# chemprop/chemprop

Measured on AMD Instinct MI355X. Metric: million directed-edge-updates/sec (depth=3, hidden=300), higher is better.
Workload: dtype f32 (exact 3-term f16 split of fp32 operands, fp32 accumulate); 1 GPU; qm9-shaped synthetic molecules, 512 mols/GPU/step, BondMessagePassing depth=3 hidden=300, forward (plan K0 + K1..K5); mols_per_gpu=512, directed_edges_per_gpu=9120, parallelism=dp1 (molecule shards, no data-path collective), launch=eager

## Files before the change

### chemprop_amd/_lib.py

```python
from __future__ import annotations

import ctypes as C
import os
import shutil
import subprocess
from typing import Optional

_HERE = os.path.dirname(os.path.abspath(__file__))
_ROOT = os.path.dirname(_HERE)
CSRC = os.path.join(_HERE, "csrc")
INCLUDE = os.path.join(_ROOT, "include")
LIB_PATH = os.environ.get("DMPNN_LIB") or os.path.join(_HERE, "libdmpnn_gfx950.so")
SOURCES = ["dmpnn_abi.hip", "dmpnn_prepare.hip", "dmpnn_segment.hip", "dmpnn_gemm.hip", "dmpnn_gemm_p1.hip",
           "dmpnn_gemm_p2.hip", "dmpnn_gemm_p3.hip", "dmpnn_gemm_p4.hip", "dmpnn_gemm_s1.hip", "dmpnn_mega.hip", "dmpnn_mega16.hip", "dmpnn_mega16_lp.hip", "dmpnn_mega16_bwd.hip", "dmpnn_rows16.hip", "dmpnn_step16.hip", "dmpnn_bstep16.hip", "dmpnn_backward.hip", "dmpnn_molagg.hip", "dmpnn_collate.hip", "dmpnn_tiles_large.hip", "dmpnn_optim.hip", "dmpnn_wgrad16.hip", "dmpnn_head.hip", "dmpnn_vd.hip"]
HEADERS = ["dmpnn_common.hpp", "dmpnn_spill_impl.hpp", "dmpnn_gemm_impl.hpp", "dmpnn_mega_impl.hpp", "dmpnn_mega16_impl.hpp", "dmpnn_mega16_bwd_impl.hpp", "dmpnn_rows16_impl.hpp", "dmpnn_seg16.hpp", "dmpnn_step16_impl.hpp"]
ABI_VERSION = 15
PLAN_NOFFSETS = 15

EXPORTS = [
    "dmpnn_version", "dmpnn_debug_timestamps", "dmpnn_last_error_string", "dmpnn_last_launch_count", "dmpnn_plan_bytes",
    "dmpnn_plan_layout", "dmpnn_prepare", "dmpnn_prepare_light", "dmpnn_prepare_tiles", "dmpnn_message_fwd", "dmpnn_aggregate_fwd",
    "dmpnn_linear_fwd", "dmpnn_linear16_wsplit_bytes", "dmpnn_linear16_ok", "dmpnn_linear16_fwd", "dmpnn_update_fwd", "dmpnn_forward", "dmpnn_forward_can_fuse", "dmpnn_forward_wsplit_bytes", "dmpnn_forward_keep_bits_bytes", "dmpnn_forward_spill_bytes", "dmpnn_backward_ws_bytes", "dmpnn_backward", "dmpnn_message_bwd",
    "dmpnn_aggregate_bwd", "dmpnn_linear_wgrad_ws_bytes", "dmpnn_linear_wgrad",
    "dmpnn_molagg_ws_bytes", "dmpnn_molagg_bounds", "dmpnn_molagg_fwd", "dmpnn_molagg_bwd", "dmpnn_gather_rows", "dmpnn_collate", "dmpnn_pack_tiles", "dmpnn_max_tiles",
    "dmpnn_prepare_tiles_from_table", "dmpnn_prepare_with_batch", "dmpnn_tile_plan_any_size", "dmpnn_split_row_floats", "dmpnn_forward_can_fuse16", "dmpnn_adam_step",
    "dmpnn_full_plan_keeps_tiles", "dmpnn_head_ws_bytes", "dmpnn_head", "dmpnn_train_step", "dmpnn_forward_tiles", "dmpnn_forward_route", "dmpnn_dropout_keep",
    "dmpnn_clip_grad", "dmpnn_clip_grad_ws_bytes", "dmpnn_train_route", "dmpnn_forward_h0_bytes", "dmpnn_tile_waves", "dmpnn_debug_lds_poison",
    "dmpnn_vd_ws_bytes", "dmpnn_vd_forward", "dmpnn_vd_backward",
]

ACT = {"none": 0, "relu": 1, "leakyrelu": 2, "prelu": 3, "tanh": 4, "elu": 5}
F_UNDIRECTED = 1
F_FUSED = 2
F_MEGA = 4
F_KEEP = 8
F_SPLIT16 = 16
F_WSPLIT_READY = 32
F_LOADER_TILES = 64
F_STORE16 = 128
F_ATOM = 1024
F_TILE_PLAN = 2048
F_H0_RESIDUAL = 256
F_ROW_FINALIZE = 512
ROUTES = ("general", "general16", "fused", "fused16", "mega", "mega16")
PLAN_NOMEGA_MASK = 15
PLAN_NOFUSE_MASK = 7


class GemmArgs(C.Structure):
    _fields_ = [
        ("M", C.c_int64), ("N", C.c_int64), ("K1", C.c_int64), ("K2", C.c_int64),
        ("A1", C.c_void_p), ("lda1", C.c_int64), ("gather1", C.c_void_p), ("gather1_rows", C.c_int64),
        ("A2", C.c_void_p), ("lda2", C.c_int64),
        ("W", C.c_void_p), ("ldw", C.c_int64),
        ("bias", C.c_void_p),
        ("Cadd", C.c_void_p), ("ldcadd", C.c_int64),
        ("C", C.c_void_p), ("ldc", C.c_int64),
        ("Zpre", C.c_void_p), ("ldz", C.c_int64),
        ("act", C.c_int), ("act_slope", C.c_float), ("act_slope_ptr", C.c_void_p),
    ]


class FwdArgs(C.Structure):
    _fields_ = [
        ("plan", C.c_void_p), ("n_atoms", C.c_int64), ("n_edges", C.c_int64),
        ("d_v", C.c_int64), ("d_e", C.c_int64), ("d_h", C.c_int64), ("d_vd", C.c_int64),
        ("depth", C.c_int32), ("flags", C.c_uint32),
        ("act", C.c_int32), ("act_slope", C.c_float), ("act_slope_ptr", C.c_void_p),
        ("V", C.c_void_p), ("ldv", C.c_int64),
        ("E", C.c_void_p), ("lde", C.c_int64),
        ("V_d", C.c_void_p), ("ldvd", C.c_int64),
        ("W_i", C.c_void_p), ("b_i", C.c_void_p),
        ("W_h", C.c_void_p), ("b_h", C.c_void_p),
        ("W_o", C.c_void_p), ("b_o", C.c_void_p),
        ("W_d", C.c_void_p), ("b_d", C.c_void_p),
        ("ldh", C.c_int64), ("H0", C.c_void_p), ("Hs", C.c_void_p), ("n_hslots", C.c_int32),
        ("Ms", C.c_void_p), ("n_mslots", C.c_int32),
        ("Mv", C.c_void_p), ("Hv", C.c_void_p),
        ("out", C.c_void_p), ("ldout", C.c_int64),
        ("wsplit", C.c_void_p), ("wsplit_bytes", C.c_size_t),
        ("edge_index", C.c_void_p), ("rev_edge_index", C.c_void_p),
        ("n_tiles_launch", C.c_int64),
        ("spill_ws", C.c_void_p), ("spill_bytes", C.c_size_t),
        ("msplit", C.c_void_p), ("msplit_bytes", C.c_size_t),
        ("dropout_p", C.c_float), ("dropout_seed", C.c_uint64),
        ("keep_bits", C.c_void_p), ("keep_bits_bytes", C.c_size_t),
        ("h0_bytes", C.c_size_t),
    ]


class BwdArgs(C.Structure):
    _fields_ = [
        ("f", FwdArgs), ("gout", C.c_void_p), ("ldgout", C.c_int64),
        ("gW_i", C.c_void_p), ("gb_i", C.c_void_p), ("gW_h", C.c_void_p), ("gb_h", C.c_void_p),
        ("gW_o", C.c_void_p), ("gb_o", C.c_void_p), ("gW_d", C.c_void_p), ("gb_d", C.c_void_p),
        ("ws", C.c_void_p), ("ws_bytes", C.c_size_t),
        ("g_edge", C.c_void_p), ("ld_gedge", C.c_int64),
    ]


MAX_FFN_LAYERS = 8
MAX_COMPONENTS = 8
DROP_SITE_FFN = 0x10000
LOSS = {"mse": 0, "mae": 1, "bce": 2, "ce": 3, "mve": 4, "evidential": 5, "quantile": 6}
STEP_FORWARD, STEP_BACKWARD, STEP_UPDATE = 1, 2, 4


class HeadArgs(C.Structure):
    _fields_ = [
        ("n_atoms", C.c_int64), ("n_mols", C.c_int64), ("d_h", C.c_int64),
        ("batch", C.c_void_p),
        ("agg_mode", C.c_int32), ("agg_norm", C.c_float),
        ("bn_weight", C.c_void_p), ("bn_bias", C.c_void_p), ("bn_running_mean", C.c_void_p), ("bn_running_var", C.c_void_p),
        ("bn_eps", C.c_float), ("bn_momentum", C.c_float), ("bn_training", C.c_int32),
        ("n_layers", C.c_int32), ("act", C.c_int32), ("act_slope", C.c_float),
        ("W", C.c_void_p * MAX_FFN_LAYERS), ("b", C.c_void_p * MAX_FFN_LAYERS), ("dims", C.c_int64 * (MAX_FFN_LAYERS + 1)),
        ("loss", C.c_int32),
        ("targets", C.c_void_p), ("weights", C.c_void_p), ("task_weights", C.c_void_p), ("lt_mask", C.c_void_p), ("gt_mask", C.c_void_p),
        ("preds", C.c_void_p), ("loss_out", C.c_void_p),
        ("gW", C.c_void_p * MAX_FFN_LAYERS), ("gb", C.c_void_p * MAX_FFN_LAYERS), ("g_bn_weight", C.c_void_p), ("g_bn_bias", C.c_void_p),
        ("gHv", C.c_void_p), ("ldg", C.c_int64),
        ("ws", C.c_void_p), ("ws_bytes", C.c_size_t),
        ("bn_num_batches_tracked", C.c_void_p),
        ("n_classes", C.c_int32),
        ("evid_v_kl", C.c_float), ("evid_eps", C.c_float), ("quantile_alpha", C.c_float),
        ("X_d", C.c_void_p), ("ld_xd", C.c_int64),
        ("n_components", C.c_int32),
        ("ffn_dropout_p", C.c_float), ("ffn_dropout_seed", C.c_uint64),
    ]


class TrainRouteInfo(C.Structure):
    _fields_ = [("plan_kind", C.c_int32), ("route", C.c_int32), ("keep_rows", C.c_int32), ("keep_bits", C.c_int32), ("lean", C.c_int32)]


class StepComponent(C.Structure):
    _fields_ = [
        ("edge_index", C.c_void_p), ("rev_edge_index", C.c_void_p), ("batch", C.c_void_p), ("plan_bytes", C.c_size_t), ("plan_ready", C.c_int32),
        ("bwd", BwdArgs),
    ]


class VdArgs(C.Structure):
    _fields_ = [
        ("n_atoms", C.c_int64), ("d_h", C.c_int64), ("d_vd", C.c_int64),
        ("Hv", C.c_void_p), ("ldhv", C.c_int64),
        ("V_d", C.c_void_p), ("ldvd", C.c_int64),
        ("W_d", C.c_void_p), ("b_d", C.c_void_p),
        ("out", C.c_void_p), ("ldout", C.c_int64),
        ("gout", C.c_void_p), ("ldgout", C.c_int64),
        ("gHv", C.c_void_p), ("ldghv", C.c_int64),
        ("gW_d", C.c_void_p), ("gb_d", C.c_void_p),
        ("ws", C.c_void_p), ("ws_bytes", C.c_size_t),
    ]


VD_MAX_WIDTH = 544


class StepArgs(C.Structure):
    _fields_ = [
        ("edge_index", C.c_void_p), ("rev_edge_index", C.c_void_p), ("batch", C.c_void_p), ("plan_bytes", C.c_size_t), ("plan_ready", C.c_int32),
        ("stages", C.c_int32),
        ("bwd", BwdArgs), ("head", HeadArgs),
        ("p", C.c_void_p), ("g", C.c_void_p), ("m", C.c_void_p), ("v", C.c_void_p), ("n_params", C.c_int64),
        ("lr", C.c_float), ("beta1", C.c_float), ("beta2", C.c_float), ("eps", C.c_float), ("weight_decay", C.c_float),
        ("bias_corr1", C.c_float), ("sqrt_bias_corr2", C.c_float), ("grad_scale", C.c_float), ("dev_scalars", C.c_void_p),
        ("clip_val", C.c_float), ("clip_mode", C.c_int32), ("clip_ws", C.c_void_p),
        ("n_extra", C.c_int32), ("extra", C.POINTER(StepComponent)),
        ("vd", C.POINTER(VdArgs)),
    ]


def sources() -> list[str]:
    return [os.path.join(CSRC, s) for s in SOURCES if os.path.isfile(os.path.join(CSRC, s))]


def _stale() -> bool:
    if os.environ.get("DMPNN_LIB"):
        return False
    if not os.path.isfile(LIB_PATH):
        return True
    t = os.path.getmtime(LIB_PATH)
    deps = sources() + [os.path.join(CSRC, h) for h in HEADERS] + [os.path.join(INCLUDE, "dmpnn.h")]
    return any(os.path.getmtime(d) > t for d in deps if os.path.isfile(d))


def build(force: bool = False, verbose: bool = False, defines=(), out: Optional[str] = None) -> str:
    lib_path = out or LIB_PATH
    if not force and not _stale() and out is None:
        return LIB_PATH
    hipcc = shutil.which("hipcc") or "/opt/rocm/bin/hipcc"
    if not os.path.isfile(hipcc):
        raise RuntimeError("hipcc not found: cannot build libdmpnn_gfx950.so")
    import concurrent.futures as cf
    import tempfile

    flags = ["--offload-arch=gfx950", "-O3", "-std=c++17", "-fPIC", f"-I{INCLUDE}", f"-I{CSRC}", *[f"-D{d}" for d in defines]]
    with tempfile.TemporaryDirectory(prefix="dmpnn_build_") as tmp:
        def cc(src):
            obj = os.path.join(tmp, os.path.basename(src) + ".o")
            cmd = [hipcc, *flags, "-c", src, "-o", obj]
            if verbose:
                print(" ".join(cmd))
            r = subprocess.run(cmd, capture_output=True, text=True)
            if r.returncode != 0:
                raise RuntimeError(f"hipcc failed on {src} ({r.returncode}):\n{r.stdout}\n{r.stderr}")
            return obj

        with cf.ThreadPoolExecutor(max_workers=8) as ex:
            objs = list(ex.map(cc, sources()))
        linked = os.path.join(os.path.dirname(objs[0]), "libdmpnn.so")
        cmd = [hipcc, "--offload-arch=gfx950", "-shared", "-fPIC", *objs, "-o", linked]
        if verbose:
            print(" ".join(cmd))
        r = subprocess.run(cmd, capture_output=True, text=True)
        if r.returncode != 0:
            raise RuntimeError(f"hipcc link failed ({r.returncode}):\n{r.stdout}\n{r.stderr}")
        shutil.copyfile(linked, lib_path + ".tmp")
        os.chmod(lib_path + ".tmp", 0o755)
    os.replace(lib_path + ".tmp", lib_path)
    _clean_unbundle_temporaries(lib_path)
    return lib_path


def _clean_unbundle_temporaries(lib_path: str) -> int:
    import glob

    n = 0
    for f in glob.glob(glob.escape(lib_path) + ".*"):
        tail = f[len(lib_path) + 1:]
        if tail.split(".", 1)[0].isdigit() and ("hipv4-" in tail or "host-" in tail):
            try:
                os.remove(f)
                n += 1
            except OSError:
                pass
    return n


_lib: Optional[C.CDLL] = None


def load() -> C.CDLL:
    global _lib
    if _lib is not None:
        return _lib
    import torch

    if _stale() and (shutil.which("hipcc") or os.path.isfile("/opt/rocm/bin/hipcc")):
        build()
    if not os.path.isfile(LIB_PATH):
        raise RuntimeError(
            f"{LIB_PATH} is missing: run `python -c 'import __graft_entry__ as g; g.build()'` "
            "(the MI355X engine has no CPU / eager fallback)")
    lib = C.CDLL(LIB_PATH)
    lib.dmpnn_version.restype = C.c_int
    lib.dmpnn_last_error_string.restype = C.c_char_p
    lib.dmpnn_last_launch_count.restype = C.c_int
    lib.dmpnn_plan_bytes.restype = C.c_size_t
    lib.dmpnn_plan_bytes.argtypes = [C.c_int64, C.c_int64]
    lib.dmpnn_plan_layout.argtypes = [C.c_int64, C.c_int64, C.POINTER(C.c_int64)]
    lib.dmpnn_forward_can_fuse.argtypes = [C.POINTER(FwdArgs)]
    lib.dmpnn_prepare.argtypes = [C.c_void_p, C.c_void_p, C.c_int64, C.c_int64, C.c_void_p, C.c_size_t, C.c_void_p]
    lib.dmpnn_prepare_light.argtypes = lib.dmpnn_prepare.argtypes
    lib.dmpnn_prepare_tiles.argtypes = [C.c_void_p, C.c_void_p, C.c_void_p, C.c_int64, C.c_int64, C.c_void_p, C.c_size_t, C.c_void_p]
    lib.dmpnn_message_fwd.argtypes = [C.c_void_p, C.c_int64, C.c_int64, C.c_int64, C.c_void_p, C.c_int64,
                                      C.c_void_p, C.c_int64, C.c_int, C.c_float, C.c_void_p, C.c_uint, C.c_void_p]
    lib.dmpnn_aggregate_fwd.argtypes = [C.c_void_p, C.c_int64, C.c_int64, C.c_int64, C.c_void_p, C.c_int64,
                                        C.c_void_p, C.c_int64, C.c_int, C.c_float, C.c_void_p, C.c_void_p]
    lib.dmpnn_linear_fwd.argtypes = [C.POINTER(GemmArgs), C.c_void_p]
    lib.dmpnn_update_fwd.argtypes = [C.c_void_p, C.c_int64, C.c_int64, C.c_int64, C.c_void_p, C.c_int64, C.c_void_p, C.c_int64,
                                     C.c_void_p, C.c_void_p, C.c_void_p, C.c_int64, C.c_void_p, C.c_int64, C.c_void_p,
                                     C.c_int64, C.c_int, C.c_float, C.c_void_p, C.c_void_p]
    lib.dmpnn_forward.argtypes = [C.POINTER(FwdArgs), C.c_void_p]
    lib.dmpnn_backward_ws_bytes.argtypes = [C.POINTER(FwdArgs)]
    lib.dmpnn_backward.argtypes = [C.POINTER(BwdArgs), C.c_void_p]
    lib.dmpnn_message_bwd.argtypes = [C.c_void_p, C.c_int64, C.c_int64, C.c_int64, C.c_void_p, C.c_int64,
                                      C.c_void_p, C.c_int64, C.c_void_p]
    lib.dmpnn_aggregate_bwd.argtypes = lib.dmpnn_message_bwd.argtypes
    lib.dmpnn_linear_wgrad_ws_bytes.argtypes = [C.c_int64, C.c_int64, C.c_int64, C.c_int]
    lib.dmpnn_linear_wgrad.argtypes = [C.POINTER(GemmArgs), C.c_void_p, C.c_int64, C.c_void_p, C.c_int64,
                                       C.c_void_p, C.c_void_p, C.c_size_t, C.c_void_p]
    size_t_fns = ("dmpnn_plan_bytes", "dmpnn_backward_ws_bytes", "dmpnn_linear_wgrad_ws_bytes", "dmpnn_forward_wsplit_bytes", "dmpnn_forward_spill_bytes",
                  "dmpnn_forward_keep_bits_bytes",
                  "dmpnn_molagg_ws_bytes", "dmpnn_linear16_wsplit_bytes", "dmpnn_head_ws_bytes", "dmpnn_clip_grad_ws_bytes", "dmpnn_forward_h0_bytes", "dmpnn_vd_ws_bytes")
    lib.dmpnn_linear16_wsplit_bytes.argtypes = [C.c_int64, C.c_int64]
    lib.dmpnn_linear16_ok.argtypes = [C.POINTER(GemmArgs)]
    lib.dmpnn_linear16_fwd.argtypes = [C.POINTER(GemmArgs), C.c_void_p, C.c_size_t, C.c_int, C.c_void_p]
    lib.dmpnn_gather_rows.argtypes = [C.c_void_p, C.c_int64, C.c_int64, C.c_void_p, C.c_int64, C.c_int64, C.c_void_p, C.c_int64,
                                      C.c_void_p]
    lib.dmpnn_pack_tiles.argtypes = [C.c_void_p, C.c_void_p, C.c_int64, C.c_void_p, C.c_void_p, C.c_int64]
    lib.dmpnn_pack_tiles.restype = C.c_int64
    lib.dmpnn_max_tiles.argtypes = [C.c_int64, C.c_int64]
    lib.dmpnn_prepare_with_batch.argtypes = [C.c_void_p, C.c_void_p, C.c_void_p, C.c_int64, C.c_int64, C.c_void_p, C.c_size_t, C.c_void_p]
    lib.dmpnn_prepare_with_batch.restype = C.c_int
    lib.dmpnn_tile_plan_any_size.argtypes = [C.c_int64, C.c_int64]
    lib.dmpnn_max_tiles.restype = C.c_int64
    lib.dmpnn_prepare_tiles_from_table.argtypes = [C.c_void_p, C.c_void_p, C.c_int64, C.c_int64, C.c_int64, C.c_void_p, C.c_size_t,
                                                   C.c_void_p]
    lib.dmpnn_collate.argtypes = [C.c_void_p, C.c_void_p, C.c_int64, C.c_void_p, C.c_void_p, C.c_void_p, C.c_int64, C.c_int64,
                                  C.c_void_p, C.c_void_p, C.c_void_p, C.c_void_p]
    lib.dmpnn_molagg_ws_bytes.argtypes = [C.c_int64]
    lib.dmpnn_molagg_bounds.argtypes = [C.c_void_p, C.c_int64, C.c_int64, C.c_void_p, C.c_size_t, C.c_void_p]
    lib.dmpnn_molagg_fwd.argtypes = [C.c_void_p, C.c_int64, C.c_int64, C.c_int64, C.c_int64, C.c_void_p, C.c_int, C.c_float,
                                     C.c_void_p, C.c_int64, C.c_void_p]
    lib.dmpnn_molagg_bwd.argtypes = [C.c_void_p, C.c_int64, C.c_void_p, C.c_int64, C.c_int64, C.c_int64, C.c_void_p, C.c_int,
                                     C.c_float, C.c_void_p, C.c_int64, C.c_void_p]
    lib.dmpnn_forward_wsplit_bytes.argtypes = [C.POINTER(FwdArgs)]
    lib.dmpnn_forward_keep_bits_bytes.argtypes = [C.POINTER(FwdArgs)]
    lib.dmpnn_forward_spill_bytes.argtypes = [C.POINTER(FwdArgs)]
    lib.dmpnn_forward_h0_bytes.argtypes = [C.POINTER(FwdArgs)]
    lib.dmpnn_forward_can_fuse16.argtypes = [C.POINTER(FwdArgs)]
    lib.dmpnn_adam_step.argtypes = [C.c_void_p, C.c_void_p, C.c_void_p, C.c_void_p, C.c_int64, C.c_float, C.c_float, C.c_float, C.c_float,
                                    C.c_float, C.c_float, C.c_float, C.c_float, C.c_void_p, C.c_void_p]
    lib.dmpnn_train_route.argtypes = [C.POINTER(FwdArgs), C.c_int64, C.c_int32, C.c_int32, C.c_int32, C.c_int32, C.c_int32, C.POINTER(TrainRouteInfo)]
    lib.dmpnn_clip_grad.argtypes = [C.c_void_p, C.c_int64, C.c_float, C.c_int32, C.c_float, C.c_void_p, C.c_void_p]
    lib.dmpnn_dropout_keep.argtypes = [C.c_uint64, C.c_int32, C.c_int64, C.c_int64, C.c_float]
    lib.dmpnn_forward_route.argtypes = [C.POINTER(FwdArgs), C.c_int, C.c_int, C.c_int, C.c_int]
    lib.dmpnn_tile_waves.restype = C.c_int
    lib.dmpnn_tile_waves.argtypes = [C.c_int64, C.c_int64, C.c_int64, C.c_int64]
    lib.dmpnn_forward_tiles.argtypes = [C.POINTER(FwdArgs), C.c_void_p, C.c_void_p, C.c_void_p, C.c_int64, C.c_size_t, C.c_void_p]
    lib.dmpnn_full_plan_keeps_tiles.argtypes = [C.c_int64, C.c_int64]
    lib.dmpnn_head_ws_bytes.argtypes = [C.POINTER(HeadArgs)]
    lib.dmpnn_head.argtypes = [C.POINTER(HeadArgs), C.c_void_p, C.c_int64, C.c_void_p]
    lib.dmpnn_train_step.argtypes = [C.POINTER(StepArgs), C.c_void_p]
    lib.dmpnn_vd_ws_bytes.argtypes = [C.POINTER(VdArgs)]
    lib.dmpnn_vd_forward.argtypes = [C.POINTER(VdArgs), C.c_void_p]
    lib.dmpnn_vd_backward.argtypes = [C.POINTER(VdArgs), C.c_void_p]
    lib.dmpnn_split_row_floats.argtypes = [C.c_int64]
    lib.dmpnn_split_row_floats.restype = C.c_int64
    lib.dmpnn_debug_timestamps.argtypes = [C.c_void_p]
    for name in size_t_fns:
        getattr(lib, name).restype = C.c_size_t
    for name in EXPORTS:
        if name != "dmpnn_last_error_string" and name not in size_t_fns and name not in ("dmpnn_pack_tiles", "dmpnn_max_tiles", "dmpnn_split_row_floats"):
            getattr(lib, name).restype = C.c_int
    if lib.dmpnn_version() != ABI_VERSION:
        raise RuntimeError(f"libdmpnn ABI version {lib.dmpnn_version()} != {ABI_VERSION} (stale build?)")
    _lib = lib
    return lib


_ENV_DATA = getattr(os.environ, "_data", None)
_ENV_KEYS: dict = {}


def opt(name: str, default: str) -> str:
    if _ENV_DATA is None or os.name != "posix":
        return os.environ.get(name, default)
    k = _ENV_KEYS.get(name)
    if k is None:
        k = _ENV_KEYS[name] = name.encode()
    v = _ENV_DATA.get(k)
    return default if v is None else v.decode()


class DmpnnError(RuntimeError):
    pass


def check(rc: int, what: str) -> None:
    if rc != 0:
        msg = load().dmpnn_last_error_string().decode(errors="replace")
        raise DmpnnError(f"{what} failed (code {rc}): {msg}")
```

### chemprop_amd/csrc/dmpnn_abi.hip

```cpp
#include <stdarg.h>
#include <stdlib.h>
#include <string.h>

#include "dmpnn_common.hpp"
#include "dmpnn_mega16_impl.hpp"

namespace dmpnn {

static thread_local char g_err[512] = "";
static thread_local int g_launches = 0;

void set_error(const char* fmt, ...) {
    va_list ap;
    va_start(ap, fmt);
    vsnprintf(g_err, sizeof(g_err), fmt, ap);
    va_end(ap);
}
static __global__ __launch_bounds__(1024) void k_debug_lds_poison(unsigned pat, unsigned* sink) {
    extern __shared__ unsigned lds_words[];
    constexpr int n = (160 * 1024 - 64) / 4;
    for (int i = threadIdx.x; i < n; i += 1024) lds_words[i] = pat;
    __syncthreads();
    if (sink && lds_words[(threadIdx.x * 7) % n] == 0x12345u) sink[0] = 1;
}
// ... 209 lines not shown
    if (n_edges == 0) {
        if (Mv && n_atoms > 0) {
            for (int64_t v = 0; v < n_atoms; ++v)
                if (hipMemsetAsync(Mv + v * ld_mv, 0, (size_t)d_h * sizeof(float), static_cast<hipStream_t>(stream)) != hipSuccess) {
                    set_error("update_fwd: memset failed");
                    return DMPNN_EHIP;
                }
        }
        return DMPNN_OK;
    }
    const int* plan_i = static_cast<const int*>(plan);
    const PlanLayout L = plan_layout(n_atoms, n_edges);
    dmpnn_gemm_args g;
    memset(&g, 0, sizeof(g));
    g.M = n_edges; g.N = d_h; g.K1 = d_h;
    g.A1 = M; g.lda1 = ld_m;
    g.W = W_h; g.ldw = d_h; g.bias = b_h;
    g.Cadd = H0; g.ldcadd = ld_h0;
    g.C = H_out; g.ldc = ld_hout;
    g.act = act; g.act_slope = act_slope; g.act_slope_ptr = act_slope_ptr;
    GemmExtra x;
    memset(&x, 0, sizeof(x));
    x.seg = true;
    x.tile_row = plan_i + L.tile_row; x.tile_atom = plan_i + L.tile_atom; x.n_tiles = (int)L.max_tiles;
    x.row_ptr = plan_i + L.row_ptr; x.revp = plan_i + L.revp;
    x.Mout = M_next; x.ldm = ld_mnext; x.Sout = Mv; x.lds = ld_mv;
    return launch_linear_ex(g, x, static_cast<hipStream_t>(stream));
}

static size_t steps16_wsplit_bytes(const dmpnn_fwd_args& a) {
    const int64_t h = a.d_h;
    size_t n = linear16_wsplit_bytes(h, a.d_v + a.d_e) + linear16_wsplit_bytes(h, h) + linear16_wsplit_bytes(h, a.d_v + h);
    n += linear16_wsplit_bytes(h + a.d_vd, h + a.d_vd) * ((a.W_d && a.d_vd > 0) ? 1 : 0);
    n += linear16_wsplit_bytes(h, h) + linear16_wsplit_bytes(h, a.d_v);
    return n;
}

size_t dmpnn_forward_wsplit_bytes(const dmpnn_fwd_args* a) {
    if (!a || a->d_h <= 0 || a->d_v <= 0 || a->d_e < 0) return 0;
    return (a->flags & DMPNN_F_MEGA) ? mega16_wsplit_bytes(*a) : steps16_wsplit_bytes(*a);
}

static bool keep_bits_apply(const dmpnn_fwd_args& a) {
    const unsigned need = DMPNN_F_TILE_PLAN | DMPNN_F_KEEP | DMPNN_F_MEGA | DMPNN_F_SPLIT16 | DMPNN_F_FUSED;
    return (a.flags & need) == need && (a.act == DMPNN_ACT_NONE || a.act == DMPNN_ACT_RELU || a.act == DMPNN_ACT_LEAKYRELU) &&
           !(a.dropout_p > 0.f) && !a.W_d && a.n_atoms > 0 && a.n_edges > 0;
}
size_t dmpnn_forward_keep_bits_bytes(const dmpnn_fwd_args* a) {
    if (!a) return 0;
    if ((a->flags & (DMPNN_F_FUSED | DMPNN_F_SPLIT16)) == (DMPNN_F_FUSED | DMPNN_F_SPLIT16) && !(a->flags & DMPNN_F_MEGA)) return fused16_lean_bits_bytes(*a);
    if (!keep_bits_apply(*a)) return 0;
    return (size_t)a->depth * (size_t)plan_layout(a->n_atoms, a->n_edges).max_mtiles * 256u * 8u;
}

size_t dmpnn_forward_h0_bytes(const dmpnn_fwd_args* a) { return a ? fused16_h0q_bytes(*a) : 0; }

size_t dmpnn_forward_spill_bytes(const dmpnn_fwd_args* a) {
    if (!a || a->n_atoms < 0 || a->n_edges < 0 || a->ldh <= 0) return 0;
    return (size_t)(3 * a->n_edges + a->n_atoms) * (size_t)a->ldh * sizeof(float);
}

static bool al_ptr(const void* p, int bytes) { return (reinterpret_cast<uintptr_t>(p) & (uintptr_t)(bytes - 1)) == 0; }

int dmpnn_forward_can_fuse(const dmpnn_fwd_args* a) {
    if (!a) return 0;
    const int64_t h = a->d_h, dv = a->d_v, de = a->d_e;
    if (a->flags & DMPNN_F_UNDIRECTED) return 0;
    if (h <= 0 || h % 4 != 0 || h > 320 || a->ldh % 4 != 0) return 0;
    if (dv % 2 != 0 || de % 2 != 0 || a->ldv % 2 != 0 || a->lde % 2 != 0) return 0;
    if (!al_ptr(a->V, 8) || !al_ptr(a->E, 8) || !al_ptr(a->W_i, 8) || !al_ptr(a->W_h, 16)) return 0;
    if (!al_ptr(a->H0, 16) || !al_ptr(a->Ms, 16) || !al_ptr(a->Mv, 16) || (a->Hs && !al_ptr(a->Hs, 16))) return 0;
    if (a->n_atoms * a->ldv * 4 > 0x7FFFFFFF || a->n_edges * a->lde * 4 > 0x7FFFFFFF) return 0;
    return mega_shapes_ok(*a) ? 2 : 1;
}

static const int64_t kSteps16MinEdges = 20000, kFused16MinEdges = 2048;

int dmpnn_tile_waves(int64_t n_atoms, int64_t n_edges, int64_t d_h, int64_t n_tiles) {
    dmpnn_fwd_args t;
    memset(&t, 0, sizeof(t));
    t.n_atoms = n_atoms; t.n_edges = n_edges; t.d_h = d_h;
    return tile_waves(t, n_tiles > 0 ? (int)n_tiles : (int)plan_layout(n_atoms, n_edges).max_mtiles);
}

int dmpnn_forward_route(const dmpnn_fwd_args* a, int keep, int max_level, int plan_kind, int arith) {
    if (!a || max_level < 0 || plan_kind < 0 || plan_kind > 2 || arith < 0 || arith > 1) return -1;
    const bool undirected = (a->flags & DMPNN_F_UNDIRECTED) != 0;
    int level = undirected ? 0 : dmpnn_forward_can_fuse(a);
    if (level > max_level) level = max_level;
    if (plan_kind == 2) return (level == 2 && arith == 0 && !(keep && a->W_d)) ? DMPNN_ROUTE_MEGA16 : -1;
    if (plan_kind == 1 && keep) return -1;
    const int64_t nE = a->n_edges, h = a->d_h;
    if (!keep && !undirected && arith == 0 && nE >= kFused16MinEdges && (level == 1 || (level == 0 && h > 320 && max_level >= 1))) {
        dmpnn_fwd_args t = *a;
        t.flags &= ~(unsigned)(DMPNN_F_KEEP | DMPNN_F_STORE16);
        if (fused16_shapes_ok(t)) return DMPNN_ROUTE_FUSED16;
    }
    if (keep && level == 1 && arith == 0 && nE >= kSteps16MinEdges && plan_kind == 0) {
        dmpnn_fwd_args t = *a;
        t.flags = (t.flags | DMPNN_F_FUSED | DMPNN_F_SPLIT16) & ~(unsigned)(DMPNN_F_MEGA | DMPNN_F_STORE16);
        if (fused16_lean_shapes(t)) return DMPNN_ROUTE_FUSED16;
    }
    if (level == 1 && arith == 0 && nE >= kSteps16MinEdges && plan_kind != 1) level = 0;
    if (level == 2) return arith == 0 ? DMPNN_ROUTE_MEGA16 : DMPNN_ROUTE_MEGA;
    if (level == 1) return DMPNN_ROUTE_FUSED;
    if (plan_kind == 1) return -1;
    return (arith == 0 && (h > 320 || nE >= kSteps16MinEdges)) ? DMPNN_ROUTE_GENERAL16 : DMPNN_ROUTE_GENERAL;
}

int dmpnn_train_route(const dmpnn_fwd_args* a, int64_t n_mols, int32_t have, int32_t oversize, int32_t max_level, int32_t arith,
                      int32_t keep_rows, dmpnn_train_route_info* out) {
    DMPNN_CHECK_ARG(a && out && max_level >= 0 && (arith == 0 || arith == 1) && keep_rows >= -1 && keep_rows <= 1, "train_route: bad arguments");
    memset(out, 0, sizeof(*out));
    const int64_t nV = a->n_atoms, nE = a->n_edges, h = a->d_h;
    const bool undirected = (a->flags & DMPNN_F_UNDIRECTED) != 0, atom = (a->flags & DMPNN_F_ATOM) != 0;
    const bool relu_class = a->act == DMPNN_ACT_RELU || a->act == DMPNN_ACT_LEAKYRELU;
    const bool builtin = a->act == DMPNN_ACT_NONE || relu_class || a->act == DMPNN_ACT_TANH || a->act == DMPNN_ACT_ELU;
    bool tiles = !undirected && !a->W_d && builtin && max_level >= 2 && arith == 0 && nE > 0 && nV > 0 && oversize != 1;
    if (a->dropout_p > 0.f && !relu_class) tiles = false;
    if (!(h > 0 && h % 4 == 0 && h <= 320 && a->d_v % 2 == 0 && a->d_e % 2 == 0)) tiles = false;
    if (atom && !(a->d_e >= 2 && a->d_e <= 16) ) tiles = false;
    const bool small = small_plan_fits(nV, nE), table = (have & 2) != 0, large = (have & 1) != 0 && tiles_large_fits(nV, nE);
    if (!(small || table || large)) tiles = false;
    if (!(n_mols > 0 && nE <= 30 * n_mols && (table || large || small))) tiles = false;
    out->plan_kind = tiles ? 2 : 0;
    int cap = max_level;
    if (oversize == 1 && cap > 1) cap = 1;
    dmpnn_fwd_args t = *a;
    if (table || large) t.flags |= DMPNN_F_LOADER_TILES;
    out->route = dmpnn_forward_route(&t, 1, cap, out->plan_kind, arith);
    if (out->route < 0 && out->plan_kind == 2) {
        out->plan_kind = 0;
        out->route = dmpnn_forward_route(&t, 1, cap, 0, arith);
    }
    const int64_t n_steps = a->depth > 1 ? a->depth - 1 : 0;
    const bool rows = keep_rows == 1 || (keep_rows < 0 && nE * n_steps >= DMPNN_KEEP_ROWS_MIN);
    out->keep_rows = (!atom && n_steps > 0 && h > 0 && h <= 320 && rows) ? 1 : 0;
    if (out->route == DMPNN_ROUTE_MEGA16) {
        out->keep_bits = (out->plan_kind == 2 && (relu_class || a->act == DMPNN_ACT_NONE) && !(a->dropout_p > 0.f)) ? 1 : 0;
    } else if (out->route == DMPNN_ROUTE_FUSED16) {
        dmpnn_fwd_args l = *a;
        l.flags = (l.flags | DMPNN_F_FUSED | DMPNN_F_SPLIT16) & ~(unsigned)(DMPNN_F_MEGA | DMPNN_F_STORE16);
        out->lean = fused16_lean_shapes(l) ? 1 : 0;
        out->keep_bits = out->lean;
    }
    return DMPNN_OK;
}

int dmpnn_forward_tiles(const dmpnn_fwd_args* a, const int64_t* batch, const int* tile_row, const int* tile_atom, int64_t n_tiles,
                        size_t plan_bytes, void* stream) {
    DMPNN_CHECK_ARG(a != nullptr && a->plan != nullptr, "forward_tiles: null args / plan");
    void* plan = const_cast<void*>(a->plan);
    bool did_split = false;
    if (tile_row && tile_atom && n_tiles > 0) {
        const dmpnn::PlanLayout L = dmpnn::plan_layout(a->n_atoms, a->n_edges);
        const bool ok = a->n_atoms >= 0 && a->n_edges >= 0 && a->n_atoms < (1ll << 31) && a->n_edges < (1ll << 31) &&
                        plan_bytes >= (size_t)L.words * sizeof(int) && n_tiles <= L.max_mtiles;
        if (ok) DMPNN_TRY(launch_tiles_from_table_split(tile_row, tile_atom, n_tiles, a->n_atoms, a->n_edges, static_cast<int*>(plan),
                                                        static_cast<hipStream_t>(stream), a, &did_split));
        if (!did_split)
            DMPNN_TRY(dmpnn_prepare_tiles_from_table(tile_row, tile_atom, n_tiles, a->n_atoms, a->n_edges, plan, plan_bytes, stream));
    } else
        DMPNN_TRY(prepare_tiles_and_bounds(a->edge_index, a->rev_edge_index, batch, a->n_atoms, a->n_edges, plan, plan_bytes, nullptr, 0, stream, nullptr, a, &did_split));
    if (!did_split) return dmpnn_forward(a, stream);
    dmpnn_fwd_args f = *a;
    f.flags |= DMPNN_F_WSPLIT_READY;
    return dmpnn_forward(&f, stream);
}

int dmpnn_forward(const dmpnn_fwd_args* a, void* stream) {
    g_launches = 0;
    DMPNN_CHECK_ARG(a != nullptr, "forward: null args");
    DMPNN_TRY(check_graph_sizes(a->n_atoms, a->n_edges));
    const int64_t nV = a->n_atoms, nE = a->n_edges, h = a->d_h, dv = a->d_v, de = a->d_e;
    DMPNN_CHECK_ARG(a->plan, "forward: null plan");
    DMPNN_CHECK_ARG(h > 0 && dv > 0 && de >= 0 && a->d_vd >= 0 && a->depth >= 1, "forward: bad dimensions");
    DMPNN_CHECK_ARG(a->act >= DMPNN_ACT_RELU && a->act <= DMPNN_ACT_ELU,
                    "forward: activation %d is not built in (chain the row kernels instead)", a->act);
    DMPNN_CHECK_ARG(a->act != DMPNN_ACT_PRELU || a->act_slope_ptr, "forward: PReLU needs act_slope_ptr");
    DMPNN_CHECK_ARG(a->W_i && a->W_h && a->W_o && a->b_o, "forward: null weight");
    DMPNN_CHECK_ARG(a->ldh >= h && a->ldv >= dv && a->lde >= de, "forward: leading dimension too small");
    DMPNN_CHECK_ARG(nV == 0 || (a->V && a->Mv && a->out), "forward: null V / Mv / out");
    DMPNN_CHECK_ARG(nE == 0 || (a->E && (a->H0 || (a->flags & DMPNN_F_MEGA))), "forward: null E / H0");
    const bool has_vd = a->W_d != nullptr;
    DMPNN_CHECK_ARG(!has_vd || (a->d_vd > 0 && a->V_d && a->b_d && a->Hv && a->ldvd >= a->d_vd),
                    "forward: W_d given but V_d / b_d / Hv / d_vd missing");
    DMPNN_CHECK_ARG(a->ldout >= h + (has_vd ? a->d_vd : 0), "forward: ldout too small");
    const bool fused = a->flags & DMPNN_F_FUSED;
    DMPNN_CHECK_ARG(!(a->flags & DMPNN_F_STORE16) || (fused && (a->flags & DMPNN_F_SPLIT16) && !(a->flags & (DMPNN_F_KEEP | DMPNN_F_ATOM))),
                    "forward: DMPNN_F_STORE16 only goes with the fused routes on the f16 pipe (DMPNN_F_FUSED | DMPNN_F_SPLIT16 [| DMPNN_F_MEGA]), inference, bond messages");
    const bool lean16 = fused && (a->flags & DMPNN_F_SPLIT16) && (a->flags & DMPNN_F_KEEP) && !(a->flags & DMPNN_F_MEGA) && a->keep_bits;
    if (a->depth > 1 && nE > 0 && !(a->flags & DMPNN_F_MEGA) && !lean16) {
        DMPNN_CHECK_ARG(a->Ms && a->n_mslots >= 1, "forward: missing Ms workspace");
        DMPNN_CHECK_ARG(fused || (a->Hs && a->n_hslots >= 1), "forward: missing Hs workspace");
    }

    if (a->flags & DMPNN_F_ATOM) {
        DMPNN_CHECK_ARG((a->flags & DMPNN_F_FUSED) && (a->flags & DMPNN_F_MEGA) && (a->flags & DMPNN_F_SPLIT16) &&
                        !has_vd && de >= 1 && de <= 16 && a->dropout_p == 0.f,
                        "forward: DMPNN_F_ATOM (atom messages) runs on the whole-forward tile kernel only (DMPNN_F_FUSED | DMPNN_F_MEGA | "
                        "DMPNN_F_SPLIT16, 1 <= d_e <= 16, no W_d, no dropout inside the kernels) — chain the row kernels otherwise");
        DMPNN_CHECK_ARG(!(a->flags & DMPNN_F_KEEP) || (de % 2 == 0 && dv % 2 == 0 && h % 2 == 0 &&
                        (a->depth < 2 || nE == 0 || (a->msplit && aligned16(a->msplit) && a->msplit_bytes >= (size_t)(a->depth - 1) * (size_t)nE * 16 * sizeof(float)))),
                        "forward: DMPNN_F_ATOM | DMPNN_F_KEEP needs even d_v / d_e / d_h and `msplit` >= (depth - 1) * n_edges * 64 bytes, 16-byte aligned");
    }
    if (a->dropout_p != 0.f) {
        DMPNN_CHECK_ARG(a->dropout_p > 0.f && a->dropout_p < 1.f, "forward: dropout_p must lie in [0, 1)");
        const bool tile_train = (a->flags & DMPNN_F_MEGA) && (a->flags & DMPNN_F_SPLIT16) && (a->flags & DMPNN_F_KEEP);
        const bool lean_train = lean16 && fused16_lean_shapes(*a, true);
        DMPNN_CHECK_ARG(lean_train || (tile_train && !has_vd && (a->act == DMPNN_ACT_RELU || a->act == DMPNN_ACT_LEAKYRELU)),
                        "forward: dropout inside the kernels needs the training forward of the tile kernel (DMPNN_F_MEGA | DMPNN_F_SPLIT16 | "
                        "DMPNN_F_KEEP) or the lean training forward of the per-step fused route (DMPNN_F_FUSED | DMPNN_F_SPLIT16 | DMPNN_F_KEEP "
                        "with keep_bits; d_h <= 320, d_h %% 4 == 0, even d_v / d_e, depth 2 .. %d, a full plan), a ReLU-class activation and "
                        "no W_d — run dropout between the row kernels otherwise", kWProdMaxJobs);
    }
    hipStream_t s = static_cast<hipStream_t>(stream);
    const PlanView pv = plan_view(a->plan, nV, nE);
    const int64_t slot = nE * a->ldh;
    const int* plan_i = static_cast<const int*>(a->plan);

    if (fused && (a->flags & DMPNN_F_SPLIT16) && !(a->flags & DMPNN_F_MEGA)) {
        DMPNN_CHECK_ARG(fused16_shapes_ok(*a), "forward: DMPNN_F_FUSED | DMPNN_F_SPLIT16 given but the shapes do not allow it "
                        "(directed, d_h %% 4 == 0, d_h <= 640, even d_v / d_e; with DMPNN_F_KEEP: depth - 1 kept H / M slots and `msplit`)");
        DMPNN_CHECK_ARG(nE == 0 || (a->H0 && ((a->flags & DMPNN_F_KEEP) ? (a->Ms || a->depth == 1 || lean16) : (a->Ms && a->n_mslots >= 2))),
                        "forward(fused16): H0 and two split message slots (training: `msplit` + the kept fp32 slots) are required");
        DMPNN_CHECK_ARG(a->wsplit && a->wsplit_bytes >= steps16_wsplit_bytes(*a), "forward(fused16): wsplit workspace missing or too small");
        SplitWView w[6];
        unsigned char* wp = static_cast<unsigned char*>(a->wsplit);
        const bool ready = (a->flags & DMPNN_F_WSPLIT_READY) != 0;
        const float* Ws[6] = {a->W_i, a->W_h, a->W_o, has_vd ? a->W_d : nullptr, a->W_o + dv, a->W_o};
        const int64_t Ns[6] = {h, h, h, h + a->d_vd, h, h}, Ks[6] = {dv + de, h, dv + h, h + a->d_vd, h, dv};
        const int64_t Ls[6] = {dv + de, h, dv + h, h + a->d_vd, dv + h, dv + h};
        SplitWJob jobs[6];
        SplitWView views[6];
        int idx[6], nj = 0;
        for (int i = 0; i < 6; ++i) {
            if (!Ws[i]) continue;
            if (ready) w[i] = split_weights_view_of(wp, Ns[i], Ks[i]);
            else { jobs[nj] = SplitWJob{Ws[i], Ls[i], Ns[i], Ks[i], 0, wp}; idx[nj++] = i; }
            wp += linear16_wsplit_bytes(Ns[i], Ks[i]);
        }
        mega16::SplitArgs sp;
        const bool pend = nj > 0 && split_weights_args(jobs, nj, views, &sp);
        for (int k = 0; k < nj; ++k) w[idx[k]] = views[k];
        DMPNN_TRY(launch_fused16_forward(*a, w, has_vd ? a->Hv : a->out, has_vd ? a->ldh : a->ldout, s, pend ? &sp : nullptr));
        if (has_vd) {
            dmpnn_gemm_args g;
            memset(&g, 0, sizeof(g));
            g.M = nV; g.N = h + a->d_vd; g.K1 = h; g.K2 = a->d_vd;
            g.A1 = a->Hv; g.lda1 = a->ldh;
            g.A2 = a->V_d; g.lda2 = a->ldvd;
            g.W = a->W_d; g.ldw = h + a->d_vd; g.bias = a->b_d;
            g.C = a->out; g.ldc = a->ldout; g.act = DMPNN_ACT_NONE;
            if (linear16_ok(g)) DMPNN_TRY(launch_linear16_view(g, w[3], nullptr, 0, s));
            else DMPNN_TRY(launch_linear(g, s));
        }
        return DMPNN_OK;
    }
    if (fused) {
        DMPNN_CHECK_ARG(dmpnn_forward_can_fuse(a), "forward: DMPNN_F_FUSED given but the shapes / alignment do not allow it "
                        "(d_h %% 4, d_h <= 320, even d_v / d_e, directed); call dmpnn_forward_can_fuse first");
        const PlanLayout L = plan_layout(nV, nE);
        DMPNN_CHECK_ARG((a->flags & DMPNN_F_MEGA) || a->depth <= 2 || a->n_mslots >= 2,
                        "forward(fused): depth > 2 needs at least two message slots");
        if (a->flags & DMPNN_F_MEGA) {
            DMPNN_CHECK_ARG(mega_shapes_ok(*a), "forward: DMPNN_F_MEGA given but the shapes do not allow it");
            DMPNN_CHECK_ARG(!a->keep_bits || (keep_bits_apply(*a) && aligned16(a->keep_bits) && a->keep_bits_bytes >= dmpnn_forward_keep_bits_bytes(a)),
                            "forward: keep_bits needs DMPNN_F_TILE_PLAN | DMPNN_F_KEEP on the tile kernel (f16 pipe), a ReLU-class activation, no "
                            "dropout, no W_d, and dmpnn_forward_keep_bits_bytes() bytes");
            DMPNN_CHECK_ARG(!(a->flags & DMPNN_F_KEEP) || a->depth == 1 || nE == 0 ||
                            (a->Hs && a->n_hslots >= a->depth - 1 && a->n_mslots >= a->depth - 1),
                            "forward(mega, keep): needs depth-1 H and M slots");
            if (nV > 0) {
                if (a->flags & DMPNN_F_SPLIT16) DMPNN_TRY(launch_mega16_forward(*a, has_vd ? a->Hv : a->out, has_vd ? a->ldh : a->ldout, s));
                else DMPNN_TRY(launch_mega_forward(*a, has_vd ? a->Hv : a->out, has_vd ? a->ldh : a->ldout, s));
            }
            if (has_vd) {
                dmpnn_gemm_args g;
                memset(&g, 0, sizeof(g));
                g.M = nV; g.N = h + a->d_vd; g.K1 = h; g.K2 = a->d_vd;
                g.A1 = a->Hv; g.lda1 = a->ldh;
                g.A2 = a->V_d; g.lda2 = a->ldvd;
                g.W = a->W_d; g.ldw = h + a->d_vd; g.bias = a->b_d;
                g.C = a->out; g.ldc = a->ldout; g.act = DMPNN_ACT_NONE;
                DMPNN_TRY(launch_linear(g, s));
            }
            return DMPNN_OK;
        }
        GemmExtra x;
        memset(&x, 0, sizeof(x));
        x.seg = true;
        x.tile_row = plan_i + L.tile_row; x.tile_atom = plan_i + L.tile_atom; x.n_tiles = nE > 0 ? (int)L.max_tiles : 0;
        x.row_ptr = plan_i + L.row_ptr; x.revp = plan_i + L.revp;
        const int T = a->depth;
        if (nE == 0 && nV > 0) {
            hipError_t e = hipMemsetAsync(a->Mv, 0, (size_t)nV * a->ldh * sizeof(float), s);
            if (e != hipSuccess) { set_error("forward: memset failed: %s", hipGetErrorString(e)); return DMPNN_EHIP; }
        }
        if (nE > 0) {
            dmpnn_gemm_args g;
            memset(&g, 0, sizeof(g));
            g.M = nE; g.N = h; g.K1 = dv; g.K2 = de;
            g.A1 = a->V; g.lda1 = a->ldv; g.gather1 = plan_i + L.srcp; g.gather1_rows = nV;
            g.A2 = a->E; g.lda2 = a->lde;
            g.W = a->W_i; g.ldw = dv + de; g.bias = a->b_i;
            g.Zpre = a->H0; g.ldz = a->ldh;
            g.act = a->act; g.act_slope = a->act_slope; g.act_slope_ptr = a->act_slope_ptr;
// ... 127 lines not shown
```

### chemprop_amd/csrc/dmpnn_collate.hip

```cpp
#include "dmpnn_common.hpp"

namespace dmpnn {
namespace {

__device__ __forceinline__ int owner(const int* __restrict__ off, int n_mols, int i) {
    int lo = 0, hi = n_mols;
    while (hi - lo > 1) {
        const int mid = (lo + hi) >> 1;
        if (off[mid] <= i) lo = mid; else hi = mid;
    }
    return lo;
}

__global__ __launch_bounds__(256) void k_collate(const int* __restrict__ atom_off, const int* __restrict__ edge_off, int n_mols,
                                                 const int* __restrict__ src, const int* __restrict__ dst,
                                                 const int* __restrict__ rev, int nV, int nE, long long* __restrict__ edge_index,
                                                 long long* __restrict__ rev_edge_index, long long* __restrict__ batch) {
    const int n = nE > nV ? nE : nV;
    for (int i = blockIdx.x * blockDim.x + threadIdx.x; i < n; i += gridDim.x * blockDim.x) {
        if (i < nE) {
            const int s = src[i], d = dst[i], r = rev[i];
            const int m = owner(edge_off, n_mols, i);
            const long long a0 = atom_off[m], e0 = edge_off[m];
            edge_index[i] = s + a0;
            edge_index[(long long)nE + i] = d + a0;
            rev_edge_index[i] = r + e0;
        }
        if (i < nV) batch[i] = owner(atom_off, n_mols, i);
    }
}

__global__ __launch_bounds__(256) void k_tiles_from_table(const int* __restrict__ tile_row, const int* __restrict__ tile_atom,
                                                          int n_tiles, int nV, int nE, int* __restrict__ plan, PlanLayout L) {
    tiles_from_table_body(tile_row, tile_atom, n_tiles, nV, nE, plan, L);
}

}
}

extern "C" int64_t dmpnn_pack_tiles(const int* atom_off, const int* edge_off, int64_t n_mols, int* tile_row, int* tile_atom,
                                    int64_t cap) {
    if (n_mols < 0 || cap < 1 || !tile_row || !tile_atom || (n_mols > 0 && (!atom_off || !edge_off))) return -2;
    int64_t n = 0, m = 0;
    while (m < n_mols) {
        const int a0 = atom_off[m], e0 = edge_off[m];
        int64_t q = m;
        while (q < n_mols && atom_off[q + 1] - a0 <= dmpnn::kMegaBA && edge_off[q + 1] - e0 <= dmpnn::kMegaBM) ++q;
        if (q == m) q = m + 1;
        if (atom_off[q] == a0 && edge_off[q] == e0) { m = q; continue; }
        if (n + 1 >= cap) return -2;
        tile_row[n] = e0; tile_atom[n] = a0;
        ++n;
        m = q;
    }
    tile_row[n] = n_mols ? edge_off[n_mols] : 0;
    tile_atom[n] = n_mols ? atom_off[n_mols] : 0;
    return n;
}

extern "C" int64_t dmpnn_max_tiles(int64_t n_atoms, int64_t n_edges) { return dmpnn::mega_max_tiles(n_atoms, n_edges); }

extern "C" int dmpnn_prepare_tiles_from_table(const int* tile_row, const int* tile_atom, int64_t n_tiles, int64_t n_atoms,
                                              int64_t n_edges, void* plan, size_t plan_bytes, void* stream) {
    DMPNN_CHECK_ARG(n_atoms >= 0 && n_edges >= 0 && n_tiles >= 0 && n_atoms < (1ll << 31) && n_edges < (1ll << 31), "tiles_from_table: bad sizes");
    DMPNN_CHECK_ARG(plan && (n_tiles == 0 || (tile_row && tile_atom)), "tiles_from_table: NULL pointer");
    const dmpnn::PlanLayout L = dmpnn::plan_layout(n_atoms, n_edges);
    if (plan_bytes < (size_t)L.words * sizeof(int)) {
        dmpnn::set_error("tiles_from_table: plan buffer too small (%zu < %zu bytes)", plan_bytes, (size_t)L.words * sizeof(int));
        return DMPNN_ENOSPC;
    }
    DMPNN_CHECK_ARG(n_tiles <= L.max_mtiles, "tiles_from_table: %lld tiles exceed the launch bound %lld of this batch size",
                    (long long)n_tiles, (long long)L.max_mtiles);
    hipLaunchKernelGGL(dmpnn::k_tiles_from_table, dim3(1), dim3(256), 0, static_cast<hipStream_t>(stream), tile_row, tile_atom,
                       (int)n_tiles, (int)n_atoms, (int)n_edges, static_cast<int*>(plan), L);
    DMPNN_CHECK_LAUNCH("k_tiles_from_table");
    return DMPNN_OK;
}

extern "C" int dmpnn_collate(const int* atom_off, const int* edge_off, int64_t n_mols, const int* src, const int* dst,
                             const int* rev, int64_t n_atoms, int64_t n_edges, int64_t* edge_index, int64_t* rev_edge_index,
                             int64_t* batch, void* stream) {
    DMPNN_CHECK_ARG(n_mols >= 0 && n_atoms >= 0 && n_edges >= 0 && n_atoms < (1ll << 31) && n_edges < (1ll << 31) && n_mols < (1ll << 31),
                    "collate: bad sizes");
    if (n_atoms == 0 && n_edges == 0) return DMPNN_OK;
    DMPNN_CHECK_ARG(n_mols > 0 && atom_off && edge_off, "collate: atoms / edges without molecules");
    DMPNN_CHECK_ARG(n_edges == 0 || (src && dst && rev && edge_index && rev_edge_index), "collate: NULL edge arrays");
    DMPNN_CHECK_ARG(n_atoms == 0 || batch, "collate: NULL batch");
    const int64_t n = n_edges > n_atoms ? n_edges : n_atoms;
    int64_t blocks = (n + 255) / 256;
    if (blocks > 4096) blocks = 4096;
    hipLaunchKernelGGL(dmpnn::k_collate, dim3((unsigned)blocks), dim3(256), 0, static_cast<hipStream_t>(stream), atom_off, edge_off,
                       (int)n_mols, src, dst, rev, (int)n_atoms, (int)n_edges, reinterpret_cast<long long*>(edge_index),
                       reinterpret_cast<long long*>(rev_edge_index), reinterpret_cast<long long*>(batch));
    DMPNN_CHECK_LAUNCH("k_collate");
    return DMPNN_OK;
}
```

### chemprop_amd/csrc/dmpnn_common.hpp

```cpp
#pragma once

#include <hip/hip_runtime.h>
#include <stdint.h>
#include <stdio.h>
#include <string.h>

#include "dmpnn.h"

namespace dmpnn {

namespace mega16 { struct SplitArgs; }

void set_error(const char* fmt, ...);
void count_launch(const char* name);

#define DMPNN_CHECK_ARG(cond, ...)                 \
    do {                                           \
        if (!(cond)) {                             \
            ::dmpnn::set_error(__VA_ARGS__);       \
            return DMPNN_EINVAL;                   \
        }                                          \
    } while (0)

#define DMPNN_CHECK_LAUNCH(name)                                                         \
    do {                                                                                 \
        hipError_t e__ = hipGetLastError();                                              \
        if (e__ != hipSuccess) {                                                         \
            ::dmpnn::set_error("launch of %s failed: %s", name, hipGetErrorString(e__)); \
            return DMPNN_EHIP;                                                           \
        }                                                                                \
        ::dmpnn::count_launch(name);                                                     \
    } while (0)

#define DMPNN_TRY(expr)               \
    do {                              \
        int rc__ = (expr);            \
        if (rc__ != DMPNN_OK) return rc__; \
    } while (0)

constexpr int kFusedBM = 48;
constexpr int kFusedMaxDeg = 24;
constexpr int kFusedMinB0 = kFusedBM - kFusedMaxDeg + 1;
constexpr int kMegaBM = 48;
constexpr int kMegaBA = 32;
struct PlanLayout {
    int64_t src, dst, rev, row_ptr, perm, cursor, inv, srcp, dstp, revp, ident, tile_row, tile_atom, mtile_row, mtile_atom, words;
    int64_t max_tiles, max_mtiles;
};
inline int64_t align4(int64_t x) { return (x + 3) & ~int64_t(3); }
inline int64_t fused_max_tiles(int64_t nE) { return (nE + kFusedMinB0 - 1) / kFusedMinB0 + 1; }
inline int64_t mega_max_tiles(int64_t nV, int64_t nE) { return 2 * (nE / kMegaBM + nV / kMegaBA) + 4 + nV / 64 + 1; }
inline PlanLayout plan_layout(int64_t nV, int64_t nE) {
    PlanLayout L;
    int64_t o = DMPNN_HDR_WORDS;
    L.src = o; o += align4(nE);
    L.dst = o; o += align4(nE);
    L.rev = o; o += align4(nE);
    L.row_ptr = o; o += align4(nV + 1);
    L.perm = o; o += align4(nE);
    L.cursor = o; o += align4(nV);
    L.inv = o; o += align4(nE);
    L.srcp = o; o += align4(nE);
    L.dstp = o; o += align4(nE);
    L.revp = o; o += align4(nE);
    L.ident = o; o += align4(nE);
    L.max_tiles = fused_max_tiles(nE);
    L.tile_row = o; o += align4(L.max_tiles + 2);
    L.tile_atom = o; o += align4(L.max_tiles + 2);
    L.max_mtiles = mega_max_tiles(nV, nE);
    L.mtile_row = o; o += align4(L.max_mtiles + 2);
    L.mtile_atom = o; o += align4(L.max_mtiles + 2);
    L.words = o;
    return L;
}

enum : int { PLAN_ASYMMETRIC = 1, PLAN_RANGE_ERROR = 2, PLAN_HUGE_DEGREE = 4, PLAN_NO_PIECE_TILES = 8,
             PLAN_TILES_ONLY = 16 };
constexpr int kPlanNoFuse = PLAN_ASYMMETRIC | PLAN_RANGE_ERROR | PLAN_HUGE_DEGREE | PLAN_TILES_ONLY;
constexpr int kPlanNoMegaLean = PLAN_RANGE_ERROR | PLAN_NO_PIECE_TILES;
constexpr int kPlanNoMega = kPlanNoFuse | PLAN_NO_PIECE_TILES;

struct PlanView {
    const int* hdr;
    const int* src;
    const int* dst;
    const int* rev;
    const int* row_ptr;
    const int* perm;
};
inline PlanView plan_view(const void* plan, int64_t nV, int64_t nE) {
    const int* p = static_cast<const int*>(plan);
    PlanLayout L = plan_layout(nV, nE);
    return PlanView{p, p + L.src, p + L.dst, p + L.rev, p + L.row_ptr, p + L.perm};
}
inline PlanView plan_view_rows(const void* plan, int64_t nV, int64_t nE) {
    const int* p = static_cast<const int*>(plan);
    PlanLayout L = plan_layout(nV, nE);
    return PlanView{p, p + L.srcp, p + L.dstp, p + L.revp, p + L.row_ptr, p + L.ident};
}

__host__ __device__ __forceinline__ unsigned drop_hash(unsigned seed_lo, unsigned seed_hi, unsigned site, unsigned row, unsigned col) {
    unsigned h = (row * 1024u + col) ^ seed_lo ^ (site * 0x9E3779B9u);
    h ^= h >> 16; h *= 0x7FEB352Du; h ^= h >> 15; h += seed_hi; h *= 0x846CA68Bu; h ^= h >> 16;
    h *= 0x9E3779B1u; h ^= h >> 15;
    return h;
}
inline unsigned drop_threshold(float p) {
    const double t = (double)p * 4294967296.0;
    return t >= 4294967295.0 ? 4294967295u : (unsigned)t;
}

template <int BYTES>
__device__ __forceinline__ void warm_kernargs() {
    const unsigned long long kp = (unsigned long long)__builtin_amdgcn_kernarg_segment_ptr();
    constexpr int L = (BYTES + 63) / 64;
    static_assert(L <= 12, "argument block larger than the warm-up covers");
    int d[12];
#define DMPNN_WARM(i) if constexpr (L > i) asm volatile("s_load_dword %0, %1, %2" : "=s"(d[i]) : "s"(kp), "n"(i * 64));
    DMPNN_WARM(0) DMPNN_WARM(1) DMPNN_WARM(2) DMPNN_WARM(3) DMPNN_WARM(4) DMPNN_WARM(5)
    DMPNN_WARM(6) DMPNN_WARM(7) DMPNN_WARM(8) DMPNN_WARM(9) DMPNN_WARM(10) DMPNN_WARM(11)
#undef DMPNN_WARM
    asm volatile("s_waitcnt lgkmcnt(0)" ::: "memory");
}

__device__ __forceinline__ float apply_act(float z, int act, float slope) {
    switch (act) {
        case DMPNN_ACT_RELU: return z < 0.f ? 0.f : z;
        case DMPNN_ACT_LEAKYRELU:
        case DMPNN_ACT_PRELU: return z > 0.f ? z : slope * z;
        case DMPNN_ACT_TANH: return tanhf(z);
        case DMPNN_ACT_ELU: return z > 0.f ? z : expm1f(z);
        default: return z;
    }
}
__device__ __noinline__ float apply_act_slow(float z, int act) {
    return act == DMPNN_ACT_TANH ? tanhf(z) : (z > 0.f ? z : expm1f(z));
}
__device__ __forceinline__ float apply_act_small(float z, int act, float slope) {
    if (act == DMPNN_ACT_TANH || act == DMPNN_ACT_ELU) return apply_act_slow(z, act);
    const float neg = act == DMPNN_ACT_NONE ? 1.f : (act == DMPNN_ACT_RELU ? 0.f : slope);
    return (z > 0.f ? z : neg * z) + 0.f;
}
__device__ __forceinline__ float4 apply_act4(float4 z, int act, float slope) {
    if (act == DMPNN_ACT_NONE) return z;
    return make_float4(apply_act(z.x, act, slope), apply_act(z.y, act, slope),
                       apply_act(z.z, act, slope), apply_act(z.w, act, slope));
}
__device__ __forceinline__ float act_grad_from_out(float y, int act, float slope) {
    switch (act) {
        case DMPNN_ACT_RELU: return y > 0.f ? 1.f : 0.f;
        case DMPNN_ACT_LEAKYRELU: return y > 0.f ? 1.f : slope;
        case DMPNN_ACT_TANH: return 1.f - y * y;
        case DMPNN_ACT_ELU: return y > 0.f ? 1.f : y + 1.f;
        default: return 1.f;
    }
}

int launch_prepare(const int64_t* edge_index, const int64_t* rev, int64_t nV, int64_t nE, int* plan,
                   int light, hipStream_t s, bool keep_mtiles = false);
bool prepare_can_keep_mtiles(int64_t nV, int64_t nE);
__device__ __forceinline__ void tiles_from_table_body(const int* __restrict__ tile_row, const int* __restrict__ tile_atom,
                                                          int n_tiles, int nV, int nE, int* __restrict__ plan, PlanLayout L) {
    __shared__ int bad_s, spill_s;
    if (threadIdx.x == 0) { bad_s = 0; spill_s = 0; }
    __syncthreads();
    int* mrow = plan + L.mtile_row;
    int* matom = plan + L.mtile_atom;
    const int slots = (int)L.max_mtiles + 2;
    int bad = 0;
    for (int t = threadIdx.x; t < slots; t += blockDim.x) {
        int r = nE, a = nV;
        if (t < n_tiles) {
            r = tile_row[t]; a = tile_atom[t];
            const int r1 = t + 1 < n_tiles ? tile_row[t + 1] : nE, a1 = t + 1 < n_tiles ? tile_atom[t + 1] : nV;
            if (r < 0 || a < 0 || r1 < r || a1 < a || r1 > nE || a1 > nV) bad = 1;
            else if (a1 == a && r1 != r) bad = 1;
            else if (r1 - r > kMegaBM || a1 - a > kMegaBA) atomicAdd(&spill_s, 1);
            if (t == 0 && (r != 0 || a != 0)) bad = 1;
        }
        mrow[t] = r;
        matom[t] = a;
    }
    if (n_tiles == 0 && (nE > 0 || nV > 0)) bad = 1;
    if (bad) atomicOr(&bad_s, 1);
    __syncthreads();
    if (threadIdx.x < DMPNN_HDR_WORDS) {
        int v = 0;
        const int h = threadIdx.x;
        if (h == DMPNN_HDR_FLAGS) v = (bad_s ? PLAN_NO_PIECE_TILES : 0) | PLAN_TILES_ONLY;
        if (h == DMPNN_HDR_NMTILES) v = bad_s ? 0 : n_tiles;
        if (h == DMPNN_HDR_NSPILL) v = bad_s ? 0 : spill_s;
        if (h == DMPNN_HDR_LIGHT) v = 2;
        if (h == DMPNN_HDR_NATOMS) v = nV;
        if (h == DMPNN_HDR_NEDGES) v = nE;
        if (h == DMPNN_HDR_TILE_STRIDE) v = kFusedBM;
        plan[h] = v;
    }
}

int launch_tiles_from_table_split(const int* tile_row, const int* tile_atom, int64_t n_tiles, int64_t nV, int64_t nE, int* plan, hipStream_t s,
                                  const dmpnn_fwd_args* split_for, bool* did_split);
int launch_prepare_tiles_batch(const int64_t* edge_index, const int64_t* batch, int64_t nV, int64_t nE, int* plan, hipStream_t s,
                               int* mol_bounds = nullptr, int64_t n_mols = 0, const dmpnn_fwd_args* split_for = nullptr, bool* did_split = nullptr);
bool mega16_split_args(const dmpnn_fwd_args& a, mega16::SplitArgs* sp);
size_t fused16_h0q_bytes(const dmpnn_fwd_args& a);
bool mega16_keeps_rows(const dmpnn_fwd_args& a);
int prepare_tiles_and_bounds(const int64_t* edge_index, const int64_t* rev, const int64_t* batch, int64_t nV, int64_t nE, void* plan,
                             size_t plan_bytes, int* mol_bounds, int64_t n_mols, void* stream, bool* wrote_bounds,
                             const dmpnn_fwd_args* split_for = nullptr, bool* did_split = nullptr);
int molagg_fwd_rows(const float* H, int64_t ldh, int64_t n_atoms, int64_t d_h, int64_t n_mols, const void* ws, int mode,
                    float norm, float* out, int64_t ldo, int64_t rows, void* stream);
int molagg_bwd_rows(const float* gout, int64_t ldg, const int64_t* batch, int64_t n_atoms, int64_t d_h, int64_t n_mols,
                    const void* ws, int mode, float norm, float* gH, int64_t ldgh, int64_t rows, void* stream);
bool tiles_large_fits(int64_t nV, int64_t nE);
int launch_prepare_tiles_large(const int64_t* edge_index, const int64_t* batch, int64_t nV, int64_t nE, int* plan, hipStream_t s);
constexpr int kSmallPlanMaxAtoms = 6144, kSmallPlanMaxEdges = 10240;
inline size_t small_plan_lds_bytes(int64_t nV, int64_t nE) {
    return ((size_t)(3 * (nV + 2)) * 4 + (size_t)(5 * nE + 2) * 2 + 31) & ~size_t(15);
}
inline bool small_plan_fits(int64_t nV, int64_t nE) {
    return nV <= kSmallPlanMaxAtoms && nE <= kSmallPlanMaxEdges && small_plan_lds_bytes(nV, nE) <= 160 * 1024 - 2048;
}
int launch_message(const PlanView& pv, int64_t nV, int64_t nE, int64_t h, const float* Hin,
                   int64_t ld_in, float* M, int64_t ld_m, int act, float slope,
                   const float* slope_ptr, unsigned flags, hipStream_t s);
int launch_aggregate(const PlanView& pv, int64_t nV, int64_t nE, int64_t h, const float* Hin,
                     int64_t ld_in, float* Mv, int64_t ld_mv, int act, float slope,
                     const float* slope_ptr, hipStream_t s);
int launch_linear(const dmpnn_gemm_args& a, hipStream_t s);

struct GemmExtra {
    const int* gather2; int64_t gather2_rows;
    const int* tile_row; int n_tiles;
    bool seg;
    const int* tile_atom; const int* row_ptr; const int* revp;
    float* Mout; int64_t ldm;
    float* Sout; int64_t lds;
    const int* poison_flags; int poison_mask;
};
int launch_linear_ex(const dmpnn_gemm_args& a, const GemmExtra& x, hipStream_t s);
bool mega_shapes_ok(const dmpnn_fwd_args& a);
int launch_mega_forward(const dmpnn_fwd_args& a, float* out, int64_t ldout, hipStream_t s);
size_t mega16_wsplit_bytes(const dmpnn_fwd_args& a);
size_t mega16_fwd_wsplit_bytes(const dmpnn_fwd_args& a);
struct SplitWView { const unsigned char* p; const float* inv_scale; int nc; };
size_t linear16_wsplit_bytes(int64_t N, int64_t K);
int split_weights_view(const float* W, int64_t ldw, int64_t N, int64_t K, int tr, void* ws, SplitWView* out, hipStream_t s);
SplitWView split_weights_view_of(void* ws, int64_t N, int64_t K);
struct SplitWJob { const float* W; int64_t ldw, N, K; int tr; void* ws; };
int split_weights_views(const SplitWJob* jobs, int n, SplitWView* out, hipStream_t s);
bool split_weights_args(const SplitWJob* jobs, int n, SplitWView* out, mega16::SplitArgs* sp);
int launch_split_args(const mega16::SplitArgs& sp, hipStream_t s);
bool linear16_ok(const dmpnn_gemm_args& a);
int launch_linear16_view(const dmpnn_gemm_args& a, const SplitWView& W, const int* poison_flags, int poison_mask, hipStream_t s);
int launch_mega16_forward(const dmpnn_fwd_args& a, float* out, int64_t ldout, hipStream_t s);
int tile_waves(const dmpnn_fwd_args& a, int n_tiles);
bool fused16_shapes_ok(const dmpnn_fwd_args& a);
bool fused16_lean_shapes(const dmpnn_fwd_args& a, bool on_demand = false);
size_t fused16_lean_bits_bytes(const dmpnn_fwd_args& a);
bool fused16_lean(const dmpnn_fwd_args& a);
int64_t split_row_floats(int64_t d_h);

struct WSplitJob {
    int64_t M; int C;
    const float* A1; int64_t lda1; const int* g1; int K1;
    const float* A2; int64_t lda2; const int* g2; int K2;
    int ones;
    unsigned char* out; float* scales;
    int n_ct, n_chunks, wg0;
    const long long* g1_64; int64_t g1_rows;
};
struct WSplitArgs { WSplitJob job[8]; int n_jobs; };
struct WProdArgs {
    const unsigned char* Z; const float* sZ; const unsigned char* A; const float* sA;
    int n_nt, n_kt, n_chunks, chunks_per_split, splits;
    int N, Kt; float* slab; int ldk; int64_t slab_stride;
};
struct WProdPlan { int n_nt, n_kt, n_chunks, chunks_per_split, splits, ldk; int64_t slab_stride; };
constexpr int kWProdMaxJobs = 8;
struct WProdJobs { WProdArgs job[4]; int wg0[5]; int n_jobs; };
struct WProdRPlan { int n_kg, splits, rows_per_split, ldk; int64_t slab_stride; };
WProdRPlan plan_wgrad16r(int64_t M, int N, int K, int rows_per_split = 0);
void wgrad16r_plan_launch(const int64_t* M, const int* K, int n, int reserve, int* rows_out);
constexpr int kWProdRMaxJobs = 16;
struct WProdRJob { const unsigned char* Z; int tsz; const unsigned char* A; int tsa; int64_t M; int N, K; float* slab; WProdRPlan plan; float* slab_b; };
int launch_wgrad16r(const WProdRJob* jobs, int n, hipStream_t s);
struct SRJob { const float* A1; int64_t lda1; int K1; const int* g1; const long long* g1_64; int64_t g1_rows;
               const float* A2; int64_t lda2; int K2; const int* g2; int64_t M; unsigned char* out; int ts; };
int launch_rows2sr(const SRJob* jobs, int n, hipStream_t s);
size_t wsplit16_bytes(int64_t M, int64_t C);
struct AggRide {
    float* Hm; int ld; const int64_t* batch; int* table; int n_mols; int mode; float norm;
    bool taken;
};
extern thread_local AggRide g_agg_ride;
struct ExtraWgrad {
    const float* Z; int64_t ldz; const float* A; int64_t lda; int64_t M; int N, K, ones;
    float* gW; int64_t ldgw; float* gb; float* ws;
};
size_t extra_wgrad_ws_floats(int64_t M, int N, int Kt);
int backward_impl(const dmpnn_bwd_args* b, void* stream, const ExtraWgrad* extra, bool* extra_done);
void wsplit16_job(WSplitJob* j, int64_t M, int C, const float* A1, int64_t lda1, const int* g1, int K1, const float* A2, int64_t lda2,
                  const int* g2, int K2, int ones, void* ws);
int launch_wsplit16(WSplitArgs& a, hipStream_t s);
bool wgrad16_operand_ok(const float* A1, int64_t lda1, int K1, const float* A2, int64_t lda2, int K2);
WProdPlan plan_wgrad16(int64_t M, int N, int Kt);
void wgrad16_add(WProdJobs* jobs, const WSplitJob& Z, const WSplitJob& A, const WProdPlan& p, int N, int Kt, float* slab);
int launch_wgrad16(const WProdJobs& jobs, hipStream_t s);
int launch_fused16_forward(const dmpnn_fwd_args& a, const SplitWView* w16, float* out, int64_t ldout, hipStream_t s,
                           const mega16::SplitArgs* pending = nullptr);
int launch_bstep16(const dmpnn_fwd_args& f, int site, const float* Tin, const float* gMv, const SplitWView* W, float* Tout,
                   unsigned char* Zrows, hipStream_t s);
size_t mega16_bwd_wsplit_bytes(int64_t h);
struct Mega16BwdRows { unsigned char* gZ; unsigned char* gH0; unsigned char* gZO; int tsr; };
int launch_mega16_backward(const dmpnn_fwd_args& f, const float* gHO, int64_t ldg, const float* HO, int64_t ldho, float* gZO,
                           float* gZs, float* gH0, void* wsplit, float* sp_gM, float* sp_Ta, hipStream_t s, const float* g_edge = nullptr, int64_t ld_gedge = 0,
                           const Mega16BwdRows* rows = nullptr);

int vd_check_args(const dmpnn_vd_args* a, bool bwd);
int vd_forward_impl(const dmpnn_vd_args* a, void* stream);
int vd_backward_impl(const dmpnn_vd_args* a, void* stream, bool split_ready);

inline bool aligned16(const void* p) { return (reinterpret_cast<uintptr_t>(p) & 15u) == 0; }

inline int check_linear_lds(const dmpnn_gemm_args& a, const char* who) {
    const struct { bool live; int64_t ld, width; const char* name; } t[] = {
        {a.K1 > 0, a.lda1, a.K1, "lda1 < K1"},       {a.K2 > 0, a.lda2, a.K2, "lda2 < K2"},   {true, a.ldw, a.K1 + a.K2, "ldw < K1 + K2"},
        {a.Cadd != nullptr, a.ldcadd, a.N, "ldcadd < N"}, {a.C != nullptr, a.ldc, a.N, "ldc < N"}, {a.Zpre != nullptr, a.ldz, a.N, "ldz < N"}};
    for (const auto& x : t)
        DMPNN_CHECK_ARG(!x.live || x.ld >= x.width, "%s: leading dimension below its width (%s: %lld < %lld)", who, x.name, (long long)x.ld,
                        (long long)x.width);
    return DMPNN_OK;
}

}
```

### chemprop_amd/csrc/dmpnn_mega16_impl.hpp

```cpp
#pragma once

#include <type_traits>

#include "dmpnn_mega_impl.hpp"

namespace dmpnn {
namespace mega16 {

using gemm::BK;
using gemm::f32x4;
using gemm::kOOB;
using gemm::kThreads;
using gemm::rsrc_t;
using gemm::u32x4;
using gemm::u32x2;
using mega::RT_A;
using mega::RT_E;

typedef _Float16 h8 __attribute__((ext_vector_type(8)));
typedef _Float16 h4 __attribute__((ext_vector_type(4)));
typedef _Float16 h2 __attribute__((ext_vector_type(2)));


struct SplitW {
    const unsigned char* p;
    const float* inv_scale;
    int nc;
};

struct Mega16K {
    mega::MegaK m;
    SplitW Wi, Wh, WoM, WoV;
    SplitW WhE; int atom_de;
    float* atom_me; long long me_slot;
    unsigned char* Mrows; int tsr; long long mrow_slot;
    unsigned long long* keep_bits; long long bits_slot;
    float* agg_Hm; int agg_ld; const long long* agg_batch; const int* agg_bounds; int* agg_done; int agg_n_mols; int agg_mode; float agg_norm;
};

template <int I, int N, class F>
__device__ __forceinline__ void static_for(F&& f) {
    if constexpr (I < N) {
        f(std::integral_constant<int, I>{});
        static_for<I + 1, N>(f);
    }
}

__device__ __forceinline__ float scale_for(float maxabs) {
    if (!(maxabs > 0.f) || !(maxabs < 3.0e38f)) return 1.f;
    int e;
    frexpf(maxabs, &e);
    const int k = 14 - e;
    return ldexpf(1.f, k > 126 ? 126 : (k < -126 ? -126 : k));
}
__device__ __forceinline__ void store_keep4(float* p, float4 v) {
#if defined(DMPNN_NT_KEEP)
    __builtin_nontemporal_store(f32x4{v.x, v.y, v.z, v.w}, reinterpret_cast<f32x4*>(p));
#else
    *reinterpret_cast<float4*>(p) = v;
#endif
}
__device__ __forceinline__ void split2(float x0, float x1, float s, unsigned& hi, unsigned& lo) {
    const float a = x0 * s, b = x1 * s;
    const h2 h = h2{(_Float16)a, (_Float16)b};
    const h2 l = h2{(_Float16)(a - (float)h[0]), (_Float16)(b - (float)h[1])};
    hi = __builtin_bit_cast(unsigned, h); lo = __builtin_bit_cast(unsigned, l);
}
__device__ __forceinline__ void split4(float4 x, float s, h4& hi, h4& lo) {
    unsigned h0, l0, h1, l1;
    split2(x.x, x.y, s, h0, l0);
    split2(x.z, x.w, s, h1, l1);
    hi = __builtin_bit_cast(h4, u32x2{h0, h1});
    lo = __builtin_bit_cast(h4, u32x2{l0, l1});
}
__device__ __forceinline__ float rcp_pow2_exact(float s) { return __uint_as_float(0x7F000000u - __float_as_uint(s)); }

struct SplitJob {
    const float* W; int ldw; int col0; int K;
    int scale_col0, scale_K;
    unsigned char* out; int nc; float* inv_scale;
    int tr;
    int N;
};
struct SplitArgs {
    SplitJob job[8];
    int n_jobs, N;
};
__device__ __forceinline__ void split_weights_wave(const SplitArgs& a, int wave, int lane) {
    const int Np = (a.N + 15) & ~15;
    const int j = wave / Np, n = wave - j * Np;
    if (j >= a.n_jobs) return;
    const SplitJob& J = a.job[j];
    const int NJ = J.N > 0 ? J.N : a.N;
    if (n >= ((NJ + 15) & ~15)) return;
    const bool live = n < NJ;
    const long long rs = J.tr ? 1 : J.ldw, ks = J.tr ? J.ldw : 1;
    const float* row = J.W + (long long)(live ? n : 0) * rs;
    float mx = 0.f;
    for (int k = lane; k < J.scale_K; k += 64) mx = fmaxf(mx, fabsf(row[(J.scale_col0 + k) * ks]));
    for (int off = 32; off > 0; off >>= 1) mx = fmaxf(mx, __shfl_xor(mx, off));
    const float s = live ? scale_for(mx) : 0.f;
    if (lane == 0 && J.inv_scale && live) J.inv_scale[n] = 1.f / s;
    _Float16* out = reinterpret_cast<_Float16*>(J.out);
    const int T = n >> 4, li = n & 15;
    for (int k = lane; k < J.nc * 32; k += 64) {
        const float x = (k < J.K && live) ? row[(J.col0 + k) * ks] * s : 0.f;
        const _Float16 hi = (_Float16)x;
        const _Float16 lo = (_Float16)(x - (float)hi);
        const int c = k >> 5, kk = k & 31, lg = kk >> 3, j = kk & 7;
        const long long base = (((long long)T * J.nc + c) * 2) * 512 + (lg * 16 + li) * 8 + j;
        out[base] = hi;
        out[base + 512] = lo;
    }
}
static __global__ __launch_bounds__(256) void k_split_weights(SplitArgs a) {
    split_weights_wave(a, blockIdx.x * 4 + (threadIdx.x >> 6), threadIdx.x & 63);
}

__device__ __forceinline__ void rows_to_sr(const float* src, long long ld, long long row0, int nrows, int N, unsigned char* dst, int ts,
                                           int wave, int lane, int n_waves) {
    for (int r = wave; r < nrows; r += n_waves) {
        const float* x = src + (row0 + r) * ld;
        float v[8];
        float mx = 0.f;
#pragma unroll
        for (int j = 0; j < 8; ++j) {
            const int c = lane + 64 * j;
            v[j] = c < N ? x[c] : 0.f;
            mx = fmaxf(mx, fabsf(v[j]));
        }
        for (int off = 32; off > 0; off >>= 1) mx = fmaxf(mx, __shfl_xor(mx, off));
        const float sc = scale_for(mx);
        unsigned char* o = dst + (row0 + r) * ts;
#pragma unroll
        for (int j = 0; j < 8; ++j) {
            const int c = lane + 64 * j;
            if (c < N) {
                const float y = v[j] * sc;
                const _Float16 hi = (_Float16)y;
                *reinterpret_cast<_Float16*>(o + (c >> 5) * 128 + (c & 31) * 2) = hi;
                *reinterpret_cast<_Float16*>(o + (c >> 5) * 128 + 64 + (c & 31) * 2) = (_Float16)(y - (float)hi);
            }
        }
        if (lane == 0) *reinterpret_cast<float4*>(o + (ts - 16)) = make_float4(sc, mx > 0.f ? 0.f : 1.f, 0.f, 0.f);
    }
}

#if !defined(DMPNN_TILE8_BRING)
#define DMPNN_TILE8_BRING 1
#endif
template <int WN>
constexpr size_t tile_region_bytes() {
    constexpr size_t ts = 64 * WN * 4 + 16, tsg = 4 * 128 + 16;
    return (size_t)kMegaBM * (ts > tsg ? ts : tsg);
}
constexpr int kAtomK = 16;
constexpr size_t kAtomLds = (size_t)(kMegaBM + kMegaBA) * kAtomK * sizeof(float);
template <int WN>
constexpr size_t lds_bytes() {
    return tile_region_bytes<WN>() + (size_t)(3 * kMegaBM + kMegaBA + 24) * sizeof(int) + 10 * 64 * 16;
}
template <int WN>
constexpr size_t lds_bytes_atom() { return lds_bytes<WN>() + kAtomLds; }

template <int WN, bool SA, bool KEEP, int NW = 4, bool LP = false>
__global__ __launch_bounds__(64 * NW, 2) void k_mpnn_tile16(Mega16K G) {
    static_assert(!(LP && KEEP), "the hi-halves-alone form is inference only");
    static_assert(NW == 4 || (NW == 8 && WN == 5), "the 8-wave form splits 20 column tiles 3+3+3+3+2+2+2+2");
    const mega::MegaK& g = G.m;
    constexpr int KT = 64 * NW;
    constexpr int JR = 16 / NW;
    constexpr int BM = kMegaBM, BA = kMegaBA, BN = 64 * WN, LDC = BN + 4, QN = BN / 4;
    constexpr int TS = BN * 4 + 16;
    constexpr int ITEMS = (BM * QN + KT - 1) / KT;
    extern __shared__ __attribute__((aligned(16))) unsigned char lds[];
    unsigned char* T16 = lds;
    static_assert(LDC * 4 == TS, "the fp32 tile and the split A tile have the same footprint");
    constexpr int META_OFF = (int)tile_region_bytes<WN>();
    float* T = reinterpret_cast<float*>(lds);
    int* revl = reinterpret_cast<int*>(lds + META_OFF);
    int* aor = revl + BM;
    int* asrc = aor + BM;
    int* rp = asrc + BM;
    unsigned* maxbits = reinterpret_cast<unsigned*>(rp + BA + 1);
    h8* cfrag = reinterpret_cast<h8*>(lds + META_OFF + (((3 * BM + BA + 1 + 8) * 4 + 15) / 16) * 16);

    using T_ = std::true_type;
    using F_ = std::false_type;
    int tid = threadIdx.x, lane = tid & 63, wave = tid >> 6;
    int li = lane & 15, lg = lane >> 4;
    int kq = tid & 7;
    auto launder = [&]() {
        asm volatile("" : "+v"(tid));
        lane = tid & 63; wave = tid >> 6; li = lane & 15; lg = lane >> 4; kq = tid & 7;
    };
#if !defined(DMPNN_NO_KERNARG_WARM)
    warm_kernargs<(int)sizeof(Mega16K)>();
#endif
    int n_stamp = 0;
    auto stamp = [&]() {
        if (g.dbg && blockIdx.x == 0 && threadIdx.x == 0 && n_stamp < 32) g.dbg[n_stamp] = (long long)__builtin_readcyclecounter();
        ++n_stamp;
    };
    stamp();
    const int t = blockIdx.x;
    int rs = g.mtile_row[t], re = g.mtile_row[t + 1];
    int va = g.mtile_atom[t], vb = g.mtile_atom[t + 1];
    int hdr_light = g.flags[DMPNN_HDR_LIGHT], hdr_flags = g.flags[0], hdr_tiles = g.flags[DMPNN_HDR_NMTILES];
    asm volatile("" : "+v"(rs), "+v"(re), "+v"(va), "+v"(vb), "+v"(hdr_light), "+v"(hdr_flags), "+v"(hdr_tiles));
    rs = __builtin_amdgcn_readfirstlane(rs); re = __builtin_amdgcn_readfirstlane(re);
    va = __builtin_amdgcn_readfirstlane(va); vb = __builtin_amdgcn_readfirstlane(vb);
    hdr_light = __builtin_amdgcn_readfirstlane(hdr_light); hdr_flags = __builtin_amdgcn_readfirstlane(hdr_flags);
    hdr_tiles = __builtin_amdgcn_readfirstlane(hdr_tiles);
    const int nrows = re - rs, na = vb - va;
    const int N = g.h, qn = N >> 2;
    const bool lean = hdr_light == 2;
    const bool poison = (hdr_flags & (lean ? kPlanNoMegaLean : g.poison_mask)) != 0 || (lean && g.nE > 0 && (!g.edge_index || !g.rev64)) ||
                        hdr_tiles > (int)gridDim.x;
    if (poison) {
        const float nanv = __int_as_float(0x7fc00000);
        const long long total = (long long)g.nV * N;
        for (long long i = (long long)blockIdx.x * KT + tid; i < total; i += (long long)gridDim.x * KT)
            g.out[(i / N) * g.ldout + (i % N)] = nanv;
        return;
    }
    if (na <= 0 || nrows < 0 || va < 0 || vb > g.nV || rs < 0 || re > g.nE) return;
    if (nrows > BM || na > BA) {
        if (NW > 4 && threadIdx.x >= kThreads) return;
        const mega::MegaK& gs = spill::fresh_kernargs<Mega16K>()->m;
        if ((KEEP && gs.drop_thr) || G.atom_de) {
            const float nanv = __int_as_float(0x7fc00000);
            for (int i = tid; i < na * N; i += kThreads) gs.out[(long long)(va + i / N) * gs.ldout + (i % N)] = nanv;
            if constexpr (KEEP) {
                if (gs.Hs)
                    for (int i = tid; i < nrows * N; i += kThreads)
                        for (int sl = 0; sl < gs.depth - 1; ++sl) gs.Hs[(long long)sl * gs.slot + (long long)(rs + i / N) * gs.ldh + (i % N)] = nanv;
            }
            return;
        }
        spill::forward(mega::spill_view(gs, gs.flags[DMPNN_HDR_LIGHT] == 2, rs, nrows, va, na, gs.slope_ptr ? *gs.slope_ptr : gs.slope),
                       reinterpret_cast<float*>(lds));
        if constexpr (KEEP) {
            const Mega16K& Gs = *spill::fresh_kernargs<Mega16K>();
            if (Gs.Mrows && gs.Ms) {
                __threadfence_block();
                __syncthreads();
                for (int sl = 0; sl < gs.depth - 1; ++sl)
                    rows_to_sr(gs.Ms + (long long)sl * gs.slot, gs.ldh, rs, nrows, gs.h, Gs.Mrows + (long long)sl * Gs.mrow_slot, Gs.tsr,
                               (int)(threadIdx.x >> 6), (int)(threadIdx.x & 63), kThreads / 64);
            }
        }
        return;
    }
    const float slope = g.slope_ptr ? *g.slope_ptr : g.slope;
    const float neg_slope = g.act == DMPNN_ACT_NONE ? 1.f : (g.act == DMPNN_ACT_RELU ? 0.f : slope);
    constexpr bool simple_act = SA;

    int revl_v = 0, rp_v = 0, aor_v = 0, asrc_v = 0;
    bool row_bad = false;
    unsigned ro1[JR * RT_E], ro2[JR * RT_E];
    {
        int i1[JR * RT_E], i2[JR * RT_E];
        if (lean && nrows > 0) {
            const int e = rs + (tid < nrows ? tid : 0);
            const long long es = g.edge_index[e], ed = g.edge_index[(long long)g.nE + e], er = g.rev64[e];
            const long long r_l = er - rs, d_l = ed - va, s_l = es - va;
            row_bad = tid < nrows && (r_l < 0 || r_l >= nrows || d_l < 0 || d_l >= na || s_l < 0 || s_l >= na);
            revl_v = (tid < nrows && !row_bad) ? (int)r_l : 0;
            aor_v = (tid < nrows && !row_bad) ? (int)d_l : 0;
            asrc_v = (tid < nrows && !row_bad) ? (int)s_l : 0;
#pragma unroll
            for (int j = 0; j < JR * RT_E; ++j) {
                const int r = wave + NW * j;
                const long long sj = g.edge_index[r < nrows ? rs + r : rs];
                i1[j] = (sj >= 0 && sj < g.nV) ? (int)sj : 0;
                i2[j] = rs + r;
            }
        } else if (lean) {
#pragma unroll
            for (int j = 0; j < JR * RT_E; ++j) { i1[j] = 0; i2[j] = 0; }
        } else {
            revl_v = tid < nrows ? g.revp[rs + tid] - rs : 0;
            rp_v = g.row_ptr[va + (tid <= na ? tid : na)] - rs;
#pragma unroll
            for (int j = 0; j < JR * RT_E; ++j) {
                const int r = wave + NW * j;
                i1[j] = g.srcp[r < nrows ? rs + r : 0];
                i2[j] = g.perm[r < nrows ? rs + r : 0];
            }
        }
#pragma unroll
        for (int j = 0; j < JR * RT_E; ++j) {
            const bool ok = wave + NW * j < nrows;
            ro1[j] = ok ? (unsigned)i1[j] * (unsigned)g.ldv * 4u : kOOB;
            ro2[j] = ok ? (unsigned)i2[j] * (unsigned)g.lde * 4u : kOOB;
        }
    }
    const rsrc_t rVg = gemm::make_rsrc(g.V, g.v_bytes), rEg = gemm::make_rsrc(g.E, g.e_bytes);
    u32x2 a_grp[JR * RT_E];
    {
        const int k = lane * 2;
        const unsigned k1o = k < g.d_v ? (unsigned)k * 4u : kOOB;
        const unsigned k2o = (k >= g.d_v && k < g.d_v + g.d_e) ? (unsigned)(k - g.d_v) * 4u : kOOB;
#pragma unroll
        for (int j = 0; j < JR * RT_E; ++j)
            a_grp[j] = __builtin_amdgcn_raw_buffer_load_b64(rVg, gemm::join_off(ro1[j], k1o), 0, 0) |
                       __builtin_amdgcn_raw_buffer_load_b64(rEg, gemm::join_off(ro2[j], k2o), 0, 0);
    }
    unsigned pf_word[4] = {0u, 0u, 0u, 0u};
#if defined(DMPNN_META_STAMPS)
    stamp();
#endif
    if (tid < BM) { revl[tid] = revl_v; asrc[tid] = asrc_v; if (lean) aor[tid] = aor_v; }
    if (tid <= BA) rp[tid] = rp_v;
    if (tid < 8) maxbits[tid] = 0u;
    __syncthreads();
#if defined(DMPNN_META_STAMPS)
    stamp();
#endif
    if (row_bad) atomicOr(&maxbits[5], 1u);
    if (!lean && tid < na)
        for (int r = rp[tid]; r < rp[tid + 1]; ++r) aor[r] = tid;
    __syncthreads();
#if defined(DMPNN_META_STAMPS)
    stamp();
#endif
    int ar[12];
    {
        const int4 q0 = *reinterpret_cast<const int4*>(aor + lg * 4), q1 = *reinterpret_cast<const int4*>(aor + 16 + lg * 4),
                   q2 = *reinterpret_cast<const int4*>(aor + 32 + lg * 4);
        const int qa[12] = {q0.x, q0.y, q0.z, q0.w, q1.x, q1.y, q1.z, q1.w, q2.x, q2.y, q2.z, q2.w};
#pragma unroll
        for (int i = 0; i < 12; ++i) ar[i] = ((i >> 2) * 16 + lg * 4 + (i & 3)) < nrows ? qa[i] : -2;
    }
    for (int f = wave; f < 10; f += NW) {
        const bool agg = f >= 6;
        const int ff = agg ? f - 6 : f, jt = ff >> 1, ks = ff & 1;
        const int j = jt * 16 + li;
        int a_t = -1, rv = -1;
        if (agg) {
            a_t = j < na ? j : -1;
        } else if (j < nrows) {
            rv = revl[j];
            a_t = lean ? asrc[j] : aor[rv];
        }
        if (G.atom_de) rv = -1;
        unsigned hb[8];
#pragma unroll
        for (int sl = 0; sl < 8; ++sl) {
            const int row = ks == 0 ? (sl < 4 ? lg * 4 + sl : 16 + lg * 4 + (sl - 4)) : (sl < 4 ? 32 + lg * 4 + sl : -2);
            const int av = ks == 0 ? ar[sl] : (sl < 4 ? ar[8 + sl] : -2);
            const bool in = av == a_t, isrev = row == rv;
            hb[sl] = in ? (isrev ? 0u : 0x3C00u) : (isrev ? 0xBC00u : 0u);
        }
        const u32x4 pk = {hb[0] | (hb[1] << 16), hb[2] | (hb[3] << 16), hb[4] | (hb[5] << 16), hb[6] | (hb[7] << 16)};
        cfrag[f * 64 + lane] = __builtin_bit_cast(h8, pk);
    }
    __syncthreads();

    auto wave_max = [&](float v) -> float {
        int u = (int)__float_as_uint(v);
        u = max(u, __builtin_amdgcn_update_dpp(0, u, 0xB1, 0xf, 0xf, true));
        u = max(u, __builtin_amdgcn_update_dpp(0, u, 0x4E, 0xf, 0xf, true));
        u = max(u, __builtin_amdgcn_update_dpp(0, u, 0x141, 0xf, 0xf, true));
        u = max(u, __builtin_amdgcn_update_dpp(0, u, 0x140, 0xf, 0xf, true));
        const int m = max(max(__builtin_amdgcn_readlane(u, 0), __builtin_amdgcn_readlane(u, 16)),
                          max(__builtin_amdgcn_readlane(u, 32), __builtin_amdgcn_readlane(u, 48)));
        return __uint_as_float((unsigned)m);
    };
    int scale_phase = 0;
    float tile_mx = 0.f;
// ... 676 lines not shown
```

### chemprop_amd/csrc/dmpnn_prepare.hip

```cpp
#include <atomic>
#include <limits.h>

#include "dmpnn_common.hpp"
#include "dmpnn_mega16_impl.hpp"

namespace dmpnn {

extern thread_local long long* g_debug_stamps;

namespace {

constexpr int kBlock = 256;

__global__ void k_plan_init(int* __restrict__ plan, int64_t cursor_off, int nV, int nE, int keep_mtiles) {
    const int64_t tid = blockIdx.x * (int64_t)blockDim.x + threadIdx.x;
    if (tid < DMPNN_HDR_WORDS) {
        int v = 0;
        if (tid == DMPNN_HDR_NATOMS) v = nV;
        if (tid == DMPNN_HDR_NEDGES) v = nE;
        if (keep_mtiles) {
            if (tid == DMPNN_HDR_FLAGS) v = plan[tid] & PLAN_NO_PIECE_TILES;
            if (tid == DMPNN_HDR_NMTILES || tid == DMPNN_HDR_NSPILL) v = plan[tid];
        }
        plan[tid] = v;
// ... 773 lines not shown
    S.tag = 0u;
    int64_t o = (L.src + 1) & ~int64_t(1);
    S.aoff = o; o += align4(2 * (nV + 2));
    S.eoff = o; o += align4(2 * (nV + 2));
    S.done = o; o += align4(2 * (int64_t)S.n_bounds);
    S.end = o;
    return S;
}
__device__ __forceinline__ void st_agent(int* p, int v) { __hip_atomic_store(p, v, __ATOMIC_RELAXED, __HIP_MEMORY_SCOPE_AGENT); }
__device__ __forceinline__ int ld_agent(const int* p) { return __hip_atomic_load(p, __ATOMIC_RELAXED, __HIP_MEMORY_SCOPE_AGENT); }
__device__ __forceinline__ void st_tagged(int* base, int m, unsigned tag, int v) {
    __hip_atomic_store(reinterpret_cast<unsigned long long*>(base) + m, ((unsigned long long)tag << 32) | (unsigned)v, __ATOMIC_RELAXED, __HIP_MEMORY_SCOPE_AGENT);
}

__device__ __forceinline__ void tiles_bounds_block(const int64_t* __restrict__ edge_index, const int64_t* __restrict__ batch, int* __restrict__ plan,
                                                   const MultiScratch& S, int nV, int nE, int b) {
    __shared__ int bad_blk;
    if (threadIdx.x == 0) bad_blk = 0;
    __syncthreads();
    const int i = b * kSmallThreads + (int)threadIdx.x;
    const int64_t last = batch[nV - 1];
    const int n_mols = last < 0 ? 0 : (last >= nV ? nV : (int)last + 1);
    int* aoff = plan + S.aoff;
    int* eoff = plan + S.eoff;
    const int64_t* dst = edge_index + nE;
    int bad = 0;
    auto clampm = [&](int64_t m) -> int { return m < 0 ? 0 : (m >= n_mols ? (n_mols > 0 ? n_mols - 1 : 0) : (int)m); };
    const int64_t bm = i < nV ? batch[i] : 0, bp = (i > 0 && i < nV) ? batch[i - 1] : -1;
    int64_t d = (i < nE) ? dst[i] : 0, dp = (i > 0 && i <= nE && nE > 0) ? dst[i - 1] : 0;
    if (i < nE && (d < 0 || d >= nV)) { bad |= PLAN_RANGE_ERROR; d = 0; }
    if (dp < 0 || dp >= nV) dp = 0;
    const int64_t em64 = i < nE ? batch[d] : 0, ep64 = (i > 0 && i <= nE && nE > 0) ? batch[dp] : -1;
    if (i < nV) {
        if (bm < 0 || bm >= nV) bad |= PLAN_RANGE_ERROR;
        if (bm < bp || bm > last) bad |= PLAN_NO_PIECE_TILES;
        const int m = clampm(bm), pm = i > 0 ? clampm(bp) : -1;
        for (int mm = pm + 1; mm <= m; ++mm) st_tagged(aoff, mm, S.tag, i);
    } else if (i == nV) {
        st_tagged(aoff, n_mols, S.tag, nV);
    }
    if (i < nE) {
        if (em64 < ep64) bad |= PLAN_NO_PIECE_TILES;
        const int m = clampm(em64), pm = i > 0 ? clampm(ep64) : -1;
        for (int mm = pm + 1; mm <= m; ++mm) st_tagged(eoff, mm, S.tag, i);
    } else if (i == nE) {
        const int pm = nE > 0 ? clampm(ep64) : -1;
        for (int mm = pm + 1; mm <= n_mols; ++mm) st_tagged(eoff, mm, S.tag, nE);
    }
    if (bad) atomicOr(&bad_blk, bad);
    asm volatile("s_waitcnt vmcnt(0)" ::: "memory");
    __syncthreads();
    if (threadIdx.x == 0)
        __hip_atomic_store(reinterpret_cast<unsigned long long*>(plan + S.done) + b, ((unsigned long long)S.tag << 32) | (unsigned)bad_blk,
                           __ATOMIC_RELAXED, __HIP_MEMORY_SCOPE_AGENT);
}

__device__ __forceinline__ void tiles_pack_block(int* lds_i, const int64_t* __restrict__ batch, int* __restrict__ plan, const PlanLayout& L,
                                                 const MultiScratch& S, int nV, int nE, long long* dbg, int* __restrict__ mol_bounds, int n_mols_out) {
    int n_stamp = 0;
    auto stamp = [&]() {
        if (dbg && threadIdx.x == 0 && n_stamp < 16) dbg[n_stamp] = (long long)__builtin_readcyclecounter();
        ++n_stamp;
    };
    stamp();
    int* fa = lds_i;
    int* fe = fa + nV + 2;
    int* Y = fe + nV + 2;
    __shared__ int bad_s, flags_s, spill_s;
    const int tid = threadIdx.x;
    if (tid == 0) { bad_s = 0; flags_s = 0; spill_s = 0; }
    const int64_t last = batch[nV - 1];
    const int nm = last < 0 ? 0 : (last >= nV ? nV : (int)last + 1);
    __syncthreads();
    unsigned long long* done = reinterpret_cast<unsigned long long*>(plan + S.done);
    {
        unsigned long long* a64 = reinterpret_cast<unsigned long long*>(plan + S.aoff);
        unsigned long long* e64 = reinterpret_cast<unsigned long long*>(plan + S.eoff);
        for (int m = tid; m <= nm; m += kSmallThreads) {
            unsigned long long wa = 0ull, we = 0ull;
            int spins = 0;
            for (;;) {
                wa = __hip_atomic_load(a64 + m, __ATOMIC_RELAXED, __HIP_MEMORY_SCOPE_AGENT);
                we = __hip_atomic_load(e64 + m, __ATOMIC_RELAXED, __HIP_MEMORY_SCOPE_AGENT);
                if (((unsigned)(wa >> 32) == S.tag && (unsigned)(we >> 32) == S.tag) || ++spins >= kBoundsMaxSpins) break;
                __builtin_amdgcn_s_sleep(2);
            }
            const bool ok = (unsigned)(wa >> 32) == S.tag && (unsigned)(we >> 32) == S.tag;
            if (!ok) atomicOr(&flags_s, PLAN_NO_PIECE_TILES);
            fa[m] = ok ? (int)(unsigned)wa : 0;
            fe[m] = ok ? (int)(unsigned)we : 0;
            __hip_atomic_store(a64 + m, 0ull, __ATOMIC_RELAXED, __HIP_MEMORY_SCOPE_AGENT);
            __hip_atomic_store(e64 + m, 0ull, __ATOMIC_RELAXED, __HIP_MEMORY_SCOPE_AGENT);
        }
    }
    __syncthreads();
    stamp();
    __syncthreads();
    stamp();
    {
        int bad = 0;
        for (int m = tid; m <= nm; m += kSmallThreads) {
            const int a = fa[m], e = fe[m];
            if (a < 0 || a > nV || e < 0 || e > nE) bad = 1;
            if (m > 0 && (fa[m - 1] > a || fe[m - 1] > e)) bad = 1;
        }
        if (bad) atomicOr(&flags_s, PLAN_NO_PIECE_TILES);
    }
    __syncthreads();
    if ((flags_s & (PLAN_NO_PIECE_TILES | PLAN_RANGE_ERROR)) && tid == 0) bad_s = 1;
    __syncthreads();
    stamp();
    unsigned long long w_early = 0ull;
    if (tid < S.n_bounds) w_early = __hip_atomic_load(done + tid, __ATOMIC_RELAXED, __HIP_MEMORY_SCOPE_AGENT);
    tiles_batch_finish(fa, fe, Y, nm, &bad_s, &flags_s, &spill_s, plan, L, nV, nE, dbg, n_stamp, mol_bounds, n_mols_out);
    __shared__ int late_s;
    if (tid == 0) late_s = 0;
    __syncthreads();
    if (tid < S.n_bounds) {
        unsigned long long w = w_early;
        int spins = 0;
        while ((unsigned)(w >> 32) != S.tag && ++spins < kBoundsMaxSpins) {
            __builtin_amdgcn_s_sleep(8);
            w = __hip_atomic_load(done + tid, __ATOMIC_RELAXED, __HIP_MEMORY_SCOPE_AGENT);
        }
        if ((unsigned)(w >> 32) != S.tag) atomicOr(&late_s, PLAN_NO_PIECE_TILES);
        else if ((unsigned)w) atomicOr(&late_s, (int)((unsigned)w & (PLAN_NO_PIECE_TILES | PLAN_RANGE_ERROR)));
        __hip_atomic_store(done + tid, 0ull, __ATOMIC_RELAXED, __HIP_MEMORY_SCOPE_AGENT);
    }
    __syncthreads();
    if (tid == 0 && (late_s & ~flags_s)) {
        plan[DMPNN_HDR_FLAGS] |= late_s & (PLAN_NO_PIECE_TILES | PLAN_RANGE_ERROR);
        if (late_s & PLAN_NO_PIECE_TILES) { plan[DMPNN_HDR_NMTILES] = 0; plan[DMPNN_HDR_NSPILL] = 0; }
        if (mol_bounds) mol_bounds[2 * n_mols_out] |= ((late_s & PLAN_RANGE_ERROR) ? 1 : 0) | ((late_s & PLAN_NO_PIECE_TILES) ? 2 : 0);
    }
}

__global__ __launch_bounds__(kSmallThreads) void k_prepare_tiles_batch_multi(const int64_t* __restrict__ edge_index, const int64_t* __restrict__ batch,
                                                                            int* __restrict__ plan, PlanLayout L, MultiScratch S, int nV, int nE,
                                                                            long long* dbg, int* __restrict__ mol_bounds, int n_mols_out,
                                                                            mega16::SplitArgs sp) {
    extern __shared__ __attribute__((aligned(16))) int lds_i[];
    const int b = (int)blockIdx.x;
    if (b < S.n_bounds) tiles_bounds_block(edge_index, batch, plan, S, nV, nE, b);
    else if (b + 1 < (int)gridDim.x) mega16::split_weights_wave(sp, (b - S.n_bounds) * (kSmallThreads / 64) + (int)(threadIdx.x >> 6), (int)(threadIdx.x & 63));
    else tiles_pack_block(lds_i, batch, plan, L, S, nV, nE, dbg, mol_bounds, n_mols_out);
}

__global__ __launch_bounds__(256) void k_tiles_from_table_split(const int* __restrict__ tile_row, const int* __restrict__ tile_atom, int n_tiles,
                                                                int nV, int nE, int* __restrict__ plan, PlanLayout L, mega16::SplitArgs sp) {
    if (blockIdx.x == 0) tiles_from_table_body(tile_row, tile_atom, n_tiles, nV, nE, plan, L);
    else mega16::split_weights_wave(sp, ((int)blockIdx.x - 1) * 4 + (int)(threadIdx.x >> 6), (int)(threadIdx.x & 63));
}

}

int launch_tiles_from_table_split(const int* tile_row, const int* tile_atom, int64_t n_tiles, int64_t nV, int64_t nE, int* plan, hipStream_t s,
                                  const dmpnn_fwd_args* split_for, bool* did_split) {
    *did_split = false;
    mega16::SplitArgs sp;
    if (!split_for || !(split_for->flags & DMPNN_F_MEGA) || !(split_for->flags & DMPNN_F_SPLIT16) || (split_for->flags & DMPNN_F_WSPLIT_READY) ||
        !mega16_split_args(*split_for, &sp))
        return DMPNN_OK;
    const PlanLayout L = plan_layout(nV, nE);
    const int waves = ((sp.N + 15) & ~15) * sp.n_jobs;
    hipLaunchKernelGGL(k_tiles_from_table_split, dim3((unsigned)(1 + (waves + 3) / 4)), dim3(256), 0, s, tile_row, tile_atom, (int)n_tiles, (int)nV,
                       (int)nE, plan, L, sp);
    DMPNN_CHECK_LAUNCH("k_tiles_from_table_split");
    *did_split = true;
    return DMPNN_OK;
}

static size_t tiles_batch_lds_bytes(int64_t nV, int64_t nE) {
    return ((size_t)(3 * (nV + 2)) * 4 + (size_t)(nV + 1 + nE + 2) * 2 + 31) & ~size_t(15);
}

int launch_prepare_tiles_batch(const int64_t* edge_index, const int64_t* batch, int64_t nV64, int64_t nE64, int* plan, hipStream_t s,
                               int* mol_bounds, int64_t n_mols, const dmpnn_fwd_args* split_for, bool* did_split) {
    const int nV = (int)nV64, nE = (int)nE64;
    const PlanLayout L = plan_layout(nV, nE);
    if (did_split) *did_split = false;
    mega16::SplitArgs sp;
    {
        const char* k0e = getenv("DMPNN_K0_SINGLE");
        const bool multi_off = k0e && atoi(k0e) != 0;
        MultiScratch S = multi_scratch(L, nV, nE);
        static std::atomic<unsigned> launch_no{0u};
        S.tag = kBoundsTag ^ (launch_no.fetch_add(1u, std::memory_order_relaxed) * 0x9E3779B1u);
        if (S.tag == 0u) S.tag = kBoundsTag;
        if (!multi_off && nV > 0 && S.end <= L.tile_row) {
            const bool split = split_for && did_split && (split_for->flags & DMPNN_F_MEGA) && (split_for->flags & DMPNN_F_SPLIT16) &&
                               !(split_for->flags & DMPNN_F_WSPLIT_READY) && mega16_split_args(*split_for, &sp);
            if (!split) memset(&sp, 0, sizeof(sp));
            static bool attr3_set = false;
            if (!attr3_set) {
                hipError_t e = hipFuncSetAttribute(reinterpret_cast<const void*>(&k_prepare_tiles_batch_multi),
                                                   hipFuncAttributeMaxDynamicSharedMemorySize, 160 * 1024 - 2048);
                if (e != hipSuccess) {
                    set_error("hipFuncSetAttribute(k_prepare_tiles_batch_multi): %s", hipGetErrorString(e));
                    return DMPNN_EHIP;
                }
                attr3_set = true;
            }
            const int waves = split ? ((sp.N + 15) & ~15) * sp.n_jobs : 0, wpb = kSmallThreads / 64;
            const size_t lds = ((size_t)(3 * (nV + 2)) * 4 + 31) & ~size_t(15);
            hipLaunchKernelGGL(k_prepare_tiles_batch_multi, dim3((unsigned)(S.n_bounds + (waves + wpb - 1) / wpb + 1)), dim3(kSmallThreads), lds, s,
                               edge_index, batch, plan, L, S, nV, nE, g_debug_stamps ? g_debug_stamps + 32 : nullptr, mol_bounds, (int)n_mols, sp);
            DMPNN_CHECK_LAUNCH("k_prepare_tiles_batch_multi");
            if (split) *did_split = true;
            return DMPNN_OK;
        }
    }
    if (split_for && did_split && (split_for->flags & DMPNN_F_MEGA) && (split_for->flags & DMPNN_F_SPLIT16) && !(split_for->flags & DMPNN_F_WSPLIT_READY) &&
        mega16_split_args(*split_for, &sp)) {
        static bool attr2_set = false;
        if (!attr2_set) {
            hipError_t e = hipFuncSetAttribute(reinterpret_cast<const void*>(&k_prepare_tiles_batch_split),
                                               hipFuncAttributeMaxDynamicSharedMemorySize, 160 * 1024 - 2048);
            if (e != hipSuccess) {
                set_error("hipFuncSetAttribute(k_prepare_tiles_batch_split): %s", hipGetErrorString(e));
                return DMPNN_EHIP;
            }
            attr2_set = true;
        }
        const int waves = ((sp.N + 15) & ~15) * sp.n_jobs, wpb = kSmallThreads / 64;
        hipLaunchKernelGGL(k_prepare_tiles_batch_split, dim3((unsigned)(1 + (waves + wpb - 1) / wpb)), dim3(kSmallThreads), tiles_batch_lds_bytes(nV, nE), s,
                           edge_index, batch, plan, L, nV, nE, g_debug_stamps ? g_debug_stamps + 32 : nullptr, mol_bounds, (int)n_mols, sp);
        DMPNN_CHECK_LAUNCH("k_prepare_tiles_batch_split");
        *did_split = true;
        return DMPNN_OK;
    }
    static bool attr_set = false;
    if (!attr_set) {
        hipError_t e = hipFuncSetAttribute(reinterpret_cast<const void*>(&k_prepare_tiles_batch),
                                           hipFuncAttributeMaxDynamicSharedMemorySize, 160 * 1024 - 2048);
        if (e != hipSuccess) {
            set_error("hipFuncSetAttribute(k_prepare_tiles_batch): %s", hipGetErrorString(e));
            return DMPNN_EHIP;
        }
        attr_set = true;
    }
    hipLaunchKernelGGL(k_prepare_tiles_batch, dim3(1), dim3(kSmallThreads), tiles_batch_lds_bytes(nV, nE), s, edge_index, batch, plan,
                       L, nV, nE, g_debug_stamps ? g_debug_stamps + 32 : nullptr, mol_bounds, (int)n_mols);
    DMPNN_CHECK_LAUNCH("k_prepare_tiles_batch");
    return DMPNN_OK;
}

bool prepare_can_keep_mtiles(int64_t nV, int64_t nE) {
    const PlanLayout L = plan_layout(nV, nE);
    return (nV + kScanThreads * kScanItems - 1) / (kScanThreads * kScanItems) <= L.max_tiles + 2;
}

int launch_prepare(const int64_t* edge_index, const int64_t* rev, int64_t nV64, int64_t nE64,
                   int* plan, int light, hipStream_t s, bool keep_mtiles) {
    const int nV = (int)nV64, nE = (int)nE64;
    const PlanLayout L = plan_layout(nV, nE);
    if (small_plan_fits(nV, nE)) {
        const size_t lds = small_plan_lds_bytes(nV, nE);
        static bool attr_set = false;
        if (!attr_set) {
            hipError_t e = hipFuncSetAttribute(reinterpret_cast<const void*>(&k_prepare_small),
                                               hipFuncAttributeMaxDynamicSharedMemorySize, 160 * 1024 - 2048);
            if (e != hipSuccess) {
                set_error("hipFuncSetAttribute(k_prepare_small): %s", hipGetErrorString(e));
                return DMPNN_EHIP;
            }
            attr_set = true;
        }
        hipLaunchKernelGGL(k_prepare_small, dim3(1), dim3(kSmallThreads), lds, s, edge_index, rev, plan, L, nV, nE, light,
                           g_debug_stamps ? g_debug_stamps + 32 : nullptr);
        DMPNN_CHECK_LAUNCH("k_prepare_small");
        return DMPNN_OK;
    }
    {
        const int64_t n = nV > DMPNN_HDR_WORDS ? nV : DMPNN_HDR_WORDS;
        int grid = (int)((n + kBlock - 1) / kBlock);
        if (grid > 2048) grid = 2048;
        hipLaunchKernelGGL(k_plan_init, dim3(grid), dim3(kBlock), 0, s, plan, L.cursor, nV, nE, keep_mtiles ? 1 : 0);
        DMPNN_CHECK_LAUNCH("k_plan_init");
    }
    if (nE > 0) {
        const int grid = (nE + kBlock - 1) / kBlock;
        hipLaunchKernelGGL(k_convert_count, dim3(grid), dim3(kBlock), 0, s, edge_index, rev, plan, L, nV, nE);
        DMPNN_CHECK_LAUNCH("k_convert_count");
    }
    {
        const int nblk = nV > 0 ? (nV + kScanThreads * kScanItems - 1) / (kScanThreads * kScanItems) : 1;
        int* part = plan + (keep_mtiles ? L.tile_row : L.mtile_row);
        if (nblk > 1) {
            hipLaunchKernelGGL(k_scan_totals, dim3(nblk), dim3(kScanThreads), 0, s, plan, L, nV, part);
            DMPNN_CHECK_LAUNCH("k_scan_totals");
        }
        hipLaunchKernelGGL(k_scan, dim3(nblk), dim3(kScanThreads), 0, s, plan, L, nV, part);
        DMPNN_CHECK_LAUNCH("k_scan");
    }
    if (nE > 0) {
        const int grid = (nE + kBlock - 1) / kBlock;
        hipLaunchKernelGGL(k_fill, dim3(grid), dim3(kBlock), 0, s, plan, L, nE);
        DMPNN_CHECK_LAUNCH("k_fill");
        const int gridv = (nV + kBlock - 1) / kBlock;
        hipLaunchKernelGGL(k_sort_rows, dim3(gridv), dim3(kBlock), 0, s, plan, L, nV);
        DMPNN_CHECK_LAUNCH("k_sort_rows");
        hipLaunchKernelGGL(k_inverse, dim3(grid), dim3(kBlock), 0, s, plan, L, nE);
        DMPNN_CHECK_LAUNCH("k_inverse");
    }
    {
        const int64_t n = nV > nE ? nV : nE;
// ... 11 lines not shown
```

### chemprop_amd/data.py

```python
from __future__ import annotations

from typing import NamedTuple, Sequence

import numpy as np
import torch
from torch import Tensor


class MolGraph(NamedTuple):

    V: np.ndarray
    E: np.ndarray
    edge_index: np.ndarray
    rev_edge_index: np.ndarray


TILE_MAX_ATOMS, TILE_MAX_EDGES = 32, 48


def molecules_oversize(n_atoms, n_edges) -> bool:
    n_atoms, n_edges = np.asarray(n_atoms), np.asarray(n_edges)
    return bool(n_atoms.size and (int(n_atoms.max()) > TILE_MAX_ATOMS or int(n_edges.max()) > TILE_MAX_EDGES))


class BatchMolGraph:

    __slots__ = ("V", "E", "edge_index", "rev_edge_index", "batch", "_size", "tiles", "oversize")

    def __init__(self, mgs: Sequence[MolGraph]):
        self._size = len(mgs)
        self.tiles = None
        n_atoms = np.fromiter((len(mg.V) for mg in mgs), dtype=np.int64, count=len(mgs))
        n_edges = np.fromiter((mg.edge_index.shape[1] for mg in mgs), dtype=np.int64, count=len(mgs))
        self.oversize = molecules_oversize(n_atoms, n_edges)
        atom_off = np.concatenate([[0], np.cumsum(n_atoms)[:-1]]) if len(mgs) else np.zeros(0, np.int64)
        edge_off = np.concatenate([[0], np.cumsum(n_edges)[:-1]]) if len(mgs) else np.zeros(0, np.int64)

        self.V = torch.from_numpy(np.concatenate([mg.V for mg in mgs])).float()
        self.E = torch.from_numpy(np.concatenate([mg.E for mg in mgs])).float()
        ei = np.hstack([mg.edge_index + o for mg, o in zip(mgs, atom_off)])
        self.edge_index = torch.from_numpy(ei).long()
        rev = np.concatenate([mg.rev_edge_index + o for mg, o in zip(mgs, edge_off)])
        self.rev_edge_index = torch.from_numpy(rev).long()
        self.batch = torch.from_numpy(np.repeat(np.arange(len(mgs), dtype=np.int64), n_atoms))

    def __len__(self) -> int:
        return self._size

    def to(self, device) -> None:
        self.V = self.V.to(device)
        self.E = self.E.to(device)
        self.edge_index = self.edge_index.to(device)
        self.rev_edge_index = self.rev_edge_index.to(device)
        self.batch = self.batch.to(device)
        self.tiles = None

    @classmethod
    def from_tensors(cls, V: Tensor, E: Tensor, edge_index: Tensor, rev_edge_index: Tensor,
                     batch: Tensor, size: int | None = None) -> "BatchMolGraph":
        self = object.__new__(cls)
        self.V, self.E = V, E
        self.edge_index, self.rev_edge_index, self.batch = edge_index, rev_edge_index, batch
        self._size = int(size) if size is not None else (int(batch[-1]) + 1 if batch.numel() else 0)
        self.tiles = None
        self.oversize = None
        return self

    def __copy__(self):
        b = BatchMolGraph.from_tensors(self.V, self.E, self.edge_index, self.rev_edge_index, self.batch, self._size)
        b.tiles = self.tiles
        b.oversize = self.oversize
        return b


_WIRE_MAGIC = 0x31424D44
_WIRE_HEADER = 8


def _align16(n: int) -> int:
    return (n + 15) // 16 * 16


class PackedBatch:

    __slots__ = ("buf", "n_mols", "n_atoms", "n_edges", "n_erows", "d_v", "d_e", "sections", "n_tiles", "oversize")

    def __init__(self, mgs: Sequence[MolGraph], pin: bool = False, tiles: bool = True):
        n_mols = len(mgs)
        n_at = np.fromiter((len(mg.V) for mg in mgs), dtype=np.int64, count=n_mols)
        n_ed = np.fromiter((mg.edge_index.shape[1] for mg in mgs), dtype=np.int64, count=n_mols)
        nV, nE = int(n_at.sum()), int(n_ed.sum())
        nEr = int(sum(len(mg.E) for mg in mgs))
        if nV >= 2 ** 31 or nE >= 2 ** 31:
            raise ValueError("PackedBatch: more than 2^31 atoms or edges in one batch")
        d_v = int(mgs[0].V.shape[1]) if n_mols else 0
        d_e = int(mgs[0].E.shape[1]) if n_mols else 0
        atom_off = np.zeros(n_mols + 1, dtype=np.int32)
        edge_off = np.zeros(n_mols + 1, dtype=np.int32)
        atom_off[1:] = np.cumsum(n_at)
        edge_off[1:] = np.cumsum(n_ed)
        n_tiles, trow, tatom = -1, None, None
        self.oversize = molecules_oversize(n_at, n_ed)
        if tiles and n_mols and nV and not self.oversize:
            from . import _lib

            lib = _lib.load()
            cap = int(lib.dmpnn_max_tiles(nV, nE)) + 1
            trow, tatom = np.empty(cap, dtype=np.int32), np.empty(cap, dtype=np.int32)
            n_tiles = int(lib.dmpnn_pack_tiles(atom_off.ctypes.data, edge_off.ctypes.data, n_mols, trow.ctypes.data,
                                               tatom.ctypes.data, cap))
            if n_tiles < 0:
                n_tiles = -1
        nt = n_tiles + 1 if n_tiles >= 0 else 0
        sec, o = {}, _WIRE_HEADER * 8
        for name, nbytes in (("atom_off", 4 * (n_mols + 1)), ("edge_off", 4 * (n_mols + 1)), ("src", 4 * nE), ("dst", 4 * nE),
                             ("rev", 4 * nE), ("V", 4 * nV * d_v), ("E", 4 * nEr * d_e), ("tile_row", 4 * nt), ("tile_atom", 4 * nt)):
            sec[name] = (o, nbytes)
            o = _align16(o + nbytes)
        if pin:
            buf = torch.empty(o, dtype=torch.uint8).pin_memory()
            raw = buf.numpy()
            raw[:] = 0
        else:
            raw = np.zeros(o, dtype=np.uint8)
            buf = torch.from_numpy(raw)
        view = lambda name, dt: raw[sec[name][0]:sec[name][0] + sec[name][1]].view(dt)
        raw[:_WIRE_HEADER * 8].view(np.int64)[:8] = (_WIRE_MAGIC, n_mols, nV, nE, d_v, d_e, n_tiles, nEr)
        view("atom_off", np.int32)[:] = atom_off
        view("edge_off", np.int32)[:] = edge_off
        if nt:
            view("tile_row", np.int32)[:] = trow[:nt]
            view("tile_atom", np.int32)[:] = tatom[:nt]
        if n_mols:
            if nE:
                view("src", np.int32)[:] = np.concatenate([mg.edge_index[0] for mg in mgs])
                view("dst", np.int32)[:] = np.concatenate([mg.edge_index[1] for mg in mgs])
                view("rev", np.int32)[:] = np.concatenate([mg.rev_edge_index for mg in mgs])
            if nEr and d_e:
                view("E", np.float32).reshape(nEr, d_e)[:] = np.concatenate([mg.E for mg in mgs])
            if nV and d_v:
                view("V", np.float32).reshape(nV, d_v)[:] = np.concatenate([mg.V for mg in mgs])
        self.buf, self.sections = buf, sec
        self.n_mols, self.n_atoms, self.n_edges, self.d_v, self.d_e = n_mols, nV, nE, d_v, d_e
        self.n_tiles, self.n_erows = n_tiles, nEr

    def __len__(self) -> int:
        return self.n_mols

    def pin_memory(self) -> "PackedBatch":
        self.buf = self.buf.pin_memory()
        return self

    def to_device(self, device) -> "BatchMolGraph":
        from . import _lib, engine

        device = torch.device(device)
        if device.type != "cuda":
            raise RuntimeError("PackedBatch.to_device: batching runs in a HIP kernel; use BatchMolGraph(mgs) on the host")
        dbuf = self.buf.to(device, non_blocking=True)
        nV, nE = self.n_atoms, self.n_edges
        sl = lambda name: dbuf[self.sections[name][0]:self.sections[name][0] + self.sections[name][1]]
        V = sl("V").view(torch.float32).view(nV, self.d_v)
        E = sl("E").view(torch.float32).view(self.n_erows, self.d_e)
        edge_index = torch.empty(2, nE, dtype=torch.int64, device=device)
        rev = torch.empty(nE, dtype=torch.int64, device=device)
        batch = torch.empty(nV, dtype=torch.int64, device=device)
        base = dbuf.data_ptr()
        at = lambda name: base + self.sections[name][0]
        with engine._OnDevice(device):
            _lib.check(_lib.load().dmpnn_collate(at("atom_off"), at("edge_off"), self.n_mols, at("src"), at("dst"), at("rev"),
                                                 nV, nE, edge_index.data_ptr(), rev.data_ptr(), batch.data_ptr(),
                                                 engine._stream_ptr(device)), "dmpnn_collate")
        bmg = BatchMolGraph.from_tensors(V, E, edge_index, rev, batch, self.n_mols)
        bmg.oversize = self.oversize
        if self.n_tiles >= 0:
            bmg.tiles = (sl("tile_row").view(torch.int32), sl("tile_atom").view(torch.int32), self.n_tiles)
        return bmg


def merge_components(bmgs: Sequence["BatchMolGraph"]) -> "BatchMolGraph":
    bmgs = list(bmgs)
    if not bmgs:
        raise ValueError("merge_components: no components")
    B = len(bmgs[0])
    if any(len(b) != B for b in bmgs):
        raise ValueError(f"merge_components: every component must hold the same number of molecules, got {[len(b) for b in bmgs]}")
    if any(b.V.shape[1:] != bmgs[0].V.shape[1:] or b.E.shape[1:] != bmgs[0].E.shape[1:] for b in bmgs):
        raise ValueError("merge_components: components of one shared block must have the same atom / bond feature widths")
    ei, rev, bt = [], [], []
    a_off = e_off = 0
    for c, b in enumerate(bmgs):
        ei.append(b.edge_index + a_off)
        rev.append(b.rev_edge_index + e_off)
        bt.append(b.batch + c * B)
        a_off += int(b.V.shape[0])
        e_off += int(b.E.shape[0])
    m = BatchMolGraph.from_tensors(torch.cat([b.V for b in bmgs]), torch.cat([b.E for b in bmgs]), torch.cat(ei, dim=1),
                                   torch.cat(rev), torch.cat(bt).contiguous(), len(bmgs) * B)
    ov = [getattr(b, "oversize", None) for b in bmgs]
    m.oversize = True if any(o is True for o in ov) else (False if all(o is False for o in ov) else None)
    return m
```

### chemprop_amd/engine.py

```python
from __future__ import annotations

import ctypes as C
import os
from typing import Optional

import torch
from torch import Tensor

from . import _lib
from ._lib import (ACT, F_FUSED, F_H0_RESIDUAL, F_KEEP, F_LOADER_TILES, F_MEGA, F_ROW_FINALIZE, F_SPLIT16, F_STORE16, F_TILE_PLAN, F_UNDIRECTED, F_WSPLIT_READY,
                   PLAN_NOFUSE_MASK, PLAN_NOMEGA_MASK, FwdArgs, GemmArgs)


STEPS16_MIN_EDGES = 20000
FUSED16_MIN_EDGES = 2048


def small_plan_fits(n_atoms: int, n_edges: int) -> bool:
    lds = ((3 * (n_atoms + 2)) * 4 + (5 * n_edges + 2) * 2 + 31) & ~15
    return n_atoms <= 6144 and n_edges <= 10240 and lds <= 160 * 1024 - 2048


_raw_stream = getattr(torch._C, "_cuda_getCurrentRawStream", None)


_plan_bytes_cache: dict = {}


def plan_bytes(n_atoms: int, n_edges: int) -> int:
    k = (n_atoms, n_edges)
    v = _plan_bytes_cache.get(k)
    if v is None:
        if len(_plan_bytes_cache) > 4096:
            _plan_bytes_cache.clear()
        v = _plan_bytes_cache[k] = int(_lib.load().dmpnn_plan_bytes(n_atoms, n_edges))
    return v


def _stream_ptr(device) -> int:
    if _raw_stream is not None:
        idx = device.index
        return _raw_stream(torch.cuda.current_device() if idx is None else idx)
    return torch.cuda.current_stream(device).cuda_stream


class _OnDevice:

    __slots__ = ("ctx",)

    def __init__(self, dev):
        idx = dev.index
        self.ctx = None if (idx is None or idx == torch.cuda.current_device()) else torch.cuda.device(dev)

    def __enter__(self):
        if self.ctx is not None:
            self.ctx.__enter__()

    def __exit__(self, *a):
        if self.ctx is not None:
            self.ctx.__exit__(*a)


def _require_device(t: Tensor, name: str) -> None:
    if t.device.type != "cuda":
        raise RuntimeError(
            f"chemprop_amd: `{name}` lives on {t.device}; the MI355X engine runs HIP kernels only "
            "(no CPU fallback) — move the batch and the module to a GPU device first")


def _f32c(t: Tensor, name: str) -> Tensor:
    _require_device(t, name)
    if t.dtype != torch.float32:
        t = t.float()
    if t.dim() == 2 and t.stride(1) == 1 and t.stride(0) >= t.shape[1]:
        return t
    if t.dim() == 2 and t.shape[0] <= 1:
        return torch.empty(t.shape, dtype=t.dtype, device=t.device).copy_(t)
    return t.contiguous()


def _ptr(t: Optional[Tensor]) -> Optional[int]:
    return None if t is None else t.data_ptr()


class GraphPlan:

    __slots__ = ("buf", "n_atoms", "n_edges", "device", "light", "tiles_only", "edge_index", "rev_edge_index", "loader_tiles",
                 "any_size", "oversize", "pending", "_job")

    def __init__(self, edge_index: Tensor, rev_edge_index: Tensor, n_atoms: int, light=False, batch: Optional[Tensor] = None,
                 tiles: Optional[tuple] = None, launch: bool = True):
        _require_device(edge_index, "edge_index")
        lib = _lib.load()
        dev = edge_index.device
        n_edges = int(edge_index.shape[1])
        ei = edge_index if edge_index.dtype == torch.int64 else edge_index.long()
        ei = ei.contiguous()
        rev = rev_edge_index if rev_edge_index.dtype == torch.int64 else rev_edge_index.long()
        rev = rev.contiguous()
        nbytes = plan_bytes(n_atoms, n_edges)
        self.buf = torch.empty(nbytes // 4, dtype=torch.int32, device=dev)
        self.n_atoms, self.n_edges, self.device = int(n_atoms), n_edges, dev
        self.oversize = None
        small = small_plan_fits(n_atoms, n_edges)
        self.loader_tiles = 0
        if light == "tiles" and tiles is not None:
            tr, ta, nt = tiles
            if (tr.dtype == torch.int32 and ta.dtype == torch.int32 and tr.device == dev and ta.device == dev
                    and tr.is_contiguous() and ta.is_contiguous() and tr.numel() > nt and ta.numel() > nt and nt > 0):
                self.loader_tiles = int(nt)
        bt = batch if (batch is not None and batch.dtype == torch.int64 and batch.device == dev
                       and batch.numel() == n_atoms and batch.is_contiguous()) else None
        big = (light == "tiles" and not small and not self.loader_tiles and bt is not None and n_atoms > 0
               and bool(lib.dmpnn_tile_plan_any_size(n_atoms, n_edges)))
        self.tiles_only = light == "tiles" and (small or self.loader_tiles > 0 or big)
        self.light = bool(light) and (small or self.loader_tiles > 0 or big)
        full_tiles = (not light and not small and bt is not None and n_atoms > 0 and n_edges > 0
                      and bool(lib.dmpnn_full_plan_keeps_tiles(n_atoms, n_edges)))
        self.any_size = (self.tiles_only and not small) or full_tiles
        self.edge_index, self.rev_edge_index = ei, rev
        self.pending, self._job = None, None
        if launch == "defer":
            if self.tiles_only and small and not self.loader_tiles and bt is not None:
                self.pending = bt
                self._job = (tiles, bt, full_tiles, nbytes)
                return
            launch = True
        if not launch:
            if light and not self.tiles_only:
                raise RuntimeError("GraphPlan(launch=False) is the plan of a training step: full, or the tile plan (light='tiles')")
            self.loader_tiles = 0
            return
        self._job = (tiles, bt, full_tiles, nbytes)
        self._launch()

    def ensure_launched(self) -> None:
        if self.pending is not None:
            self.pending = None
            self._launch()

    def _launch(self) -> None:
        lib = _lib.load()
        tiles, bt, full_tiles, nbytes = self._job
        self._job = None
        dev, ei, rev, n_atoms, n_edges = self.device, self.edge_index, self.rev_edge_index, self.n_atoms, self.n_edges
        with _OnDevice(dev):
            if self.loader_tiles:
                _lib.check(lib.dmpnn_prepare_tiles_from_table(tiles[0].data_ptr(), tiles[1].data_ptr(), self.loader_tiles, n_atoms,
                                                              n_edges, self.buf.data_ptr(), nbytes, _stream_ptr(dev)),
                           "dmpnn_prepare_tiles_from_table")
            elif self.tiles_only:
                _lib.check(lib.dmpnn_prepare_tiles(ei.data_ptr(), rev.data_ptr(), bt.data_ptr() if bt is not None else None,
                                                   n_atoms, n_edges, self.buf.data_ptr(), nbytes, _stream_ptr(dev)),
                           "dmpnn_prepare_tiles")
            elif full_tiles:
                _lib.check(lib.dmpnn_prepare_with_batch(ei.data_ptr(), rev.data_ptr(), bt.data_ptr(), n_atoms, n_edges,
                                                        self.buf.data_ptr(), nbytes, _stream_ptr(dev)), "dmpnn_prepare_with_batch")
            else:
                prep = lib.dmpnn_prepare_light if self.light else lib.dmpnn_prepare
                _lib.check(prep(ei.data_ptr(), rev.data_ptr(), n_atoms, n_edges,
                                self.buf.data_ptr(), nbytes, _stream_ptr(dev)), "dmpnn_prepare")

    @classmethod
    def from_bmg(cls, bmg, light=False, use_batch: bool = True, launch=True) -> "GraphPlan":
        return cls(bmg.edge_index, bmg.rev_edge_index, int(bmg.V.shape[0]), light=light,
                   batch=getattr(bmg, "batch", None) if use_batch else None,
                   tiles=getattr(bmg, "tiles", None) if light == "tiles" else None, launch=launch)

    def arrays(self) -> dict:
        self.ensure_launched()
        off = self._offsets()
        b = self.buf.cpu()
        E, V, T = self.n_edges, self.n_atoms, int(off[11])
        cut = lambda o, n: b[o:o + n]
        return dict(hdr=b[:16], src=cut(off[0], E), dst=cut(off[1], E), rev=cut(off[2], E),
                    row_ptr=cut(off[3], V + 1), perm=cut(off[4], E), inv=cut(off[5], E), srcp=cut(off[6], E),
                    dstp=cut(off[7], E), revp=cut(off[8], E), tile_row=cut(off[9], T + 2),
                    tile_atom=cut(off[10], T + 2), mtile_row=cut(off[12], int(off[14]) + 2),
                    mtile_atom=cut(off[13], int(off[14]) + 2))

    def header(self) -> list:
        self.ensure_launched()
        return self.buf[:16].tolist()

    def flags(self) -> int:
        self.ensure_launched()
        return int(self.buf[0].item())

    def fusable(self) -> bool:
        return (self.flags() & PLAN_NOFUSE_MASK) == 0

    def mega_ok(self) -> bool:
        return (self.flags() & PLAN_NOMEGA_MASK) == 0

    def _offsets(self):
        off = (C.c_int64 * _lib.PLAN_NOFFSETS)()
        _lib.check(_lib.load().dmpnn_plan_layout(self.n_atoms, self.n_edges, off), "dmpnn_plan_layout")
        return off

    def _view(self, k: int) -> Tensor:
        self.ensure_launched()
        off = self._offsets()
        return self.buf[off[k]:off[k] + self.n_edges]

    @property
    def src32(self) -> Tensor:
        return self._view(0)

    @property
    def dst32(self) -> Tensor:
        return self._view(1)

    @property
    def rev32(self) -> Tensor:
        return self._view(2)

    @property
    def rev64(self) -> Tensor:
        return self._view(2).long()

    @property
    def inv32(self) -> Tensor:
        return self._view(5)

    @property
    def perm32(self) -> Tensor:
        return self._view(4)

    @property
    def perm64(self) -> Tensor:
        return self._view(4).long()


def fuse16_shapes(a) -> bool:
    flags = a.flags
    a.flags = flags & ~_lib.F_KEEP
    try:
        return bool(_lib.load().dmpnn_forward_can_fuse16(C.byref(a)))
    finally:
        a.flags = flags


def _lean16_bits(lib, a) -> int:
    flags = a.flags
    a.flags = (flags | F_FUSED | F_SPLIT16 | F_KEEP) & ~F_MEGA
    try:
        return int(lib.dmpnn_forward_keep_bits_bytes(C.byref(a)))
    finally:
        a.flags = flags


def lean_sign_bits(st: "ForwardState") -> Tensor:
    if not st.route.startswith("fused16/lean"):
        raise RuntimeError("lean_sign_bits: not a lean forward of the per-step fused route")
    bits = st.refs[16]
    d_h, depth = st.dims["d_h"], int(st.args.depth)
    bn = (d_h + 63) // 64 * 64
    b = bits.view(depth, st.plan.n_edges, bn // 8)
    sh = torch.arange(8, device=b.device, dtype=torch.uint8)
    return ((b.unsqueeze(-1) >> sh) & 1).bool().reshape(depth, st.plan.n_edges, bn)[:, :, :d_h]


def lean_dropout_refusal(d_v: int, d_e: int, d_h: int, depth: int, act: str, has_vd: bool = False) -> Optional[str]:
    if act not in ("relu", "leakyrelu"):
        return f"activation {act!r} (relu / leakyrelu: the mask rides on a sign bit)"
    if has_vd:
        return "a W_d layer (d_vd > 0)"
    if depth < 2:
        return "depth 1 (no update step)"
    if depth > 8:
        return f"depth {depth} > 8 (the weight-gradient launch holds 8 product jobs per matrix)"
    if d_h > 320:
        return f"d_h {d_h} > 320"
    if d_h % 4:
# ... 245 lines not shown
        if light and (not use_fused or (keep and not (tiles_only and use_mega and not d_vd))):
            raise RuntimeError("forward: a light GraphPlan only serves inference forwards of the fused routes "
                               "(build the plan with light=False for the general route or for training; the tile plan also "
                               "serves a training forward of the tile kernel without W_d)")
        if tiles_only and (not use_mega or mf == "f32"):
            raise RuntimeError("forward: a tile plan (light='tiles') only serves the whole-forward tile kernel on the f16 pipe")
        want16 = use_mega or use_fused16 or (not use_fused and (mfma == "split16" or (mfma is None and mf == "split16" and (d_h > 320 or nE >= STEPS16_MIN_EDGES))))
        if mf == "f32":
            want16 = False

    if atom:
        if not (use_mega and want16 and not d_vd and 1 <= d_e <= 16 and (not keep or (d_e % 2 == 0 and d_v % 2 == 0 and d_h % 2 == 0))):
            raise RouteUnavailable("atom messages inside the kernels: the tile kernel, 1 <= d_e <= 16, no W_d (training: even d_v / d_e / d_h)")
        a.flags |= _lib.F_ATOM
    if dropout is not None and float(dropout[0]) > 0.0:
        tile_home = bool(use_mega and want16 and keep and not d_vd and act in ("relu", "leakyrelu"))
        lean_home = bool(route == "fused16" and use_fused16 and keep and keep_bits and not d_vd and act in ("relu", "leakyrelu"))
        if tile_home or lean_home:
            a.dropout_p, a.dropout_seed = float(dropout[0]), int(dropout[1]) & 0xFFFFFFFFFFFFFFFF
        if not tile_home and not (lean_home and _lean16_bits(lib, a) > 0):
            why = lean_dropout_refusal(d_v, d_e, d_h, depth, act, bool(d_vd)) if route == "fused16" else None
            raise RouteUnavailable("dropout inside the kernels: a training forward of the tile kernel, or the lean training forward of the "
                                   "per-step fused route (route='fused16', keep, keep_bits); ReLU-class activation, no W_d"
                                   + (f" — the lean step kernels refuse: {why}" if why else ""))
    bits = None
    lean16 = False
    st = ForwardState()
    st.fused = use_fused
    st.route = "mega" if use_mega else ("fused16" if use_fused16 else ("fused" if use_fused else "general"))
    if use_mega:
        n_hslots = n_steps if keep else 0
        n_mslots = n_steps if keep else 0
    elif use_fused:
        n_hslots = n_steps if keep else 0
        n_mslots = n_steps if keep else min(n_steps, 2)
    else:
        n_hslots = max(n_steps, 1) if keep else 1
        n_mslots = max(n_steps, 1) if keep else 1
    st.plan, st.ldh, st.n_hslots, st.n_mslots = plan, ldh, n_hslots, n_mslots
    need_h0 = not (use_mega and not keep)
    spill_ws = None
    if use_mega and not keep and getattr(plan, "oversize", None) is not False and nV:
        spill_ws = torch.empty((3 * nE + nV) * ldh, dtype=torch.float32, device=dev)
        a.spill_ws, a.spill_bytes = spill_ws.data_ptr(), spill_ws.numel() * 4
    split_ms = None
    if use_mega and not keep and not d_vd:
        edge_ws = atom_ws = None
    elif use_fused16 and keep and keep_bits and _lean16_bits(lib, a) > 0:
        srf = int(lib.dmpnn_split_row_floats(d_h))
        lean16 = True
        n_hslots = n_mslots = 0
        xrow = ((d_v + d_e + 31) // 32 * 128 + 16) // 4
        edge_ws = torch.empty((1, nE, max(ldh, xrow)), dtype=torch.float32, device=dev)
        split_ms = torch.empty((max(n_steps, 1), nE, srf), dtype=torch.float32, device=dev)
        atom_ws = torch.empty((2, nV, ldh), dtype=torch.float32, device=dev)
        bits = torch.empty(_lean16_bits(lib, a), dtype=torch.uint8, device=dev)
    elif use_fused16 and keep:
        srf = int(lib.dmpnn_split_row_floats(d_h))
        n_hslots = n_mslots = n_steps
        edge_ws = torch.empty((1 + 2 * n_steps, nE, ldh), dtype=torch.float32, device=dev)
        split_ms = torch.empty((2, nE, srf), dtype=torch.float32, device=dev)
        atom_ws = torch.empty((2, nV, ldh), dtype=torch.float32, device=dev)
    elif use_fused16:
        srf = int(lib.dmpnn_split_row_floats(d_h))
        h0_rows = nE
        if _lib.opt("DMPNN_H0", "quads") != "x":
            flags = a.flags
            a.flags = (flags | F_FUSED | F_SPLIT16) & ~(F_MEGA | F_KEEP)
            try:
                need = int(lib.dmpnn_forward_h0_bytes(C.byref(a)))
            finally:
                a.flags = flags
            if need:
                h0_rows = max(nE, (need // 4 + ldh - 1) // ldh)
                a.h0_bytes = h0_rows * ldh * 4
        edge_ws = torch.empty((1, h0_rows, ldh), dtype=torch.float32, device=dev)
        split_ms = torch.empty((2, nE, srf), dtype=torch.float32, device=dev)
        atom_ws = torch.empty((2, nV, ldh), dtype=torch.float32, device=dev)
        n_hslots, n_mslots = 0, 2
    else:
        edge_ws = torch.empty(((1 if need_h0 else 0) + n_hslots + n_mslots, nE, ldh), dtype=torch.float32, device=dev)
        atom_ws = torch.empty((2, nV, ldh), dtype=torch.float32, device=dev)
        if atom and keep:
            split_ms = torch.empty((max(n_steps, 1), nE, 16), dtype=torch.float32, device=dev)
        elif use_mega and want16 and keep and n_steps and train_route(nV, nE, d_v, d_e, d_h, depth, act, 1, max_level=2).keep_rows:
            split_ms = torch.empty((n_steps, nE, int(lib.dmpnn_split_row_floats(d_h))), dtype=torch.float32, device=dev)
    st.out = out
    if edge_ws is None:
        st.H0 = st.Hs = st.Ms = st.Mv = st.Hv = None
        a.H0 = a.Hs = a.Ms = None
        a.n_hslots, a.n_mslots = 0, 1
        a.Mv = a.Hv = plan.buf.data_ptr()
    else:
        if ldh != d_h:
            edge_ws.zero_()
            atom_ws.zero_()
        i0 = 1 if need_h0 else 0
        st.H0, st.Hs, st.Ms = (edge_ws[0] if need_h0 else None), edge_ws[i0:i0 + n_hslots], edge_ws[i0 + n_hslots:]
        st.Mv, st.Hv = atom_ws[0], atom_ws[1]
        a.H0 = st.H0.data_ptr() if need_h0 else None
        a.Hs, a.n_hslots = (st.Hs.data_ptr() if n_hslots else None), n_hslots
        a.Ms, a.n_mslots = (st.Ms.data_ptr() if n_mslots else None), max(n_mslots, 1)
        a.Mv, a.Hv = st.Mv.data_ptr(), st.Hv.data_ptr()
        if lean16:
            a.msplit, a.msplit_bytes = split_ms.data_ptr(), split_ms.numel() * 4
            a.keep_bits, a.keep_bits_bytes = bits.data_ptr(), bits.numel()
            a.Hs = a.Ms = None
            st.Ms = split_ms
        elif split_ms is not None and keep:
            a.msplit, a.msplit_bytes = split_ms.data_ptr(), split_ms.numel() * 4
        elif split_ms is not None:
            st.Ms = split_ms
            a.Ms, a.n_mslots = split_ms.data_ptr(), 2
    if use_fused:
        a.flags |= F_FUSED
    wsplit = None
    if want16:
        if use_mega:
            a.flags |= F_MEGA
        a.flags |= F_SPLIT16
        if keep:
            a.flags |= F_KEEP
        nb = int(lib.dmpnn_forward_wsplit_bytes(C.byref(a)))
        wsplit = wcache.get("buf") if (wcache is not None and not keep) else None
        if wsplit is None or wsplit.numel() != nb or wsplit.device != dev:
            wsplit = torch.empty(nb, dtype=torch.uint8, device=dev)
            if wcache is not None and not keep:
                wcache["buf"] = wsplit
        a.wsplit, a.wsplit_bytes = wsplit.data_ptr(), nb
        st.route = "mega16" if use_mega else (("fused16/lean" if lean16 else "fused16") if use_fused16 else "general16")
        if use_fused16 and storage_f16() and not keep:
            a.flags |= F_STORE16
            st.route = "fused16/f16-storage"
        elif use_mega and storage_f16() and not keep and not atom:
            a.flags |= F_STORE16
            st.route = "mega16/f16-operands"
    elif use_mega:
        a.flags |= F_MEGA
    if keep:
        a.flags |= F_KEEP
        if tiles_only:
            if not (use_mega and want16 and not d_vd):
                raise RuntimeError("forward: a tile plan serves a training forward only on the tile kernel (f16 pipe), without W_d")
            a.flags |= F_TILE_PLAN
            nbits = int(lib.dmpnn_forward_keep_bits_bytes(C.byref(a))) if keep_bits else 0
            if nbits:
                bits = torch.empty(nbits, dtype=torch.uint8, device=dev)
                a.keep_bits, a.keep_bits_bytes = bits.data_ptr(), nbits
    if launch:
        pend = getattr(plan, "pending", None)
        with _OnDevice(dev):
            if pend is not None and use_mega and want16 and tiles_only:
                plan.pending = None
                _lib.check(lib.dmpnn_forward_tiles(C.byref(a), pend.data_ptr(), None, None, 0, plan.buf.numel() * 4, _stream_ptr(dev)), "dmpnn_forward_tiles")
            else:
                if pend is not None:
                    plan.ensure_launched()
                _lib.check(lib.dmpnn_forward(C.byref(a), _stream_ptr(dev)), "dmpnn_forward")
    st.args = a
    st.refs = (V, E, V_d, W_i, W_h, W_o, b_o, b_i, b_h, W_d, b_d, slope_t, edge_ws, atom_ws, spill_ws, split_ms, bits, wsplit)
    st.dims = dict(d_v=d_v, d_e=d_e, d_h=d_h, d_vd=d_vd, has_bi=b_i is not None, has_bh=b_h is not None, atom=bool(atom))
    return out, st


def backward(st: ForwardState, gout: Tensor, need: dict, out: Optional[dict] = None, launch: bool = True, g_edge: Optional[Tensor] = None):
    from ._lib import BwdArgs

    lib = _lib.load()
    gout = _f32c(gout, "grad_output")
    dev = gout.device
    d = st.dims
    h, dv, de, dvd = d["d_h"], d["d_v"], d["d_e"], d["d_vd"]
    atom = bool(d.get("atom"))
    shapes = dict(W_i=(h, dv if atom else dv + de), b_i=(h,), W_h=(h, h + de if atom else h), b_h=(h,), W_o=(h, dv + h), b_o=(h,),
                  W_d=(h + dvd, h + dvd), b_d=(h + dvd,))
    present = dict(W_i=True, b_i=d["has_bi"], W_h=True, b_h=d["has_bh"], W_o=True, b_o=True, W_d=dvd > 0, b_d=dvd > 0)
    def _buf(k):
        t = out.get(k) if out else None
        if (t is not None and t.dtype == torch.float32 and t.device == dev and tuple(t.shape) == shapes[k] and t.is_contiguous()):
            return t
        return torch.empty(shapes[k], dtype=torch.float32, device=dev)

    grads = {k: (_buf(k) if (need.get(k) and present[k]) else None) for k in shapes}
    b = BwdArgs()
    b.f = st.args
    b.gout, b.ldgout = gout.data_ptr(), gout.stride(0)
    for k, g in grads.items():
        setattr(b, "g" + k, _ptr(g))
    nbytes = lib.dmpnn_backward_ws_bytes(C.byref(st.args))
    ws = torch.empty(max(nbytes // 4, 1), dtype=torch.float32, device=dev)
    b.ws, b.ws_bytes = ws.data_ptr(), nbytes
    if g_edge is not None:
        g_edge = _f32c(g_edge, "g_edge").contiguous()
        if g_edge.shape[0] != st.args.n_edges or g_edge.shape[1] < h or g_edge.stride(0) % 4:
            raise RuntimeError("backward: g_edge must be [n_edges, d_h] with a row stride that is a multiple of 4")
        b.g_edge, b.ld_gedge = g_edge.data_ptr(), g_edge.stride(0)
    if not launch:
        return grads, b, (ws, gout)
    with _OnDevice(dev):
        _lib.check(lib.dmpnn_backward(C.byref(b), _stream_ptr(dev)), "dmpnn_backward")
    return grads


def message_bwd(plan: GraphPlan, gM: Tensor) -> Tensor:
    gM = _f32c(gM, "gM")
    gH = torch.empty_like(gM)
    with _OnDevice(gM.device):
        _lib.check(_lib.load().dmpnn_message_bwd(plan.buf.data_ptr(), plan.n_atoms, plan.n_edges, gM.shape[1],
                                                 gM.data_ptr(), gM.stride(0), gH.data_ptr(), gH.stride(0),
                                                 _stream_ptr(gM.device)), "dmpnn_message_bwd")
    return gH


def aggregate_bwd(plan: GraphPlan, gMv: Tensor) -> Tensor:
    gMv = _f32c(gMv, "gMv")
    gH = torch.empty(plan.n_edges, gMv.shape[1], dtype=torch.float32, device=gMv.device)
    with _OnDevice(gMv.device):
        _lib.check(_lib.load().dmpnn_aggregate_bwd(plan.buf.data_ptr(), plan.n_atoms, plan.n_edges, gMv.shape[1],
                                                   gMv.data_ptr(), gMv.stride(0), gH.data_ptr(), gH.stride(0),
                                                   _stream_ptr(gMv.device)), "dmpnn_aggregate_bwd")
    return gH


def linear_wgrad(gZ: Tensor, A1: Tensor, A2: Optional[Tensor] = None, gather1: Optional[Tensor] = None,
                 want_bias: bool = False) -> tuple[Tensor, Optional[Tensor]]:
    gZ = _f32c(gZ, "gZ")
    A1 = _f32c(A1, "A1")
    if A2 is not None:
        A2 = _f32c(A2, "A2")
    lib = _lib.load()
    M, N = int(gZ.shape[0]), int(gZ.shape[1])
    K1, K2 = int(A1.shape[1]), (int(A2.shape[1]) if A2 is not None else 0)
    g = GemmArgs()
    g.M, g.N, g.K1, g.K2 = M, N, K1, K2
    g.A1, g.lda1, g.gather1 = A1.data_ptr(), A1.stride(0), _ptr(gather1)
    g.gather1_rows = int(A1.shape[0])
    g.A2, g.lda2 = _ptr(A2), (A2.stride(0) if A2 is not None else 0)
    gW = torch.empty(N, K1 + K2, dtype=torch.float32, device=gZ.device)
    gb = torch.empty(N, dtype=torch.float32, device=gZ.device) if want_bias else None
    nbytes = lib.dmpnn_linear_wgrad_ws_bytes(M, N, K1 + K2, 1 if want_bias else 0)
    ws = torch.empty(max(nbytes // 4, 1), dtype=torch.float32, device=gZ.device)
    with _OnDevice(gZ.device):
        _lib.check(lib.dmpnn_linear_wgrad(C.byref(g), gZ.data_ptr(), gZ.stride(0), gW.data_ptr(), gW.stride(0),
                                          _ptr(gb), ws.data_ptr(), nbytes, _stream_ptr(gZ.device)), "dmpnn_linear_wgrad")
    return gW, gb
```

### chemprop_amd/nn.py

```python
from __future__ import annotations

import copy
import ctypes as _ctypes
import os
from typing import Optional

import torch
from torch import Tensor, nn

from . import _lib, engine
from .autograd import mp_forward
from .data import BatchMolGraph as _OwnBatch

DEFAULT_ATOM_FDIM, DEFAULT_BOND_FDIM = 72, 14
DEFAULT_HIDDEN_DIM = 300


class InvalidShapeError(ValueError):

    def __init__(self, var_name, received, expected):
        super().__init__(f"arg '{var_name}' has incorrect shape! got: `{tuple(received)}`. "
                         f"expected: `{tuple(expected)}`")


# ... 25 lines not shown


class _HParams(dict):
    def __getattr__(self, k):
        try:
            return self[k]
        except KeyError as e:
            raise AttributeError(k) from e


_CACHE_KEYS = ("_dmpnn_replay", "_dmpnn_wcache", "_dmpnn_last", "_dmpnn_mon")
_STATE_SKIP_KEYS = _CACHE_KEYS + ("_dmpnn_grad_views", "_dmpnn_grad_written")


def invalidate(module: nn.Module) -> None:
    for m in module.modules():
        for k in _CACHE_KEYS:
            m.__dict__.pop(k, None)


class EngineStateMixin:

    def __getstate__(self):
        return {k: v for k, v in self.__dict__.items() if k not in _STATE_SKIP_KEYS}

    def _apply(self, fn, *args, **kwargs):
        for k in _CACHE_KEYS:
            self.__dict__.pop(k, None)
        return super()._apply(fn, *args, **kwargs)


class BondMessagePassing(EngineStateMixin, nn.Module):

    def __init__(self, d_v: int = DEFAULT_ATOM_FDIM, d_e: int = DEFAULT_BOND_FDIM,
                 d_h: int = DEFAULT_HIDDEN_DIM, bias: bool = False, depth: int = 3, dropout: float = 0.0,
                 activation="relu", undirected: bool = False, d_vd: Optional[int] = None,
                 V_d_transform: Optional[nn.Module] = None, graph_transform: Optional[nn.Module] = None):
        super().__init__()
        self.hparams = _HParams(d_v=d_v, d_e=d_e, d_h=d_h, bias=bias, depth=depth, dropout=dropout,
                                activation=activation, undirected=undirected, d_vd=d_vd,
                                V_d_transform=V_d_transform, graph_transform=graph_transform,
                                cls=self.__class__)
        self.W_i = nn.Linear(d_v + d_e, d_h, bias)
        self.W_h = nn.Linear(d_h, d_h, bias)
        self.W_o = nn.Linear(d_v + d_h, d_h)
        self.W_d = nn.Linear(d_h + d_vd, d_h + d_vd) if d_vd else None
        self.depth = depth
        self.undirected = undirected
        self.dropout = nn.Dropout(dropout)
        self.tau = get_activation_function(activation)
        self.V_d_transform = V_d_transform if V_d_transform is not None else nn.Identity()
        self.graph_transform = graph_transform if graph_transform is not None else nn.Identity()

    @property
    def output_dim(self) -> int:
        return self.W_d.out_features if self.W_d is not None else self.W_o.out_features

    def forward(self, bmg, V_d: Optional[Tensor] = None) -> Tensor:
        return bond_message_passing_forward(self, bmg, V_d)


def _training_plan_kind(mp, bmg, atom: bool = False, vd_outside: bool = False):
    if _lib.opt("DMPNN_GENERAL", "0") == "1" or _lib.opt("DMPNN_TRAIN_PLAN", "tiles") == "full":
        return False
    act = classify_activation(mp.tau)[0]
    if act == "custom" or (mp.training and mp.dropout.p > 0 and type(mp.dropout) is not nn.Dropout):
        return False
    mode = _lib.opt("DMPNN_VALIDATE", "first")
    if mode == "always" or (mode != "never" and getattr(mp, "_dmpnn_batches_checked", 0) < _VALIDATE_FIRST_N):
        return False
    if not (mp.W_i.weight.requires_grad or mp.W_h.weight.requires_grad):
        return False
    d_h, d_in = mp.W_h.weight.shape[0], mp.W_i.weight.shape[1]
    d_v = mp.W_o.weight.shape[1] - d_h
    d_e = int(bmg.E.shape[1]) if atom else d_in - d_v
    batch = getattr(bmg, "batch", None)
    info = engine.train_route(int(bmg.V.shape[0]), int(bmg.E.shape[0]), d_v, d_e, d_h, mp.depth, act,
                              len(bmg) if hasattr(bmg, "__len__") else 0, undirected=bool(mp.undirected), has_vd=mp.W_d is not None and not vd_outside,
                              dropout_p=float(mp.dropout.p) if mp.training else 0.0, atom=atom,
                              have_batch=batch is not None and batch.dtype == torch.int64 and batch.is_contiguous(),
                              have_table=getattr(bmg, "tiles", None) is not None, oversize=getattr(bmg, "oversize", None),
                              max_level=1 if getattr(mp, "_dmpnn_no_mega", False) else 2)
    return "tiles" if info.plan_kind == 2 else False


_ENV_KEYS = ("DMPNN_GENERAL", "DMPNN_MEGA", "DMPNN_MFMA", "DMPNN_VALIDATE", "DMPNN_STORE")


class _Replay:

    __slots__ = ("args", "tensors", "ptrs", "tau", "training", "env", "dev", "d_v", "d_e", "d_h", "wsplit", "depth", "block", "flags",
                 "ldh", "spill")


def _param(mp, lin: str, name: str):
    m = mp._modules.get(lin)
    return None if m is None else m._parameters.get(name)


def _make_replay(mp, plan, st) -> None:
    mp.__dict__.pop("_dmpnn_replay", None)
    if st is None or st.route not in ("mega16", "mega16/f16-operands") or not plan.tiles_only or mp.W_d is not None:
        return
    r = _Replay()
    r.args = bytes(st.args)
    r.tensors = tuple(_param(mp, l, n) for l, n in (("W_i", "weight"), ("W_h", "weight"), ("W_o", "weight"), ("W_i", "bias"),
                                                      ("W_h", "bias"), ("W_o", "bias")))
    r.ptrs = tuple(0 if t is None else t.data_ptr() for t in r.tensors)
    r.tau, r.training, r.depth = mp._modules.get("tau"), mp.training, mp.depth
    r.env = tuple(_lib.opt(k, "") for k in _ENV_KEYS)
    r.dev = plan.device
    r.d_v, r.d_e, r.d_h = st.dims["d_v"], st.dims["d_e"], st.dims["d_h"]
    r.wsplit = st.refs[-1]
    if r.wsplit is None or any(t is not None and (t.dtype != torch.float32 or not t.is_contiguous()) for t in r.tensors):
        return
    blk = r.block = _lib.FwdArgs.from_buffer_copy(r.args)
    blk.ldv, blk.lde, blk.ldout = r.d_v, r.d_e, r.d_h
    r.flags = int(blk.flags) & ~_lib.F_WSPLIT_READY & ~_lib.F_LOADER_TILES
    r.ldh, r.spill = int(blk.ldh), None
    mp.__dict__["_dmpnn_replay"] = r


def _replay_forward(mp, r: "_Replay", bmg):
    mods = mp._modules
    if (mp.training != r.training or mods.get("tau") is not r.tau or mp.depth != r.depth or mp.undirected
            or type(mods.get("graph_transform")) is not nn.Identity or mods.get("W_d") is not None):
        return None
    ts = r.tensors
    if (_param(mp, "W_i", "weight") is not ts[0] or _param(mp, "W_h", "weight") is not ts[1] or _param(mp, "W_o", "weight") is not ts[2]
            or _param(mp, "W_i", "bias") is not ts[3] or _param(mp, "W_h", "bias") is not ts[4] or _param(mp, "W_o", "bias") is not ts[5]):
        return None
    for t, ptr in zip(ts, r.ptrs):
        if t is not None and (t.data_ptr() != ptr or t.device != r.dev):
            return None
    if tuple(_lib.opt(k, "") for k in _ENV_KEYS) != r.env:
        return None
    V, E, ei, rev, batch = bmg.V, bmg.E, bmg.edge_index, bmg.rev_edge_index, getattr(bmg, "batch", None)
    dev = r.dev
    if V.device != dev or batch is None or V.dim() != 2 or E.dim() != 2 or V.shape[1] != r.d_v or E.shape[1] != r.d_e:
        return None
    if (type(bmg) is not _OwnBatch or bmg.oversize is None) and (
            V.dtype != torch.float32 or E.dtype != torch.float32 or not V.is_contiguous() or not E.is_contiguous() or ei.dtype != torch.int64
            or rev.dtype != torch.int64 or not ei.is_contiguous() or not rev.is_contiguous() or ei.device != dev
            or batch.dtype != torch.int64 or not batch.is_contiguous() or batch.device != dev):
        return None
    nV, nE = V.shape[0], E.shape[0]
    n_mols = len(bmg) if hasattr(bmg, "__len__") else 0
    oversize = getattr(bmg, "oversize", None)
    if oversize is True:
        return None
    tiles = getattr(bmg, "tiles", None)
    if tiles is not None and (tiles[0].device != dev or tiles[2] <= 0):
        tiles = None
    small = engine.small_plan_fits(nV, nE)
    lib = _lib.load()
    if (n_mols <= 0 or nE > 30 * n_mols or nE == 0 or (tiles is None and not small and not lib.dmpnn_tile_plan_any_size(nV, nE))
            or batch.numel() != nV
            or ei.shape[1] != nE or rev.numel() != nE or getattr(mp, "_dmpnn_no_mega", False)):
        return None
    nbytes = engine.plan_bytes(nV, nE)
    buf = torch.empty(nbytes // 4, dtype=torch.int32, device=dev)
    out = torch.empty(nV, r.d_h, dtype=torch.float32, device=dev)
    a = r.block
    pb = buf.data_ptr()
    a.plan, a.n_atoms, a.n_edges = pb, nV, nE
    a.V, a.E = V.data_ptr(), E.data_ptr()
    a.out = out.data_ptr()
    a.Mv = a.Hv = pb
    a.edge_index, a.rev_edge_index = ei.data_ptr(), rev.data_ptr()
    if oversize is None:
        need = (3 * nE + nV) * r.ldh
        sp = r.spill
        if sp is None or sp.numel() < need:
            sp = r.spill = torch.empty(need + need // 4, dtype=torch.float32, device=dev)
        a.spill_ws, a.spill_bytes = sp.data_ptr(), need * 4
    else:
        a.spill_ws, a.spill_bytes = None, 0
    cur = torch.cuda.current_device()
    ctx = None if dev.index is None or dev.index == cur else torch.cuda.device(dev)
    if ctx is not None:
        ctx.__enter__()
    try:
        stream = engine._raw_stream(dev.index if dev.index is not None else cur) if engine._raw_stream is not None else engine._stream_ptr(dev)
        if tiles is not None:
            a.flags = r.flags | _lib.F_LOADER_TILES
            a.n_tiles_launch = tiles[2]
            rc = lib.dmpnn_forward_tiles(_ctypes.byref(a), None, tiles[0].data_ptr(), tiles[1].data_ptr(), tiles[2], nbytes, stream)
        else:
            a.flags = r.flags if small else (r.flags | _lib.F_LOADER_TILES)
            a.n_tiles_launch = n_mols
            rc = lib.dmpnn_forward_tiles(_ctypes.byref(a), batch.data_ptr(), None, None, 0, nbytes, stream)
    finally:
        if ctx is not None:
            ctx.__exit__(None, None, None)
    if rc:
        _lib.check(rc, "dmpnn_forward_tiles")
    if oversize is None:
        _spill_monitor(mp, buf, dev)
    from .agg import note_batch

    note_batch(batch, n_mols)
    return out


class _Monitor:
    __slots__ = ("host", "event", "pending", "calls", "observed", "with_spill")


def _spill_monitor(mp, plan_buf: Tensor, dev) -> None:
    if torch.cuda.is_current_stream_capturing():
        return
    m = mp.__dict__.get("_dmpnn_mon")
    if m is None:
        m = _Monitor()
        m.host = torch.zeros(16, dtype=torch.int32).pin_memory()
        m.event = torch.cuda.Event()
        m.pending, m.calls, m.observed, m.with_spill = False, 0, 0, 0
        mp.__dict__["_dmpnn_mon"] = m
    if m.pending and m.event.query():
        m.pending = False
        _note_spills(mp, m, int(m.host[8]))
    m.calls += 1
    if not m.pending and (m.calls % 8 == 0 if m.calls <= 64 else m.calls % 64 == 0) and not torch.cuda.is_current_stream_capturing():
        m.host.copy_(plan_buf[:16], non_blocking=True)
        m.event.record(torch.cuda.current_stream(dev))
        m.pending = True


def _note_spills(mp, m, n_spill: int) -> None:
    m.observed += 1
    if n_spill > 0:
        m.with_spill += 1
    if m.with_spill >= 2 and 4 * m.with_spill >= m.observed:
        object.__setattr__(mp, "_dmpnn_no_mega", True)


def bond_message_passing_forward(mp, bmg, V_d: Optional[Tensor] = None) -> Tensor:
    if torch.compiler.is_compiling() or torch.compiler.is_exporting():
        from .export import traced_forward

        return traced_forward(mp, bmg, V_d)
    if V_d is None and not torch.is_grad_enabled():
        r = mp.__dict__.get("_dmpnn_replay")
        if r is not None:
            out = _replay_forward(mp, r, bmg)
            if out is not None:
                return out
    bmg = mp.graph_transform(bmg)
    engine._require_device(bmg.V, "bmg.V")
    if mp.W_i.weight.device != bmg.V.device:
        raise RuntimeError(f"module is on {mp.W_i.weight.device} but the batch is on {bmg.V.device}")
    n_atoms = int(bmg.V.shape[0])
    if V_d is not None:
        V_d = mp.V_d_transform(V_d)
        d_vd = (mp.W_d.in_features - mp.W_o.out_features) if mp.W_d is not None else None
        if mp.W_d is None or V_d.dim() != 2 or V_d.shape[0] != n_atoms or V_d.shape[1] != d_vd:
            raise InvalidShapeError("V_d", V_d.shape, [n_atoms, d_vd if d_vd is not None else 0])
    n_mols = len(bmg) if hasattr(bmg, "__len__") else 0
    loader_tiles = getattr(bmg, "tiles", None) is not None or (
        getattr(bmg, "batch", None) is not None and not engine.small_plan_fits(int(bmg.V.shape[0]), int(bmg.E.shape[0]))
        and bool(_lib.load().dmpnn_tile_plan_any_size(int(bmg.V.shape[0]), int(bmg.E.shape[0]))))
    oversize = getattr(bmg, "oversize", None)
    if oversize is None and mp.training and mp.dropout.p > 0 and torch.is_grad_enabled():
        oversize = batch_oversize(bmg, n_mols)
    if oversize is True:
        loader_tiles = False
    light = _light_plan_ok(mp)
    if light and oversize is not True and _tile_plan_ok(mp, int(bmg.V.shape[0]), int(bmg.E.shape[0]), n_mols, loader_tiles):
        light = "tiles"
    if not light and torch.is_grad_enabled() and V_d is None:
        light = _training_plan_kind(mp, bmg) if oversize is not True else False
    plan = engine.GraphPlan.from_bmg(bmg, light=light, launch="defer" if light == "tiles" else True)
    if n_mols and getattr(bmg, "batch", None) is not None:
        from .agg import note_batch

        note_batch(bmg.batch, n_mols)
    mp.__dict__.pop("_dmpnn_last", None)
    plan.oversize = oversize
    level = _route(mp, plan, n_mols, getattr(bmg, "batch", None))
    if oversize is True:
        level = min(level, 1)
    out = mp_forward(mp, plan, bmg.V, bmg.E, V_d, max_level=level)
    last = mp.__dict__.pop("_dmpnn_last", None)
    mp.__dict__["_dmpnn_route"] = getattr(last, "route", None)
    plan.ensure_launched()
    if oversize is None and plan.tiles_only and last is not None and last.route in ("mega16", "mega16/f16-operands"):
        _spill_monitor(mp, plan.buf, plan.device)
    if light == "tiles" and V_d is None and not torch.is_grad_enabled() and _lib.opt("DMPNN_REPLAY", "1") != "0":
        _make_replay(mp, plan, last)
    return out


_VALIDATE_FIRST_N = 2


def batch_oversize(bmg, n_mols: int = 0):
    o = getattr(bmg, "oversize", None)
    if o is not None:
        return bool(o)
    batch = getattr(bmg, "batch", None)
    if batch is None or batch.dtype != torch.int64 or batch.numel() != int(bmg.V.shape[0]):
        return None
    from .data import TILE_MAX_ATOMS, TILE_MAX_EDGES

    if batch.numel() == 0:
        return False
    n_mols = int(n_mols) if n_mols else 0
    na = torch.bincount(batch, minlength=n_mols)
    bad = na.max() > TILE_MAX_ATOMS
    if int(bmg.E.shape[0]) > 0:
        ne = torch.bincount(batch[bmg.edge_index[1]], minlength=n_mols)
        bad = bad | (ne.max() > TILE_MAX_EDGES)
    return bool(bad.item())


def _light_plan_ok(mp) -> bool:
    if torch.is_grad_enabled() and any(p.requires_grad for p in mp.parameters()):
        return False
    if mp.undirected or (mp.training and mp.dropout.p > 0) or classify_activation(mp.tau)[0] == "custom":
        return False
    if _lib.opt("DMPNN_GENERAL", "0") == "1":
        return False
    if _lib.opt("DMPNN_VALIDATE", "first") != "never" and getattr(mp, "_dmpnn_batches_checked", 0) < _VALIDATE_FIRST_N:
        return False
    d_h, d_in = mp.W_h.weight.shape[0], mp.W_i.weight.shape[1]
    d_v = mp.W_o.weight.shape[1] - d_h
    return d_h % 4 == 0 and d_h <= 320 and d_v % 2 == 0 and (d_in - d_v) % 2 == 0


def _tile_plan_ok(mp, n_atoms: int, n_edges: int, n_mols: int, loader_tiles: bool = False) -> bool:
    if _lib.opt("DMPNN_MEGA", "1") == "0" or _lib.opt("DMPNN_MFMA", "split16") == "f32":
        return False
    if getattr(mp, "_dmpnn_no_mega", False):
        return False
    if _lib.opt("DMPNN_VALIDATE", "first") == "always":
        return False
    return n_mols > 0 and n_edges <= 30 * n_mols and (loader_tiles or engine.small_plan_fits(n_atoms, n_edges))


def _route(mp, plan, n_mols: int = 0, batch=None) -> int:
    mode = _lib.opt("DMPNN_VALIDATE", "first")
    seen = getattr(mp, "_dmpnn_batches_checked", 0)
    no_mega = getattr(mp, "_dmpnn_no_mega", False)
    if n_mols > 0 and plan.n_edges > 30 * n_mols:
        no_mega = True
    if mode == "always" or (mode == "first" and seen < _VALIDATE_FIRST_N):
        object.__setattr__(mp, "_dmpnn_batches_checked", seen + 1)
        hdr = plan.header()
        flags = hdr[0]
        if flags & 7:
            return 0
        if hdr[8] > 0 and getattr(plan, "oversize", None) is None:
            no_mega = True
            object.__setattr__(mp, "_dmpnn_no_mega", True)
        if flags & 8:
            if engine.small_plan_fits(plan.n_atoms, plan.n_edges) or (getattr(plan, "any_size", False) and not plan.tiles_only):
                object.__setattr__(mp, "_dmpnn_no_mega", True)
            elif batch is not None and not no_mega and _lib.load().dmpnn_tile_plan_any_size(plan.n_atoms, plan.n_edges):
                tp = engine.GraphPlan(plan.edge_index, plan.rev_edge_index, plan.n_atoms, light="tiles", batch=batch)
                if tp.tiles_only and tp.flags() & 8:
                    object.__setattr__(mp, "_dmpnn_no_mega", True)
            return 1
    return 1 if no_mega else 2


class AtomMessagePassing(BondMessagePassing):

    def __init__(self, d_v: int = DEFAULT_ATOM_FDIM, d_e: int = DEFAULT_BOND_FDIM,
                 d_h: int = DEFAULT_HIDDEN_DIM, bias: bool = False, depth: int = 3, dropout: float = 0.0,
                 activation="relu", undirected: bool = False, d_vd: Optional[int] = None,
                 V_d_transform: Optional[nn.Module] = None, graph_transform: Optional[nn.Module] = None):
        nn.Module.__init__(self)
        self.hparams = _HParams(d_v=d_v, d_e=d_e, d_h=d_h, bias=bias, depth=depth, dropout=dropout,
                                activation=activation, undirected=undirected, d_vd=d_vd,
                                V_d_transform=V_d_transform, graph_transform=graph_transform,
                                cls=self.__class__)
        self.W_i = nn.Linear(d_v, d_h, bias)
        self.W_h = nn.Linear(d_e + d_h, d_h, bias)
        self.W_o = nn.Linear(d_v + d_h, d_h)
        self.W_d = nn.Linear(d_h + d_vd, d_h + d_vd) if d_vd else None
        self.depth = depth
        self.undirected = undirected
        self.dropout = nn.Dropout(dropout)
        self.tau = get_activation_function(activation)
        self.V_d_transform = V_d_transform if V_d_transform is not None else nn.Identity()
        self.graph_transform = graph_transform if graph_transform is not None else nn.Identity()

    def forward(self, bmg, V_d: Optional[Tensor] = None) -> Tensor:
        return atom_message_passing_forward(self, bmg, V_d)


def atom_message_passing_forward(mp, bmg, V_d: Optional[Tensor] = None) -> Tensor:
    from .backward import aggregate_fn, gather_src_fn, linear_fn

    if V_d is None and not torch.is_grad_enabled():
        r = mp.__dict__.get("_dmpnn_replay")
        if r is not None:
            out = _replay_forward(mp, r, bmg)
            if out is not None:
                return out
    bmg = mp.graph_transform(bmg)
    engine._require_device(bmg.V, "bmg.V")
    if mp.W_i.weight.device != bmg.V.device:
        raise RuntimeError(f"module is on {mp.W_i.weight.device} but the batch is on {bmg.V.device}")
    n_atoms = int(bmg.V.shape[0])
    has_vd = False
    if V_d is not None:
        V_d = mp.V_d_transform(V_d)
        d_vd = (mp.W_d.in_features - mp.W_o.out_features) if mp.W_d is not None else None
        if mp.W_d is None or V_d.dim() != 2 or V_d.shape[0] != n_atoms or V_d.shape[1] != d_vd:
            raise InvalidShapeError("V_d", V_d.shape, [n_atoms, d_vd if d_vd is not None else 0])
        has_vd = True
    n_mols = len(bmg) if hasattr(bmg, "__len__") else 0
    if n_mols and getattr(bmg, "batch", None) is not None:
        from .agg import note_batch

        note_batch(bmg.batch, n_mols)
    V, E = bmg.V, bmg.E
    act, slope, slope_t = classify_activation(mp.tau)
    grad = torch.is_grad_enabled() and any(p.requires_grad for p in mp.parameters())
    if (not grad and not has_vd and act != "custom" and not mp.undirected and not (mp.training and mp.dropout.p > 0)
            and 1 <= int(E.shape[1]) <= 16 and int(E.shape[0]) > 0 and batch_oversize(bmg, n_mols) is False):
        nV_, nE_ = int(V.shape[0]), int(E.shape[0])
        loader_tiles = getattr(bmg, "tiles", None) is not None or (
            getattr(bmg, "batch", None) is not None and not engine.small_plan_fits(nV_, nE_) and bool(_lib.load().dmpnn_tile_plan_any_size(nV_, nE_)))
# ... 93 lines not shown
```

### include/dmpnn.h

```cpp
#ifndef DMPNN_H
#define DMPNN_H

#include <stddef.h>
#include <stdint.h>

#ifdef __cplusplus
extern "C" {
#endif

#define DMPNN_ABI_VERSION 15

enum dmpnn_status {
    DMPNN_OK = 0,
    DMPNN_EINVAL = -1,
    DMPNN_EHIP = -2,
    DMPNN_ENOSPC = -3
};

enum dmpnn_activation {
    DMPNN_ACT_NONE = 0,
    DMPNN_ACT_RELU = 1,
    DMPNN_ACT_LEAKYRELU = 2,
    DMPNN_ACT_PRELU = 3,
    DMPNN_ACT_TANH = 4,
// ... 14 lines not shown
    DMPNN_F_TILE_PLAN = 1u << 11,
    DMPNN_F_STORE16 = 1u << 7
};

size_t dmpnn_plan_bytes(int64_t n_atoms, int64_t n_edges);

int dmpnn_prepare(const int64_t* edge_index,
                  const int64_t* rev_edge_index,
                  int64_t n_atoms, int64_t n_edges, void* plan, size_t plan_bytes, void* stream);
int dmpnn_prepare_light(const int64_t* edge_index, const int64_t* rev_edge_index, int64_t n_atoms, int64_t n_edges,
                        void* plan, size_t plan_bytes, void* stream);

int dmpnn_prepare_tiles(const int64_t* edge_index, const int64_t* rev_edge_index, const int64_t* batch, int64_t n_atoms,
                        int64_t n_edges, void* plan, size_t plan_bytes, void* stream);
int dmpnn_tile_plan_any_size(int64_t n_atoms, int64_t n_edges);

int dmpnn_prepare_with_batch(const int64_t* edge_index, const int64_t* rev_edge_index, const int64_t* batch, int64_t n_atoms,
                             int64_t n_edges, void* plan, size_t plan_bytes, void* stream);
int dmpnn_full_plan_keeps_tiles(int64_t n_atoms, int64_t n_edges);

enum dmpnn_plan_hdr {
    DMPNN_HDR_FLAGS = 0,
    DMPNN_HDR_MAXDEG = 1,
    DMPNN_HDR_NATOMS = 2,
    DMPNN_HDR_NEDGES = 3,
    DMPNN_HDR_NTILES = 4,
    DMPNN_HDR_TILE_STRIDE = 5,
    DMPNN_HDR_NMTILES = 6,
    DMPNN_HDR_LIGHT = 7,
    DMPNN_HDR_NSPILL = 8,
    DMPNN_HDR_WORDS = 16
};
#define DMPNN_PLAN_NOFFSETS 15
int dmpnn_plan_layout(int64_t n_atoms, int64_t n_edges, int64_t offsets_out[DMPNN_PLAN_NOFFSETS]);


int dmpnn_message_fwd(const void* plan, int64_t n_atoms, int64_t n_edges, int64_t d_h,
                      const float* Hin, int64_t ld_in, float* M, int64_t ld_m,
                      int act_on_load, float act_slope, const float* act_slope_ptr,
                      unsigned flags, void* stream);

int dmpnn_aggregate_fwd(const void* plan, int64_t n_atoms, int64_t n_edges, int64_t d_h,
                        const float* Hin, int64_t ld_in, float* Mv, int64_t ld_mv,
                        int act_on_load, float act_slope, const float* act_slope_ptr, void* stream);

typedef struct dmpnn_gemm_args {
    int64_t M, N, K1, K2;
    const float* A1; int64_t lda1; const int32_t* gather1;
    int64_t gather1_rows;
    const float* A2; int64_t lda2;
    const float* W;  int64_t ldw;
    const float* bias;
    const float* Cadd; int64_t ldcadd;
    float* C; int64_t ldc;
    float* Zpre; int64_t ldz;
    int act; float act_slope; const float* act_slope_ptr;
} dmpnn_gemm_args;
int dmpnn_linear_fwd(const dmpnn_gemm_args* a, void* stream);
size_t dmpnn_linear16_wsplit_bytes(int64_t N, int64_t K);
int dmpnn_linear16_ok(const dmpnn_gemm_args* a);
int dmpnn_linear16_fwd(const dmpnn_gemm_args* a, void* wsplit, size_t wsplit_bytes, int wsplit_ready, void* stream);

int dmpnn_update_fwd(const void* plan, int64_t n_atoms, int64_t n_edges, int64_t d_h,
                     const float* M, int64_t ld_m, const float* H0, int64_t ld_h0,
                     const float* W_h, const float* b_h,
                     float* H_out, int64_t ld_hout, float* M_next, int64_t ld_mnext,
                     float* Mv, int64_t ld_mv,
                     int act, float act_slope, const float* act_slope_ptr, void* stream);

typedef struct dmpnn_fwd_args {
    const void* plan; int64_t n_atoms, n_edges;
    int64_t d_v, d_e, d_h, d_vd; int32_t depth; uint32_t flags;
    int32_t act; float act_slope; const float* act_slope_ptr;
    const float* V; int64_t ldv;
    const float* E; int64_t lde;
    const float* V_d; int64_t ldvd;
    const float* W_i; const float* b_i;
    const float* W_h; const float* b_h;
    const float* W_o; const float* b_o;
    const float* W_d; const float* b_d;
    int64_t ldh; float* H0; float* Hs; int32_t n_hslots; float* Ms; int32_t n_mslots;
    float* Mv; float* Hv;
    float* out; int64_t ldout;
    void* wsplit; size_t wsplit_bytes;
    const int64_t* edge_index; const int64_t* rev_edge_index;
    int64_t n_tiles_launch;
    float* spill_ws; size_t spill_bytes;
    void* msplit; size_t msplit_bytes;
    float dropout_p; uint64_t dropout_seed;
    void* keep_bits; size_t keep_bits_bytes;
    size_t h0_bytes;
} dmpnn_fwd_args;
size_t dmpnn_forward_wsplit_bytes(const dmpnn_fwd_args* a);
size_t dmpnn_forward_keep_bits_bytes(const dmpnn_fwd_args* a);
size_t dmpnn_forward_h0_bytes(const dmpnn_fwd_args* a);
int64_t dmpnn_split_row_floats(int64_t d_h);
int dmpnn_forward_can_fuse16(const dmpnn_fwd_args* a);
size_t dmpnn_forward_spill_bytes(const dmpnn_fwd_args* a);
int dmpnn_forward(const dmpnn_fwd_args* a, void* stream);
int dmpnn_forward_tiles(const dmpnn_fwd_args* a, const int64_t* batch, const int* tile_row, const int* tile_atom, int64_t n_tiles,
                        size_t plan_bytes, void* stream);
int dmpnn_forward_can_fuse(const dmpnn_fwd_args* a);
enum dmpnn_route { DMPNN_ROUTE_GENERAL = 0, DMPNN_ROUTE_GENERAL16 = 1, DMPNN_ROUTE_FUSED = 2, DMPNN_ROUTE_FUSED16 = 3,
                   DMPNN_ROUTE_MEGA = 4, DMPNN_ROUTE_MEGA16 = 5 };
int dmpnn_forward_route(const dmpnn_fwd_args* a, int keep, int max_level, int plan_kind, int arith);
int dmpnn_tile_waves(int64_t n_atoms, int64_t n_edges, int64_t d_h, int64_t n_tiles);

#define DMPNN_KEEP_ROWS_MIN 4096
typedef struct dmpnn_train_route_info {
    int32_t plan_kind;
    int32_t route;
    int32_t keep_rows;
    int32_t keep_bits;
    int32_t lean;
} dmpnn_train_route_info;
int dmpnn_train_route(const dmpnn_fwd_args* a, int64_t n_mols, int32_t have, int32_t oversize, int32_t max_level, int32_t arith,
                      int32_t keep_rows, dmpnn_train_route_info* out);

typedef struct dmpnn_bwd_args {
    dmpnn_fwd_args f;
    const float* gout; int64_t ldgout;
    float* gW_i; float* gb_i; float* gW_h; float* gb_h;
    float* gW_o; float* gb_o; float* gW_d; float* gb_d;
    float* ws; size_t ws_bytes;
    const float* g_edge; int64_t ld_gedge;
} dmpnn_bwd_args;
size_t dmpnn_backward_ws_bytes(const dmpnn_fwd_args* f);
int dmpnn_backward(const dmpnn_bwd_args* a, void* stream);

int dmpnn_message_bwd(const void* plan, int64_t n_atoms, int64_t n_edges, int64_t d_h,
                      const float* gM, int64_t ld_gm, float* gH, int64_t ld_gh, void* stream);
int dmpnn_aggregate_bwd(const void* plan, int64_t n_atoms, int64_t n_edges, int64_t d_h,
                        const float* gMv, int64_t ld_gmv, float* gH, int64_t ld_gh, void* stream);
size_t dmpnn_linear_wgrad_ws_bytes(int64_t M, int64_t N, int64_t K, int has_bias);
int dmpnn_linear_wgrad(const dmpnn_gemm_args* g, const float* gZ, int64_t ldgz, float* gW, int64_t ldgw,
                       float* gb, void* ws, size_t ws_bytes, void* stream);

enum dmpnn_molagg_mode { DMPNN_MOLAGG_SUM = 0, DMPNN_MOLAGG_MEAN = 1, DMPNN_MOLAGG_NORM = 2 };
size_t dmpnn_molagg_ws_bytes(int64_t n_mols);
int dmpnn_molagg_bounds(const int64_t* batch, int64_t n_atoms, int64_t n_mols, void* ws, size_t ws_bytes, void* stream);
int dmpnn_molagg_fwd(const float* H, int64_t ldh, int64_t n_atoms, int64_t d_h, int64_t n_mols, const void* ws, int mode,
                     float norm, float* out, int64_t ldo, void* stream);
int dmpnn_molagg_bwd(const float* gout, int64_t ldg, const int64_t* batch, int64_t n_atoms, int64_t d_h, int64_t n_mols,
                     const void* ws, int mode, float norm, float* gH, int64_t ldgh, void* stream);

int dmpnn_gather_rows(const float* X, int64_t ldx, int64_t n_src, const int* idx, int64_t n_out, int64_t d,
                      float* out, int64_t ldo, void* stream);

int dmpnn_collate(const int* atom_off, const int* edge_off, int64_t n_mols, const int* src, const int* dst, const int* rev,
                  int64_t n_atoms, int64_t n_edges, int64_t* edge_index, int64_t* rev_edge_index, int64_t* batch,
                  void* stream);

int64_t dmpnn_pack_tiles(const int* atom_off, const int* edge_off, int64_t n_mols, int* tile_row, int* tile_atom, int64_t cap);
int64_t dmpnn_max_tiles(int64_t n_atoms, int64_t n_edges);
int dmpnn_prepare_tiles_from_table(const int* tile_row, const int* tile_atom, int64_t n_tiles, int64_t n_atoms,
                                   int64_t n_edges, void* plan, size_t plan_bytes, void* stream);

int dmpnn_adam_step(float* p, const float* g, float* m, float* v, int64_t n, float lr, float beta1, float beta2, float eps,
                    float weight_decay, float bias_corr1, float sqrt_bias_corr2, float grad_scale, const float* dev_scalars,
                    void* stream);

enum dmpnn_clip_mode { DMPNN_CLIP_NORM = 0, DMPNN_CLIP_VALUE = 1 };
size_t dmpnn_clip_grad_ws_bytes(void);
int dmpnn_clip_grad(float* g, int64_t n, float clip_val, int32_t mode, float grad_scale, float* ws, void* stream);

#define DMPNN_MAX_FFN_LAYERS 8
#define DMPNN_MAX_COMPONENTS 8
#define DMPNN_DROP_SITE_FFN 0x10000
enum dmpnn_loss { DMPNN_LOSS_MSE = 0, DMPNN_LOSS_MAE = 1,
                  DMPNN_LOSS_BCE = 2,
                  DMPNN_LOSS_CE = 3,
                  DMPNN_LOSS_MVE = 4,
                  DMPNN_LOSS_EVIDENTIAL = 5,
                  DMPNN_LOSS_QUANTILE = 6  };
typedef struct dmpnn_head_args {
    int64_t n_atoms, n_mols, d_h;
    const int64_t* batch;
    int32_t agg_mode; float agg_norm;
    const float* bn_weight; const float* bn_bias;
    float* bn_running_mean; float* bn_running_var;
    float bn_eps, bn_momentum; int32_t bn_training;
    int32_t n_layers; int32_t act; float act_slope;
    const float* W[DMPNN_MAX_FFN_LAYERS];
    const float* b[DMPNN_MAX_FFN_LAYERS];
    int64_t dims[DMPNN_MAX_FFN_LAYERS + 1];
    int32_t loss;
    const float* targets;
    const float* weights;
    const float* task_weights;
    const unsigned char* lt_mask; const unsigned char* gt_mask;
    float* preds;
    float* loss_out;
    float* gW[DMPNN_MAX_FFN_LAYERS]; float* gb[DMPNN_MAX_FFN_LAYERS];
    float* g_bn_weight; float* g_bn_bias;
    float* gHv; int64_t ldg;
    void* ws; size_t ws_bytes;
    int64_t* bn_num_batches_tracked;
    int32_t n_classes;
    float evid_v_kl, evid_eps;
    float quantile_alpha;
    const float* X_d; int64_t ld_xd;
    int32_t n_components;
    float ffn_dropout_p; uint64_t ffn_dropout_seed;
} dmpnn_head_args;
size_t dmpnn_head_ws_bytes(const dmpnn_head_args* h);
int dmpnn_head(const dmpnn_head_args* h, const float* Hv, int64_t ldhv, void* stream);

enum dmpnn_step_stage {
    DMPNN_STEP_FORWARD = 1,
    DMPNN_STEP_BACKWARD = 2,
    DMPNN_STEP_UPDATE = 4
};
typedef struct dmpnn_step_component {
    const int64_t* edge_index; const int64_t* rev_edge_index; const int64_t* batch; size_t plan_bytes; int32_t plan_ready;
    dmpnn_bwd_args bwd;
} dmpnn_step_component;

#define DMPNN_VD_MAX_WIDTH 544
typedef struct dmpnn_vd_args {
    int64_t n_atoms, d_h, d_vd;
    const float* Hv;  int64_t ldhv;
    const float* V_d; int64_t ldvd;
    const float* W_d; const float* b_d;
    float* out; int64_t ldout;
    const float* gout; int64_t ldgout;
    float* gHv; int64_t ldghv;
    float* gW_d; float* gb_d;
    void* ws; size_t ws_bytes;
} dmpnn_vd_args;
size_t dmpnn_vd_ws_bytes(const dmpnn_vd_args* a);
int dmpnn_vd_forward(const dmpnn_vd_args* a, void* stream);
int dmpnn_vd_backward(const dmpnn_vd_args* a, void* stream);

typedef struct dmpnn_step_args {
    const int64_t* edge_index; const int64_t* rev_edge_index; const int64_t* batch; size_t plan_bytes; int32_t plan_ready;
    int32_t stages;
    dmpnn_bwd_args bwd;
    dmpnn_head_args head;
    float* p; const float* g; float* m; float* v; int64_t n_params;
    float lr, beta1, beta2, eps, weight_decay, bias_corr1, sqrt_bias_corr2, grad_scale; const float* dev_scalars;
    float clip_val; int32_t clip_mode; float* clip_ws;
    int32_t n_extra; const dmpnn_step_component* extra;
    const dmpnn_vd_args* vd;
} dmpnn_step_args;
int dmpnn_train_step(const dmpnn_step_args* a, void* stream);

int dmpnn_dropout_keep(uint64_t seed, int32_t site, int64_t row, int64_t col, float p);

int dmpnn_version(void);
int dmpnn_debug_timestamps(void* device_buf);
void dmpnn_debug_lds_poison(int on);
const char* dmpnn_last_error_string(void);
int dmpnn_last_launch_count(void);

#ifdef __cplusplus
}
#endif
#endif
```

Before: 475.5 M edge-updates/s.

## Precompute molecule tile table on host and validate it on device during weight split

```diff
diff --git a/chemprop_amd/_lib.py b/chemprop_amd/_lib.py
--- a/chemprop_amd/_lib.py
+++ b/chemprop_amd/_lib.py
@@ -22,7 +22,7 @@
     "dmpnn_plan_layout", "dmpnn_prepare", "dmpnn_prepare_light", "dmpnn_prepare_tiles", "dmpnn_message_fwd", "dmpnn_aggregate_fwd",
     "dmpnn_linear_fwd", "dmpnn_linear16_wsplit_bytes", "dmpnn_linear16_ok", "dmpnn_linear16_fwd", "dmpnn_update_fwd", "dmpnn_forward", "dmpnn_forward_can_fuse", "dmpnn_forward_wsplit_bytes", "dmpnn_forward_keep_bits_bytes", "dmpnn_forward_spill_bytes", "dmpnn_backward_ws_bytes", "dmpnn_backward", "dmpnn_message_bwd",
     "dmpnn_aggregate_bwd", "dmpnn_linear_wgrad_ws_bytes", "dmpnn_linear_wgrad",
-    "dmpnn_molagg_ws_bytes", "dmpnn_molagg_bounds", "dmpnn_molagg_fwd", "dmpnn_molagg_bwd", "dmpnn_gather_rows", "dmpnn_collate", "dmpnn_pack_tiles", "dmpnn_max_tiles",
+    "dmpnn_molagg_ws_bytes", "dmpnn_molagg_bounds", "dmpnn_molagg_fwd", "dmpnn_molagg_bwd", "dmpnn_gather_rows", "dmpnn_collate", "dmpnn_pack_tiles", "dmpnn_pack_tiles_blocked", "dmpnn_max_tiles",
     "dmpnn_prepare_tiles_from_table", "dmpnn_prepare_with_batch", "dmpnn_tile_plan_any_size", "dmpnn_split_row_floats", "dmpnn_forward_can_fuse16", "dmpnn_adam_step",
     "dmpnn_full_plan_keeps_tiles", "dmpnn_head_ws_bytes", "dmpnn_head", "dmpnn_train_step", "dmpnn_forward_tiles", "dmpnn_forward_route", "dmpnn_dropout_keep",
     "dmpnn_clip_grad", "dmpnn_clip_grad_ws_bytes", "dmpnn_train_route", "dmpnn_forward_h0_bytes", "dmpnn_tile_waves", "dmpnn_debug_lds_poison",
@@ -292,6 +292,8 @@
                                       C.c_void_p]
     lib.dmpnn_pack_tiles.argtypes = [C.c_void_p, C.c_void_p, C.c_int64, C.c_void_p, C.c_void_p, C.c_int64]
     lib.dmpnn_pack_tiles.restype = C.c_int64
+    lib.dmpnn_pack_tiles_blocked.argtypes = [C.c_void_p, C.c_void_p, C.c_int64, C.c_void_p, C.c_void_p, C.c_int64]
+    lib.dmpnn_pack_tiles_blocked.restype = C.c_int64
     lib.dmpnn_max_tiles.argtypes = [C.c_int64, C.c_int64]
     lib.dmpnn_prepare_with_batch.argtypes = [C.c_void_p, C.c_void_p, C.c_void_p, C.c_int64, C.c_int64, C.c_void_p, C.c_size_t, C.c_void_p]
     lib.dmpnn_prepare_with_batch.restype = C.c_int
@@ -334,7 +336,7 @@
     for name in size_t_fns:
         getattr(lib, name).restype = C.c_size_t
     for name in EXPORTS:
-        if name != "dmpnn_last_error_string" and name not in size_t_fns and name not in ("dmpnn_pack_tiles", "dmpnn_max_tiles", "dmpnn_split_row_floats"):
+        if name != "dmpnn_last_error_string" and name not in size_t_fns and name not in ("dmpnn_pack_tiles", "dmpnn_pack_tiles_blocked", "dmpnn_max_tiles", "dmpnn_split_row_floats"):
             getattr(lib, name).restype = C.c_int
     if lib.dmpnn_version() != ABI_VERSION:
         raise RuntimeError(f"libdmpnn ABI version {lib.dmpnn_version()} != {ABI_VERSION} (stale build?)")
diff --git a/chemprop_amd/csrc/dmpnn_abi.hip b/chemprop_amd/csrc/dmpnn_abi.hip
--- a/chemprop_amd/csrc/dmpnn_abi.hip
+++ b/chemprop_amd/csrc/dmpnn_abi.hip
@@ -385,7 +385,15 @@
     DMPNN_CHECK_ARG(a != nullptr && a->plan != nullptr, "forward_tiles: null args / plan");
     void* plan = const_cast<void*>(a->plan);
     bool did_split = false;
-    if (tile_row && tile_atom && n_tiles > 0) {
+    if (batch && tile_row && tile_atom && n_tiles > 0) {
+        const dmpnn::PlanLayout L = dmpnn::plan_layout(a->n_atoms, a->n_edges);
+        const bool ok = a->n_atoms > 0 && a->n_edges > 0 && a->n_atoms < (1ll << 31) && a->n_edges < (1ll << 31) &&
+                        plan_bytes >= (size_t)L.words * sizeof(int) && n_tiles <= L.max_mtiles;
+        if (ok) DMPNN_TRY(launch_tiles_checked_split(a->edge_index, batch, tile_row, tile_atom, n_tiles, a->n_atoms, a->n_edges, static_cast<int*>(plan),
+                                                     static_cast<hipStream_t>(stream), a, &did_split));
+        if (!did_split)
+            DMPNN_TRY(prepare_tiles_and_bounds(a->edge_index, a->rev_edge_index, batch, a->n_atoms, a->n_edges, plan, plan_bytes, nullptr, 0, stream, nullptr, a, &did_split));
+    } else if (tile_row && tile_atom && n_tiles > 0) {
         const dmpnn::PlanLayout L = dmpnn::plan_layout(a->n_atoms, a->n_edges);
         const bool ok = a->n_atoms >= 0 && a->n_edges >= 0 && a->n_atoms < (1ll << 31) && a->n_edges < (1ll << 31) &&
                         plan_bytes >= (size_t)L.words * sizeof(int) && n_tiles <= L.max_mtiles;
diff --git a/chemprop_amd/csrc/dmpnn_collate.hip b/chemprop_amd/csrc/dmpnn_collate.hip
--- a/chemprop_amd/csrc/dmpnn_collate.hip
+++ b/chemprop_amd/csrc/dmpnn_collate.hip
@@ -58,6 +58,29 @@
     return n;
 }
 
+extern "C" int64_t dmpnn_pack_tiles_blocked(const int* atom_off, const int* edge_off, int64_t n_mols, int* tile_row, int* tile_atom,
+                                            int64_t cap) {
+    if (n_mols < 0 || cap < 1 || !tile_row || !tile_atom || (n_mols > 0 && (!atom_off || !edge_off))) return -2;
+    int64_t n = 0;
+    for (int64_t base = 0; base < n_mols; base += 64) {
+        const int64_t lim = base + 64 < n_mols ? base + 64 : n_mols;
+        int64_t p = base;
+        while (p < lim) {
+            const int a0 = atom_off[p], e0 = edge_off[p];
+            if (n + 1 >= cap) return -2;
+            tile_row[n] = e0; tile_atom[n] = a0;
+            ++n;
+            int64_t q = p + 1;
+            if (atom_off[q] - a0 <= dmpnn::kMegaBA && edge_off[q] - e0 <= dmpnn::kMegaBM)
+                while (q < n_mols && atom_off[q + 1] - a0 <= dmpnn::kMegaBA && edge_off[q + 1] - e0 <= dmpnn::kMegaBM) ++q;
+            p = q;
+        }
+    }
+    tile_row[n] = n_mols ? edge_off[n_mols] : 0;
+    tile_atom[n] = n_mols ? atom_off[n_mols] : 0;
+    return n;
+}
+
 extern "C" int64_t dmpnn_max_tiles(int64_t n_atoms, int64_t n_edges) { return dmpnn::mega_max_tiles(n_atoms, n_edges); }
 
 extern "C" int dmpnn_prepare_tiles_from_table(const int* tile_row, const int* tile_atom, int64_t n_tiles, int64_t n_atoms,
diff --git a/chemprop_amd/csrc/dmpnn_common.hpp b/chemprop_amd/csrc/dmpnn_common.hpp
--- a/chemprop_amd/csrc/dmpnn_common.hpp
+++ b/chemprop_amd/csrc/dmpnn_common.hpp
@@ -75,7 +75,9 @@
 }
 
 enum : int { PLAN_ASYMMETRIC = 1, PLAN_RANGE_ERROR = 2, PLAN_HUGE_DEGREE = 4, PLAN_NO_PIECE_TILES = 8,
-             PLAN_TILES_ONLY = 16 };
+             PLAN_TILES_ONLY = 16,
+             PLAN_CHECK_WORDS = 32 };
+constexpr int kPlanCheckWords = 16;
 constexpr int kPlanNoFuse = PLAN_ASYMMETRIC | PLAN_RANGE_ERROR | PLAN_HUGE_DEGREE | PLAN_TILES_ONLY;
 constexpr int kPlanNoMegaLean = PLAN_RANGE_ERROR | PLAN_NO_PIECE_TILES;
 constexpr int kPlanNoMega = kPlanNoFuse | PLAN_NO_PIECE_TILES;
@@ -160,7 +162,8 @@
                    int light, hipStream_t s, bool keep_mtiles = false);
 bool prepare_can_keep_mtiles(int64_t nV, int64_t nE);
 __device__ __forceinline__ void tiles_from_table_body(const int* __restrict__ tile_row, const int* __restrict__ tile_atom,
-                                                          int n_tiles, int nV, int nE, int* __restrict__ plan, PlanLayout L) {
+                                                          int n_tiles, int nV, int nE, int* __restrict__ plan, PlanLayout L,
+                                                          int extra_flags = 0) {
     __shared__ int bad_s, spill_s;
     if (threadIdx.x == 0) { bad_s = 0; spill_s = 0; }
     __syncthreads();
@@ -187,7 +190,7 @@
     if (threadIdx.x < DMPNN_HDR_WORDS) {
         int v = 0;
         const int h = threadIdx.x;
-        if (h == DMPNN_HDR_FLAGS) v = (bad_s ? PLAN_NO_PIECE_TILES : 0) | PLAN_TILES_ONLY;
+        if (h == DMPNN_HDR_FLAGS) v = (bad_s ? PLAN_NO_PIECE_TILES : 0) | PLAN_TILES_ONLY | extra_flags;
         if (h == DMPNN_HDR_NMTILES) v = bad_s ? 0 : n_tiles;
         if (h == DMPNN_HDR_NSPILL) v = bad_s ? 0 : spill_s;
         if (h == DMPNN_HDR_LIGHT) v = 2;
@@ -200,6 +203,8 @@
 
 int launch_tiles_from_table_split(const int* tile_row, const int* tile_atom, int64_t n_tiles, int64_t nV, int64_t nE, int* plan, hipStream_t s,
                                   const dmpnn_fwd_args* split_for, bool* did_split);
+int launch_tiles_checked_split(const int64_t* edge_index, const int64_t* batch, const int* tile_row, const int* tile_atom, int64_t n_tiles,
+                               int64_t nV, int64_t nE, int* plan, hipStream_t s, const dmpnn_fwd_args* split_for, bool* did_split);
 int launch_prepare_tiles_batch(const int64_t* edge_index, const int64_t* batch, int64_t nV, int64_t nE, int* plan, hipStream_t s,
                                int* mol_bounds = nullptr, int64_t n_mols = 0, const dmpnn_fwd_args* split_for = nullptr, bool* did_split = nullptr);
 bool mega16_split_args(const dmpnn_fwd_args& a, mega16::SplitArgs* sp);
diff --git a/chemprop_amd/csrc/dmpnn_mega16_impl.hpp b/chemprop_amd/csrc/dmpnn_mega16_impl.hpp
--- a/chemprop_amd/csrc/dmpnn_mega16_impl.hpp
+++ b/chemprop_amd/csrc/dmpnn_mega16_impl.hpp
@@ -96,13 +96,43 @@
     const bool live = n < NJ;
     const long long rs = J.tr ? 1 : J.ldw, ks = J.tr ? J.ldw : 1;
     const float* row = J.W + (long long)(live ? n : 0) * rs;
+    _Float16* out = reinterpret_cast<_Float16*>(J.out);
+    const int T = n >> 4, li = n & 15;
+    if (J.nc <= 16 && J.scale_K <= 512) {
+        float v[8], sv[8];
+        const int k0 = lane * 8;
+        const bool own_scale = J.scale_col0 == J.col0 && J.scale_K == J.K;
+#pragma unroll
+        for (int q = 0; q < 8; ++q) v[q] = (k0 + q < J.K && live) ? row[(J.col0 + k0 + q) * ks] : 0.f;
+#pragma unroll
+        for (int q = 0; q < 8; ++q) sv[q] = (!own_scale && live && lane + 64 * q < J.scale_K) ? row[(J.scale_col0 + lane + 64 * q) * ks] : 0.f;
+        float mx = 0.f;
+#pragma unroll
+        for (int q = 0; q < 8; ++q) mx = fmaxf(mx, fabsf(own_scale ? v[q] : sv[q]));
+        for (int off = 32; off > 0; off >>= 1) mx = fmaxf(mx, __shfl_xor(mx, off));
+        const float s = live ? scale_for(mx) : 0.f;
+        if (lane == 0 && J.inv_scale && live) J.inv_scale[n] = 1.f / s;
+        if (k0 < J.nc * 32) {
+            h8 hv, lv;
+#pragma unroll
+            for (int q = 0; q < 8; ++q) {
+                const float x = (k0 + q < J.K && live) ? v[q] * s : 0.f;
+                const _Float16 hi = (_Float16)x;
+                const _Float16 lo = (_Float16)(x - (float)hi);
+                hv[q] = hi; lv[q] = lo;
+            }
+            const int c = k0 >> 5, lg = (k0 & 31) >> 3;
+            const long long base = (((long long)T * J.nc + c) * 2) * 512 + (lg * 16 + li) * 8;
+            *reinterpret_cast<h8*>(out + base) = hv;
+            *reinterpret_cast<h8*>(out + base + 512) = lv;
+        }
+        return;
+    }
     float mx = 0.f;
     for (int k = lane; k < J.scale_K; k += 64) mx = fmaxf(mx, fabsf(row[(J.scale_col0 + k) * ks]));
     for (int off = 32; off > 0; off >>= 1) mx = fmaxf(mx, __shfl_xor(mx, off));
     const float s = live ? scale_for(mx) : 0.f;
     if (lane == 0 && J.inv_scale && live) J.inv_scale[n] = 1.f / s;
-    _Float16* out = reinterpret_cast<_Float16*>(J.out);
-    const int T = n >> 4, li = n & 15;
     for (int k = lane; k < J.nc * 32; k += 64) {
         const float x = (k < J.K && live) ? row[(J.col0 + k) * ks] * s : 0.f;
         const _Float16 hi = (_Float16)x;
@@ -207,7 +237,8 @@
     int rs = g.mtile_row[t], re = g.mtile_row[t + 1];
     int va = g.mtile_atom[t], vb = g.mtile_atom[t + 1];
     int hdr_light = g.flags[DMPNN_HDR_LIGHT], hdr_flags = g.flags[0], hdr_tiles = g.flags[DMPNN_HDR_NMTILES];
-    asm volatile("" : "+v"(rs), "+v"(re), "+v"(va), "+v"(vb), "+v"(hdr_light), "+v"(hdr_flags), "+v"(hdr_tiles));
+    int chk = g.flags[DMPNN_HDR_WORDS + (lane & (kPlanCheckWords - 1))];
+    asm volatile("" : "+v"(rs), "+v"(re), "+v"(va), "+v"(vb), "+v"(hdr_light), "+v"(hdr_flags), "+v"(hdr_tiles), "+v"(chk));
     rs = __builtin_amdgcn_readfirstlane(rs); re = __builtin_amdgcn_readfirstlane(re);
     va = __builtin_amdgcn_readfirstlane(va); vb = __builtin_amdgcn_readfirstlane(vb);
     hdr_light = __builtin_amdgcn_readfirstlane(hdr_light); hdr_flags = __builtin_amdgcn_readfirstlane(hdr_flags);
@@ -216,7 +247,7 @@
     const int N = g.h, qn = N >> 2;
     const bool lean = hdr_light == 2;
     const bool poison = (hdr_flags & (lean ? kPlanNoMegaLean : g.poison_mask)) != 0 || (lean && g.nE > 0 && (!g.edge_index || !g.rev64)) ||
-                        hdr_tiles > (int)gridDim.x;
+                        hdr_tiles > (int)gridDim.x || ((hdr_flags & PLAN_CHECK_WORDS) != 0 && __ballot(chk != 0) != 0ull);
     if (poison) {
         const float nanv = __int_as_float(0x7fc00000);
         const long long total = (long long)g.nV * N;
diff --git a/chemprop_amd/csrc/dmpnn_prepare.hip b/chemprop_amd/csrc/dmpnn_prepare.hip
--- a/chemprop_amd/csrc/dmpnn_prepare.hip
+++ b/chemprop_amd/csrc/dmpnn_prepare.hip
@@ -949,6 +949,86 @@
     else mega16::split_weights_wave(sp, ((int)blockIdx.x - 1) * 4 + (int)(threadIdx.x >> 6), (int)(threadIdx.x & 63));
 }
 
+constexpr int kCheckThreads = 256, kCheckItems = 4, kCheckPerBlock = kCheckThreads * kCheckItems;
+__device__ __forceinline__ void tiles_check_block(const int64_t* __restrict__ edge_index, const int64_t* __restrict__ batch,
+                                                  const int* __restrict__ tile_atom, int n_tiles, int nV, int nE, int* __restrict__ plan, int b) {
+    __shared__ int bad_blk;
+    if (threadIdx.x == 0) bad_blk = 0;
+    __syncthreads();
+    const int64_t* dst = edge_index + nE;
+    int64_t bm[kCheckItems], bp[kCheckItems], d[kCheckItems], dp[kCheckItems];
+    int ta[kCheckItems];
+#pragma unroll
+    for (int j = 0; j < kCheckItems; ++j) {
+        const int i = (b * kCheckItems + j) * kCheckThreads + (int)threadIdx.x;
+        bm[j] = i < nV ? batch[i] : 0;
+        bp[j] = (i > 0 && i < nV) ? batch[i - 1] : 0;
+        d[j] = i < nE ? dst[i] : 0;
+        dp[j] = (i > 0 && i < nE) ? dst[i - 1] : 0;
+        ta[j] = i < n_tiles ? tile_atom[i] : 0;
+    }
+    int bad = 0;
+    int64_t em[kCheckItems], ep[kCheckItems], tb[kCheckItems], tp[kCheckItems];
+#pragma unroll
+    for (int j = 0; j < kCheckItems; ++j) {
+        const int i = (b * kCheckItems + j) * kCheckThreads + (int)threadIdx.x;
+        if (i < nE && (d[j] < 0 || d[j] >= nV)) { bad |= PLAN_RANGE_ERROR; d[j] = 0; }
+        if (dp[j] < 0 || dp[j] >= nV) dp[j] = 0;
+        em[j] = i < nE ? batch[d[j]] : 0;
+        ep[j] = (i > 0 && i < nE) ? batch[dp[j]] : 0;
+        const bool inner = i < n_tiles && ta[j] > 0 && ta[j] < nV;
+        tb[j] = inner ? batch[ta[j]] : 1;
+        tp[j] = inner ? batch[ta[j] - 1] : 0;
+    }
+#pragma unroll
+    for (int j = 0; j < kCheckItems; ++j) {
+        const int i = (b * kCheckItems + j) * kCheckThreads + (int)threadIdx.x;
+        if (i < nV) {
+            if (bm[j] < 0 || bm[j] >= nV) bad |= PLAN_RANGE_ERROR;
+            if (i > 0 && bm[j] < bp[j]) bad |= PLAN_NO_PIECE_TILES;
+        }
+        if (i > 0 && i < nE && em[j] < ep[j]) bad |= PLAN_NO_PIECE_TILES;
+        if (tb[j] <= tp[j]) bad |= PLAN_NO_PIECE_TILES;
+    }
+    if (bad) atomicOr(&bad_blk, bad);
+    __syncthreads();
+    if (threadIdx.x == 0) plan[DMPNN_HDR_WORDS + b] = bad_blk;
+}
+
+__global__ __launch_bounds__(kCheckThreads) void k_tiles_checked_split(const int64_t* __restrict__ edge_index, const int64_t* __restrict__ batch,
+                                                                      const int* __restrict__ tile_row, const int* __restrict__ tile_atom, int n_tiles,
+                                                                      int nV, int nE, int n_check, int* __restrict__ plan, PlanLayout L, mega16::SplitArgs sp) {
+    const int b = (int)blockIdx.x;
+    if (b == 0) {
+        tiles_from_table_body(tile_row, tile_atom, n_tiles, nV, nE, plan, L, PLAN_CHECK_WORDS);
+        if ((int)threadIdx.x >= n_check && (int)threadIdx.x < kPlanCheckWords) plan[DMPNN_HDR_WORDS + threadIdx.x] = 0;
+    } else if (b <= n_check) {
+        tiles_check_block(edge_index, batch, tile_atom, n_tiles, nV, nE, plan, b - 1);
+    } else {
+        mega16::split_weights_wave(sp, (b - 1 - n_check) * (kCheckThreads / 64) + (int)(threadIdx.x >> 6), (int)(threadIdx.x & 63));
+    }
+}
+
+}
+
+int launch_tiles_checked_split(const int64_t* edge_index, const int64_t* batch, const int* tile_row, const int* tile_atom, int64_t n_tiles,
+                               int64_t nV, int64_t nE, int* plan, hipStream_t s, const dmpnn_fwd_args* split_for, bool* did_split) {
+    *did_split = false;
+    mega16::SplitArgs sp;
+    const PlanLayout L = plan_layout(nV, nE);
+    const int64_t n_items = nV > nE ? nV : nE;
+    const int n_check = (int)((n_items + kCheckPerBlock - 1) / kCheckPerBlock);
+    if (!split_for || !batch || !edge_index || nV <= 0 || nE <= 0 || n_tiles <= 0 || n_tiles > nV || n_check > kPlanCheckWords ||
+        L.words < DMPNN_HDR_WORDS + kPlanCheckWords || L.mtile_row < DMPNN_HDR_WORDS + kPlanCheckWords ||
+        !(split_for->flags & DMPNN_F_FUSED) || !(split_for->flags & DMPNN_F_MEGA) || !(split_for->flags & DMPNN_F_SPLIT16) ||
+        (split_for->flags & (DMPNN_F_WSPLIT_READY | DMPNN_F_KEEP)) || !mega16_split_args(*split_for, &sp))
+        return DMPNN_OK;
+    const int waves = ((sp.N + 15) & ~15) * sp.n_jobs, wpb = kCheckThreads / 64;
+    hipLaunchKernelGGL(k_tiles_checked_split, dim3((unsigned)(1 + n_check + (waves + wpb - 1) / wpb)), dim3(kCheckThreads), 0, s, edge_index, batch,
+                       tile_row, tile_atom, (int)n_tiles, (int)nV, (int)nE, n_check, plan, L, sp);
+    DMPNN_CHECK_LAUNCH("k_tiles_checked_split");
+    *did_split = true;
+    return DMPNN_OK;
 }
 
 int launch_tiles_from_table_split(const int* tile_row, const int* tile_atom, int64_t n_tiles, int64_t nV, int64_t nE, int* plan, hipStream_t s,
diff --git a/chemprop_amd/data.py b/chemprop_amd/data.py
--- a/chemprop_amd/data.py
+++ b/chemprop_amd/data.py
@@ -23,9 +23,45 @@
     return bool(n_atoms.size and (int(n_atoms.max()) > TILE_MAX_ATOMS or int(n_edges.max()) > TILE_MAX_EDGES))
 
 
+SMALL_PLAN_MAX_ATOMS, SMALL_PLAN_MAX_EDGES = 6144, 10240
+_FIVE = frozenset(("V", "E", "edge_index", "rev_edge_index", "batch"))
+
+
+def host_tile_plan(n_atoms, n_edges):
+    n_atoms, n_edges = np.asarray(n_atoms, dtype=np.int64), np.asarray(n_edges, dtype=np.int64)
+    with_atoms = np.flatnonzero(n_atoms)
+    if not with_atoms.size or molecules_oversize(n_atoms, n_edges):
+        return None
+    n = int(with_atoms[-1]) + 1
+    nV, nE = int(n_atoms[:n].sum()), int(n_edges.sum())
+    if nE == 0 or nV > SMALL_PLAN_MAX_ATOMS or nE > SMALL_PLAN_MAX_EDGES or int(n_edges[:n].sum()) != nE:
+        return None
+    try:
+        from . import _lib
+
+        lib = _lib.load()
+    except (OSError, RuntimeError):
+        return None
+    atom_off, edge_off = np.zeros(n + 1, dtype=np.int32), np.zeros(n + 1, dtype=np.int32)
+    atom_off[1:] = np.cumsum(n_atoms[:n])
+    edge_off[1:] = np.cumsum(n_edges[:n])
+    cap = int(lib.dmpnn_max_tiles(nV, nE)) + 1
+    trow, tatom = np.empty(cap, dtype=np.int32), np.empty(cap, dtype=np.int32)
+    nt = int(lib.dmpnn_pack_tiles_blocked(atom_off.ctypes.data, edge_off.ctypes.data, n, trow.ctypes.data, tatom.ctypes.data, cap))
+    if nt <= 0:
+        return None
+    return trow[:nt + 1], tatom[:nt + 1], nt
+
+
 class BatchMolGraph:
 
-    __slots__ = ("V", "E", "edge_index", "rev_edge_index", "batch", "_size", "tiles", "oversize")
+    __slots__ = ("V", "E", "edge_index", "rev_edge_index", "batch", "_size", "tiles", "oversize", "plan_table", "_bt")
+
+    def __setattr__(self, name, value):
+        object.__setattr__(self, name, value)
+        if name in _FIVE:
+            object.__setattr__(self, "plan_table", None)
+            object.__setattr__(self, "_bt", None)
 
     def __init__(self, mgs: Sequence[MolGraph]):
         self._size = len(mgs)
@@ -42,17 +78,45 @@
         self.edge_index = torch.from_numpy(ei).long()
         rev = np.concatenate([mg.rev_edge_index + o for mg, o in zip(mgs, edge_off)])
         self.rev_edge_index = torch.from_numpy(rev).long()
-        self.batch = torch.from_numpy(np.repeat(np.arange(len(mgs), dtype=np.int64), n_atoms))
+        bt = np.repeat(np.arange(len(mgs), dtype=np.int64), n_atoms)
+        plan = None if self.oversize else host_tile_plan(n_atoms, n_edges)
+        if plan is None:
+            self.batch = torch.from_numpy(bt)
+        else:
+            nV, nt = len(bt), plan[2]
+            buf = np.zeros(nV + nt + 1, dtype=np.int64)
+            buf[:nV] = bt
+            tab = buf[nV:].view(np.int32)
+            tab[:nt + 1], tab[nt + 1:] = plan[0], plan[1]
+            self._set_packed(torch.from_numpy(buf), nV, nt)
+
+    def _set_packed(self, buf: Tensor, nV: int, nt: int) -> None:
+        tab = buf[nV:].view(torch.int32)
+        self.batch = buf[:nV]
+        self.plan_table, self._bt = (tab[:nt + 1], tab[nt + 1:], nt), buf
+
+    def __getstate__(self):
+        return {k: getattr(self, k) for k in self.__slots__ if hasattr(self, k)}
+
+    def __setstate__(self, state):
+        for k, v in state.items():
+            object.__setattr__(self, k, v)
+        if state.get("_bt") is not None and state.get("plan_table") is not None:
+            self._set_packed(state["_bt"], int(state["batch"].numel()), state["plan_table"][2])
 
     def __len__(self) -> int:
         return self._size
 
     def to(self, device) -> None:
+        table, bt = self.plan_table, self._bt
         self.V = self.V.to(device)
         self.E = self.E.to(device)
         self.edge_index = self.edge_index.to(device)
         self.rev_edge_index = self.rev_edge_index.to(device)
-        self.batch = self.batch.to(device)
+        if table is not None and bt is not None:
+            self._set_packed(bt.to(device), int(self.batch.numel()), table[2])
+        else:
+            self.batch = self.batch.to(device)
         self.tiles = None
 
     @classmethod
@@ -64,12 +128,14 @@
         self._size = int(size) if size is not None else (int(batch[-1]) + 1 if batch.numel() else 0)
         self.tiles = None
         self.oversize = None
+        self.plan_table, self._bt = None, None
         return self
 
     def __copy__(self):
         b = BatchMolGraph.from_tensors(self.V, self.E, self.edge_index, self.rev_edge_index, self.batch, self._size)
         b.tiles = self.tiles
         b.oversize = self.oversize
+        b.plan_table, b._bt = self.plan_table, self._bt
         return b
 
 
diff --git a/chemprop_amd/engine.py b/chemprop_amd/engine.py
--- a/chemprop_amd/engine.py
+++ b/chemprop_amd/engine.py
@@ -86,7 +86,7 @@
 class GraphPlan:
 
     __slots__ = ("buf", "n_atoms", "n_edges", "device", "light", "tiles_only", "edge_index", "rev_edge_index", "loader_tiles",
-                 "any_size", "oversize", "pending", "_job")
+                 "any_size", "oversize", "pending", "_job", "host_tiles")
 
     def __init__(self, edge_index: Tensor, rev_edge_index: Tensor, n_atoms: int, light=False, batch: Optional[Tensor] = None,
                  tiles: Optional[tuple] = None, launch: bool = True):
@@ -120,6 +120,7 @@
         self.any_size = (self.tiles_only and not small) or full_tiles
         self.edge_index, self.rev_edge_index = ei, rev
         self.pending, self._job = None, None
+        self.host_tiles = None
         if launch == "defer":
             if self.tiles_only and small and not self.loader_tiles and bt is not None:
                 self.pending = bt
@@ -671,7 +672,13 @@
         with _OnDevice(dev):
             if pend is not None and use_mega and want16 and tiles_only:
                 plan.pending = None
-                _lib.check(lib.dmpnn_forward_tiles(C.byref(a), pend.data_ptr(), None, None, 0, plan.buf.numel() * 4, _stream_ptr(dev)), "dmpnn_forward_tiles")
+                ht = getattr(plan, "host_tiles", None) if not keep else None
+                if ht is not None:
+                    a.n_tiles_launch = ht[2]
+                    _lib.check(lib.dmpnn_forward_tiles(C.byref(a), pend.data_ptr(), ht[0].data_ptr(), ht[1].data_ptr(), ht[2],
+                                                       plan.buf.numel() * 4, _stream_ptr(dev)), "dmpnn_forward_tiles")
+                else:
+                    _lib.check(lib.dmpnn_forward_tiles(C.byref(a), pend.data_ptr(), None, None, 0, plan.buf.numel() * 4, _stream_ptr(dev)), "dmpnn_forward_tiles")
             else:
                 if pend is not None:
                     plan.ensure_launched()
diff --git a/chemprop_amd/nn.py b/chemprop_amd/nn.py
--- a/chemprop_amd/nn.py
+++ b/chemprop_amd/nn.py
@@ -201,6 +201,9 @@
     tiles = getattr(bmg, "tiles", None)
     if tiles is not None and (tiles[0].device != dev or tiles[2] <= 0):
         tiles = None
+    own = getattr(bmg, "plan_table", None) if tiles is None else None
+    if own is not None and own[0].device != dev:
+        own = None
     small = engine.small_plan_fits(nV, nE)
     lib = _lib.load()
     if (n_mols <= 0 or nE > 30 * n_mols or nE == 0 or (tiles is None and not small and not lib.dmpnn_tile_plan_any_size(nV, nE))
@@ -235,6 +238,10 @@
             a.flags = r.flags | _lib.F_LOADER_TILES
             a.n_tiles_launch = tiles[2]
             rc = lib.dmpnn_forward_tiles(_ctypes.byref(a), None, tiles[0].data_ptr(), tiles[1].data_ptr(), tiles[2], nbytes, stream)
+        elif own is not None:
+            a.flags = r.flags if small else (r.flags | _lib.F_LOADER_TILES)
+            a.n_tiles_launch = own[2]
+            rc = lib.dmpnn_forward_tiles(_ctypes.byref(a), batch.data_ptr(), own[0].data_ptr(), own[1].data_ptr(), own[2], nbytes, stream)
         else:
             a.flags = r.flags if small else (r.flags | _lib.F_LOADER_TILES)
             a.n_tiles_launch = n_mols
@@ -320,6 +327,9 @@
     if not light and torch.is_grad_enabled() and V_d is None:
         light = _training_plan_kind(mp, bmg) if oversize is not True else False
     plan = engine.GraphPlan.from_bmg(bmg, light=light, launch="defer" if light == "tiles" else True)
+    own = getattr(bmg, "plan_table", None)
+    if own is not None and plan.pending is not None and not torch.is_grad_enabled() and own[0].device == plan.device:
+        plan.host_tiles = own
     if n_mols and getattr(bmg, "batch", None) is not None:
         from .agg import note_batch
 
diff --git a/include/dmpnn.h b/include/dmpnn.h
--- a/include/dmpnn.h
+++ b/include/dmpnn.h
@@ -190,6 +190,7 @@
                   void* stream);
 
 int64_t dmpnn_pack_tiles(const int* atom_off, const int* edge_off, int64_t n_mols, int* tile_row, int* tile_atom, int64_t cap);
+int64_t dmpnn_pack_tiles_blocked(const int* atom_off, const int* edge_off, int64_t n_mols, int* tile_row, int* tile_atom, int64_t cap);
 int64_t dmpnn_max_tiles(int64_t n_atoms, int64_t n_edges);
 int dmpnn_prepare_tiles_from_table(const int* tile_row, const int* tile_atom, int64_t n_tiles, int64_t n_atoms,
                                    int64_t n_edges, void* plan, size_t plan_bytes, void* stream);
```

Result: faster. 526.1 M edge-updates/s (median of 6 runs) (+10.6%).
